# monatis/clip.cpp

Measured on AMD Instinct MI355X. Metric: image+text embeddings/sec, higher is better.
Workload: dtype f16

## Files before the change

### clip_cpp_amd/__init__.py

```python
import ctypes as C
import os
import weakref

import numpy as np

_HERE = os.path.dirname(os.path.abspath(__file__))
LIB_PATH = os.environ.get("CLIP_AMD_LIB") or os.path.join(_HERE, "libclip.so")


class ClipTextHparams(C.Structure):
    _fields_ = [("n_vocab", C.c_int32), ("num_positions", C.c_int32), ("hidden_size", C.c_int32),
                ("n_intermediate", C.c_int32), ("projection_dim", C.c_int32), ("n_head", C.c_int32),
                ("n_layer", C.c_int32), ("eps", C.c_float)]


class ClipVisionHparams(C.Structure):
    _fields_ = [("image_size", C.c_int32), ("patch_size", C.c_int32), ("hidden_size", C.c_int32),
                ("n_intermediate", C.c_int32), ("projection_dim", C.c_int32), ("n_head", C.c_int32),
                ("n_layer", C.c_int32), ("eps", C.c_float)]


class ClipTokens(C.Structure):
    _fields_ = [("data", C.POINTER(C.c_int32)), ("size", C.c_size_t)]


class ClipImageU8(C.Structure):
    _fields_ = [("nx", C.c_int), ("ny", C.c_int), ("data", C.POINTER(C.c_uint8)), ("size", C.c_size_t)]


class ClipImageF32(C.Structure):
    _fields_ = [("nx", C.c_int), ("ny", C.c_int), ("data", C.POINTER(C.c_float)), ("size", C.c_size_t)]


class ClipImageU8Batch(C.Structure):
    _fields_ = [("data", C.POINTER(ClipImageU8)), ("size", C.c_size_t)]


class ClipImageF32Batch(C.Structure):
    _fields_ = [("data", C.POINTER(ClipImageF32)), ("size", C.c_size_t)]


API_SYMBOLS = [
    "clip_model_load", "clip_free", "clip_get_text_hparams", "clip_get_vision_hparams", "clip_tokenize",
    "clip_image_u8_make", "clip_image_f32_make", "clip_image_u8_clean", "clip_image_f32_clean", "clip_image_u8_free",
    "clip_image_f32_free", "clip_image_load_from_file", "clip_image_preprocess", "clip_image_batch_preprocess",
    "clip_text_encode", "clip_image_encode", "clip_image_batch_encode", "clip_compare_text_and_image",
    "clip_similarity_score", "softmax_with_sorting", "clip_zero_shot_label_image", "clip_model_quantize",
    "ggml_time_init", "ggml_time_us", "ggml_time_ms",
]
AMD_SYMBOLS = [
    "clip_amd_device_count", "clip_amd_model_load", "clip_amd_model_load_multi", "clip_amd_ctx_device_count", "clip_amd_weights_from_cache", "clip_amd_shard_bounds",
    "clip_amd_gathered_embeddings", "clip_amd_ctx_device", "clip_amd_set_stream", "clip_amd_set_device_shared", "clip_amd_image_batch_encode_device_multi",
    "clip_amd_text_batch_encode_device_multi", "clip_amd_encode_pair_device_multi",
    "clip_amd_image_batch_encode_device", "clip_text_batch_encode", "clip_amd_text_batch_encode_device",
    "clip_amd_image_batch_preprocess_device", "clip_amd_image_batch_encode_u8",
    "clip_amd_zero_shot_score_device", "clip_amd_zero_shot_label_images",
    "clip_amd_synchronize", "clip_amd_profile_enable", "clip_amd_profile_read", "clip_amd_profile_report",
    "clip_amd_test_gemm", "clip_amd_test_gemm_ex", "clip_amd_test_gemm_tile", "clip_amd_test_gemm_tile_ex", "clip_amd_test_skinny", "clip_amd_test_layernorm", "clip_amd_test_attention", "clip_amd_bench_gemm",
    "clip_amd_test_attention_ex", "clip_amd_bench_attention",
    "clip_amd_test_layernorm_ex", "clip_amd_test_text_embed", "clip_amd_test_im2col", "clip_amd_test_layernorm_prep", "clip_amd_test_rows",
    "clip_amd_index_create", "clip_amd_index_add", "clip_amd_index_add_device", "clip_amd_index_size", "clip_amd_index_dim",
    "clip_amd_index_search", "clip_amd_index_search_device", "clip_amd_index_save", "clip_amd_index_load", "clip_amd_index_free",
    "clip_amd_bench_search", "clip_amd_index_range_search", "clip_amd_index_pairs", "clip_amd_bench_range",
    "clip_amd_index_remove", "clip_amd_index_live", "clip_amd_index_live_mask", "clip_amd_index_compact", "clip_amd_index_search_subset",
    "clip_amd_index_search_subset_device", "clip_amd_index_range_search_subset", "clip_amd_bench_search_subset",
    "clip_amd_index_search_ids", "clip_amd_index_search_ids_device", "clip_amd_index_knn_graph", "clip_amd_test_index_knn_route", "clip_amd_bench_knn",
    "clip_amd_index_search_index", "clip_amd_index_append", "clip_amd_test_index_cross_route", "clip_amd_bench_cross",
    "clip_amd_image_batch_encode_files", "clip_amd_image_batch_encode_memory", "clip_amd_test_jpeg_plan", "clip_amd_test_jpeg_decode_device",
    "clip_amd_bench_jpeg_kernels", "clip_amd_test_jpeg_device_count",
    "clip_amd_index_search_grouped", "clip_amd_index_search_grouped_device", "clip_amd_bench_search_grouped",
    "clip_amd_image_batch_encode_regions", "clip_amd_image_batch_preprocess_regions_device", "clip_amd_image_batch_encode_files_grid",
    "clip_amd_image_batch_encode_memory_grid",
    "clip_amd_index_search_sets", "clip_amd_index_search_sets_device", "clip_amd_index_search_ids_sets", "clip_amd_test_index_sets_block",
    "clip_amd_bench_search_sets",
    "clip_amd_index_search_distinct", "clip_amd_index_search_distinct_device", "clip_amd_index_search_ids_distinct",
    "clip_amd_test_index_distinct_block", "clip_amd_bench_search_distinct",
]

_lib = None


def build_lib(force=False):
    import importlib
    return importlib.import_module(__name__ + ".build").build(force=force)


def lib():
    global _lib
    if _lib is not None:
        return _lib
    if not os.path.exists(LIB_PATH):
        build_lib()
    L = C.CDLL(LIB_PATH)
    vp, i32, f32p = C.c_void_p, C.c_int, C.POINTER(C.c_float)
    L.clip_model_load.restype = vp
    L.clip_model_load.argtypes = [C.c_char_p, i32]
    L.clip_amd_model_load.restype = vp
    L.clip_amd_model_load.argtypes = [C.c_char_p, i32, i32]
    L.clip_amd_model_load_multi.restype = vp
    L.clip_amd_model_load_multi.argtypes = [C.c_char_p, i32, i32]
    L.clip_amd_ctx_device_count.restype = i32
    L.clip_amd_ctx_device_count.argtypes = [vp]
    L.clip_amd_weights_from_cache.restype = i32
    L.clip_amd_weights_from_cache.argtypes = [vp]
    L.clip_amd_shard_bounds.argtypes = [i32, i32, i32, C.POINTER(i32), C.POINTER(i32), C.POINTER(i32)]
    L.clip_amd_gathered_embeddings.restype = vp
    L.clip_amd_gathered_embeddings.argtypes = [vp, i32]
    L.clip_free.argtypes = [vp]
    L.clip_get_text_hparams.restype = C.POINTER(ClipTextHparams)
    L.clip_get_text_hparams.argtypes = [vp]
    L.clip_get_vision_hparams.restype = C.POINTER(ClipVisionHparams)
    L.clip_get_vision_hparams.argtypes = [vp]
    L.clip_tokenize.restype = C.c_bool
    L.clip_tokenize.argtypes = [vp, C.c_char_p, C.POINTER(ClipTokens)]
    L.clip_image_u8_make.restype = C.POINTER(ClipImageU8)
    L.clip_image_f32_make.restype = C.POINTER(ClipImageF32)
    L.clip_image_u8_clean.argtypes = [C.POINTER(ClipImageU8)]
    L.clip_image_f32_clean.argtypes = [C.POINTER(ClipImageF32)]
    L.clip_image_u8_free.argtypes = [C.POINTER(ClipImageU8)]
    L.clip_image_f32_free.argtypes = [C.POINTER(ClipImageF32)]
    L.clip_image_load_from_file.restype = C.c_bool
    L.clip_image_load_from_file.argtypes = [C.c_char_p, C.POINTER(ClipImageU8)]
    L.clip_image_preprocess.restype = C.c_bool
    L.clip_image_preprocess.argtypes = [vp, C.POINTER(ClipImageU8), C.POINTER(ClipImageF32)]
    L.clip_image_batch_preprocess.argtypes = [vp, i32, C.POINTER(ClipImageU8Batch), C.POINTER(ClipImageF32Batch)]
    L.clip_text_encode.restype = C.c_bool
    L.clip_text_encode.argtypes = [vp, i32, C.POINTER(ClipTokens), f32p, C.c_bool]
    L.clip_text_batch_encode.restype = C.c_bool
    L.clip_text_batch_encode.argtypes = [vp, i32, C.POINTER(ClipTokens), C.c_size_t, f32p, C.c_bool]
    L.clip_image_encode.restype = C.c_bool
    L.clip_image_encode.argtypes = [vp, i32, C.POINTER(ClipImageF32), f32p, C.c_bool]
    L.clip_image_batch_encode.restype = C.c_bool
    L.clip_image_batch_encode.argtypes = [vp, i32, C.POINTER(ClipImageF32Batch), f32p, C.c_bool]
    L.clip_compare_text_and_image.restype = C.c_bool
    L.clip_compare_text_and_image.argtypes = [vp, i32, C.c_char_p, C.POINTER(ClipImageU8), f32p]
    L.clip_similarity_score.restype = C.c_float
    L.clip_similarity_score.argtypes = [f32p, f32p, i32]
    L.softmax_with_sorting.restype = C.c_bool
    L.softmax_with_sorting.argtypes = [f32p, i32, f32p, C.POINTER(C.c_int)]
    L.clip_zero_shot_label_image.restype = C.c_bool
    L.clip_zero_shot_label_image.argtypes = [vp, i32, C.POINTER(ClipImageU8), C.POINTER(C.c_char_p), C.c_size_t, f32p,
                                             C.POINTER(C.c_int)]
    L.clip_model_quantize.restype = C.c_bool
    L.clip_model_quantize.argtypes = [C.c_char_p, C.c_char_p, i32]
    L.clip_amd_device_count.restype = i32
    L.clip_amd_ctx_device.restype = i32
    L.clip_amd_ctx_device.argtypes = [vp]
    L.clip_amd_set_stream.argtypes = [vp, vp]
    L.clip_amd_set_device_shared.restype = None
    L.clip_amd_set_device_shared.argtypes = [vp, i32]
    L.clip_amd_synchronize.argtypes = [vp]
    L.clip_amd_image_batch_encode_device.restype = C.c_bool
    L.clip_amd_image_batch_encode_device.argtypes = [vp, vp, i32, vp, C.c_bool]
    L.clip_amd_image_batch_preprocess_device.restype = C.c_bool
    L.clip_amd_image_batch_preprocess_device.argtypes = [vp, C.POINTER(ClipImageU8), i32, vp]
    L.clip_amd_zero_shot_score_device.restype = C.c_bool
    L.clip_amd_zero_shot_score_device.argtypes = [vp, vp, i32, vp, i32, i32, vp, vp]
    L.clip_amd_zero_shot_label_images.restype = C.c_bool
    L.clip_amd_zero_shot_label_images.argtypes = [vp, C.POINTER(ClipImageU8), i32, C.POINTER(C.c_char_p), C.c_size_t, f32p, C.POINTER(C.c_int)]
    L.clip_amd_image_batch_encode_u8.restype = C.c_bool
    L.clip_amd_image_batch_encode_u8.argtypes = [vp, C.POINTER(ClipImageU8), i32, f32p, C.c_bool]
    L.clip_amd_text_batch_encode_device.restype = C.c_bool
    L.clip_amd_text_batch_encode_device.argtypes = [vp, vp, C.POINTER(C.c_int32), i32, vp, C.c_bool]
    L.clip_amd_image_batch_encode_device_multi.restype = C.c_bool
    L.clip_amd_image_batch_encode_device_multi.argtypes = [vp, C.POINTER(vp), i32, C.c_bool, f32p]
    L.clip_amd_text_batch_encode_device_multi.restype = C.c_bool
    L.clip_amd_text_batch_encode_device_multi.argtypes = [vp, C.POINTER(vp), C.POINTER(C.c_int32), i32, C.c_bool, f32p]
    L.clip_amd_encode_pair_device_multi.restype = C.c_bool
    L.clip_amd_encode_pair_device_multi.argtypes = [vp, C.POINTER(vp), i32, C.POINTER(vp), C.POINTER(C.c_int32), i32, C.c_bool, f32p, f32p]
    L.clip_amd_profile_enable.argtypes = [vp, C.c_bool]
    L.clip_amd_profile_report.restype = i32
    L.clip_amd_profile_report.argtypes = [vp, C.c_char_p, i32, C.c_bool]
    L.clip_amd_test_gemm.restype = i32
    L.clip_amd_test_gemm.argtypes = [i32, vp, C.c_int64, C.c_int64, f32p, C.c_int64, f32p, f32p, f32p, i32, i32]
    L.clip_amd_test_gemm_ex.restype = i32
    L.clip_amd_test_gemm_ex.argtypes = [i32, vp, C.c_int64, C.c_int64, f32p, C.c_int64, f32p, f32p, f32p, i32, i32, i32, C.c_float, i32, i32, f32p]
    L.clip_amd_test_lnfold.restype = i32
    L.clip_amd_test_lnfold.argtypes = [i32, vp, C.c_int64, C.c_int64, vp, C.c_int64, f32p, C.c_int64, f32p, f32p, f32p, f32p, C.c_float, f32p,
                                       i32, i32, i32, i32, i32, C.c_float, f32p, f32p]
    L.clip_amd_test_gemm_tile.restype = i32
    L.clip_amd_test_gemm_tile.argtypes = [C.c_int64, C.c_int64, C.c_int64, i32]
    L.clip_amd_test_gemm_tile_ex.restype = i32
    L.clip_amd_test_gemm_tile_ex.argtypes = [C.c_int64, C.c_int64, C.c_int64, i32, i32]
    L.clip_amd_test_skinny.restype = i32
    L.clip_amd_test_skinny.argtypes = [i32, vp, C.c_int64, C.c_int64, f32p, C.c_int64, f32p, f32p, f32p, f32p, C.c_float, f32p, i32, i32, C.c_float, f32p]
    L.clip_amd_bench_gemm.restype = C.c_float
    L.clip_amd_bench_gemm.argtypes = [i32, C.c_int64, C.c_int64, C.c_int64, i32, i32, i32]
    L.clip_amd_test_layernorm.restype = i32
    L.clip_amd_test_layernorm.argtypes = [f32p, f32p, f32p, C.c_float, C.c_int64, C.c_int64, f32p, i32]
    u16p, i32p = C.POINTER(C.c_uint16), C.POINTER(C.c_int32)
    L.clip_amd_test_layernorm_ex.restype = i32
    L.clip_amd_test_layernorm_ex.argtypes = [f32p, C.c_int64, i32, i32p, i32, f32p, f32p, C.c_float, i32, i32, u16p, i32, f32p, i32]
    L.clip_amd_test_text_embed.restype = i32
    L.clip_amd_test_text_embed.argtypes = [i32, vp, C.c_int64, i32, i32p, i32p, i32, i32, f32p, i32, f32p, i32, f32p, u16p, i32, f32p, f32p]
    L.clip_amd_test_im2col.restype = i32
    L.clip_amd_test_im2col.argtypes = [f32p, i32, i32, i32, i32, i32, u16p]
    L.clip_amd_test_layernorm_prep.restype = i32
    L.clip_amd_test_layernorm_prep.argtypes = [f32p, i32, f32p, f32p, C.c_float, i32, i32, f32p, i32, f32p, f32p, i32, i32, f32p, i32, u16p, i32, f32p, f32p]
    L.clip_amd_test_rows.restype = i32
    L.clip_amd_test_rows.argtypes = [i32, vp, vp, i32p, C.c_int64, C.c_int64, C.c_int64, C.c_int64, C.c_int64, vp, vp]
    L.clip_amd_test_attention.restype = i32
    L.clip_amd_test_attention.argtypes = [f32p, i32, i32, i32, i32, i32, f32p]
    L.clip_amd_test_attention_ex.restype = i32
    L.clip_amd_test_attention_ex.argtypes = [f32p, i32, i32, i32, i32, i32, f32p, i32]
    L.clip_amd_bench_attention.restype = C.c_float
    L.clip_amd_bench_attention.argtypes = [i32, i32, i32, i32, i32, i32, i32]
    i64, i64p = C.c_int64, C.POINTER(C.c_int64)
    L.clip_amd_index_create.restype = vp
    L.clip_amd_index_create.argtypes = [vp, i32, i32]
    L.clip_amd_index_add.restype = C.c_bool
    L.clip_amd_index_add.argtypes = [vp, f32p, i64]
    L.clip_amd_index_add_device.restype = C.c_bool
    L.clip_amd_index_add_device.argtypes = [vp, vp, i64]
    L.clip_amd_index_size.restype = i64
    L.clip_amd_index_size.argtypes = [vp]
    L.clip_amd_index_dim.restype = i32
    L.clip_amd_index_dim.argtypes = [vp]
    L.clip_amd_index_search.restype = C.c_bool
    L.clip_amd_index_search.argtypes = [vp, f32p, i32, i32, f32p, i64p]
    L.clip_amd_index_search_device.restype = C.c_bool
    L.clip_amd_index_search_device.argtypes = [vp, vp, i32, i32, vp, vp]
    L.clip_amd_index_save.restype = C.c_bool
    L.clip_amd_index_save.argtypes = [vp, C.c_char_p]
    L.clip_amd_index_load.restype = vp
    L.clip_amd_index_load.argtypes = [vp, C.c_char_p]
    L.clip_amd_index_free.restype = None
    L.clip_amd_index_free.argtypes = [vp]
    L.clip_amd_bench_search.restype = C.c_float
    L.clip_amd_bench_search.argtypes = [i32, i64, i32, i32, i32, i32]
    L.clip_amd_index_range_search.restype = i64
    L.clip_amd_index_range_search.argtypes = [vp, f32p, i32, C.c_float, i64p, f32p, i64p, i64]
    L.clip_amd_index_pairs.restype = i64
    L.clip_amd_index_pairs.argtypes = [vp, C.c_float, i64p, f32p, i64p, i64]
    L.clip_amd_bench_range.restype = C.c_float
    L.clip_amd_bench_range.argtypes = [i32, i64, i32, i32, C.c_float, i32]
    u64p = C.POINTER(C.c_uint64)
    L.clip_amd_index_remove.restype = i64
    L.clip_amd_index_remove.argtypes = [vp, i64p, i64]
    L.clip_amd_index_live.restype = i64
    L.clip_amd_index_live.argtypes = [vp]
    L.clip_amd_index_live_mask.restype = C.c_bool
    L.clip_amd_index_live_mask.argtypes = [vp, u64p]
    L.clip_amd_index_compact.restype = i64
    L.clip_amd_index_compact.argtypes = [vp, i64p]
    L.clip_amd_index_search_subset.restype = C.c_bool
    L.clip_amd_index_search_subset.argtypes = [vp, f32p, i32, i32, u64p, f32p, i64p]
    L.clip_amd_index_search_subset_device.restype = C.c_bool
    L.clip_amd_index_search_subset_device.argtypes = [vp, vp, i32, i32, vp, vp, vp]
    L.clip_amd_index_range_search_subset.restype = i64
    L.clip_amd_index_range_search_subset.argtypes = [vp, f32p, i32, C.c_float, u64p, i64p, f32p, i64p, i64]
    L.clip_amd_index_search_grouped.restype = C.c_bool
    L.clip_amd_index_search_grouped.argtypes = [vp, f32p, i32, i32, C.POINTER(C.c_int32), u64p, f32p, i64p]
    L.clip_amd_index_search_grouped_device.restype = C.c_bool
    L.clip_amd_index_search_grouped_device.argtypes = [vp, vp, i32, i32, vp, vp, vp, vp]
    L.clip_amd_bench_search_grouped.restype = C.c_float
    L.clip_amd_bench_search_grouped.argtypes = [i32, i64, i32, i32, i32, i32, i32]
    L.clip_amd_index_search_sets.restype = C.c_bool
    L.clip_amd_index_search_sets.argtypes = [vp, f32p, i32, i64p, i64, i32, C.POINTER(C.c_int32), u64p, f32p, i64p, C.POINTER(C.c_int32)]
    L.clip_amd_index_search_sets_device.restype = C.c_bool
    L.clip_amd_index_search_sets_device.argtypes = [vp, vp, i32, i64p, i64, i32, vp, vp, vp, vp, vp]
    L.clip_amd_index_search_ids_sets.restype = C.c_bool
    L.clip_amd_index_search_ids_sets.argtypes = [vp, i64p, i64, i64p, i64, i32, i32, C.POINTER(C.c_int32), u64p, f32p, i64p, C.POINTER(C.c_int32)]
    L.clip_amd_test_index_sets_block.restype = i64
    L.clip_amd_test_index_sets_block.argtypes = [vp, i64]
    L.clip_amd_bench_search_sets.restype = C.c_float
    L.clip_amd_bench_search_sets.argtypes = [i32, i64, i32, i32, i32, i32, i32, i32]
    L.clip_amd_index_search_distinct.restype = C.c_bool
    L.clip_amd_index_search_distinct.argtypes = [vp, f32p, i32, i32, C.c_float, i32, u64p, f32p, i64p, C.POINTER(C.c_int32)]
    L.clip_amd_index_search_distinct_device.restype = C.c_bool
    L.clip_amd_index_search_distinct_device.argtypes = [vp, vp, i32, i32, C.c_float, i32, vp, vp, vp, vp]
    L.clip_amd_index_search_ids_distinct.restype = C.c_bool
    L.clip_amd_index_search_ids_distinct.argtypes = [vp, i64p, i32, i32, C.c_float, i32, i32, u64p, f32p, i64p, C.POINTER(C.c_int32)]
    L.clip_amd_test_index_distinct_block.restype = i32
    L.clip_amd_test_index_distinct_block.argtypes = [vp, i32]
    L.clip_amd_bench_search_distinct.restype = C.c_float
    L.clip_amd_bench_search_distinct.argtypes = [i32, i64, i32, i32, i32, i32, C.c_float, i32, i32]
    L.clip_amd_bench_search_subset.restype = C.c_float
    L.clip_amd_bench_search_subset.argtypes = [i32, i64, i32, i32, i32, C.c_float, i32, i32]
    L.clip_amd_index_search_ids.restype = C.c_bool
    L.clip_amd_index_search_ids.argtypes = [vp, i64p, i32, i32, i32, u64p, f32p, i64p]
    L.clip_amd_index_search_ids_device.restype = C.c_bool
    L.clip_amd_index_search_ids_device.argtypes = [vp, vp, i32, i32, i32, vp, vp, vp]
    L.clip_amd_index_knn_graph.restype = C.c_bool
    L.clip_amd_index_knn_graph.argtypes = [vp, i32, f32p, i64p]
    L.clip_amd_test_index_knn_route.restype = i32
    L.clip_amd_test_index_knn_route.argtypes = [vp, i32]
    L.clip_amd_bench_knn.restype = C.c_float
    L.clip_amd_bench_knn.argtypes = [i32, i64, i32, i32, i32, i32]
    L.clip_amd_index_search_index.restype = C.c_bool
    L.clip_amd_index_search_index.argtypes = [vp, vp, i64p, i64, i32, u64p, f32p, i64p]
    L.clip_amd_index_append.restype = i64
    L.clip_amd_index_append.argtypes = [vp, vp, i64p]
    L.clip_amd_test_index_cross_route.restype = i32
    L.clip_amd_test_index_cross_route.argtypes = [vp, i32]
    L.clip_amd_bench_cross.restype = C.c_float
    L.clip_amd_bench_cross.argtypes = [i32, i64, i64, i32, i32, i32, i32]
    u8p, szp = C.POINTER(C.c_uint8), C.POINTER(C.c_size_t)
    L.clip_amd_image_batch_encode_files.restype = i32
    L.clip_amd_image_batch_encode_files.argtypes = [vp, C.POINTER(C.c_char_p), i32, i32, i32, C.c_bool, f32p, C.POINTER(i32), u8p]
    i32p = C.POINTER(C.c_int32)
    L.clip_amd_image_batch_encode_regions.restype = C.c_bool
    L.clip_amd_image_batch_encode_regions.argtypes = [vp, C.POINTER(ClipImageU8), i32, i32p, i32, f32p, C.c_bool]
    L.clip_amd_image_batch_preprocess_regions_device.restype = C.c_bool
    L.clip_amd_image_batch_preprocess_regions_device.argtypes = [vp, C.POINTER(ClipImageU8), i32, i32p, i32, vp]
    L.clip_amd_image_batch_encode_files_grid.restype = i32
    L.clip_amd_image_batch_encode_files_grid.argtypes = [vp, C.POINTER(C.c_char_p), i32, i32, i32, i32, C.c_bool, f32p, i32p, C.POINTER(i32), u8p]
    L.clip_amd_image_batch_encode_memory_grid.restype = i32
    L.clip_amd_image_batch_encode_memory_grid.argtypes = [vp, C.POINTER(C.c_char_p), szp, i32, i32, i32, i32, C.c_bool, f32p, i32p, C.POINTER(i32), u8p]
    L.clip_amd_image_batch_encode_memory.restype = i32
    L.clip_amd_image_batch_encode_memory.argtypes = [vp, C.POINTER(C.c_char_p), szp, i32, i32, i32, C.c_bool, f32p, C.POINTER(i32), u8p]
    L.clip_amd_test_jpeg_plan.restype = i32
    L.clip_amd_test_jpeg_plan.argtypes = [C.c_char_p, C.c_size_t, C.POINTER(i32)]
    L.clip_amd_test_jpeg_decode_device.restype = i32
    L.clip_amd_test_jpeg_decode_device.argtypes = [C.c_char_p, C.c_size_t, u8p, C.c_size_t, C.POINTER(i32), C.POINTER(i32)]
    L.clip_amd_test_jpeg_device_count.restype = C.c_longlong
    L.clip_amd_test_jpeg_device_count.argtypes = []
    L.clip_amd_bench_jpeg_kernels.restype = i32
    L.clip_amd_bench_jpeg_kernels.argtypes = [C.c_char_p, C.c_size_t, i32, i32, f32p, C.POINTER(C.c_double)]
    _lib = L
    return L


def device_count():
    return lib().clip_amd_device_count()


def _fp(a):
    return a.ctypes.data_as(C.POINTER(C.c_float))


def _struct_to_dict(s):
    return {f: getattr(s, f) for f, _ in s._fields_}


class Clip:

    def __init__(self, model_path_or_repo_id, verbosity=0, device=None, n_devices=None):
        L = lib()
# ... 728 lines not shown
```

### clip_cpp_amd/build.py

```python
import os
import shutil
import subprocess
import sys
from concurrent.futures import ThreadPoolExecutor

HERE = os.path.dirname(os.path.abspath(__file__))
CSRC = os.path.join(HERE, "csrc")
BUILD = os.path.join(HERE, "build")
LIB = os.path.join(HERE, "libclip.so")
GGML_STUB = os.path.join(HERE, "libggml.so")
ARCH = "gfx950"

HOST_SOURCES = ["gguf.cpp", "quant.cpp", "load.cpp", "forward.cpp", "tokenizer.cpp", "preprocess.cpp", "image_io.cpp", "image_formats.cpp",
                "jpeg_decode.cpp", "host_pipeline.cpp", "files_pipeline.cpp", "api.cpp", "search.cpp"]
HIP_SOURCES = ["k_attn.hip", "k_attn_long.hip", "k_attn_f32.hip", "k_misc.hip", "k_preproc.hip", "k_jpeg.hip", "k_gemm.hip", "k_gemm8.hip", "k_gemm4.hip", "k_gemm32.hip", "k_gemm_f32.hip", "k_skinny.hip", "k_gemm_ring.hip", "k_fold.hip", "k_search.hip", "k_join.hip", "k_graph.hip", "k_group.hip", "k_sets.hip", "k_distinct.hip"]
GEMM_WTYPES = [0, 1, 2, 3, 4, 5]
EXTRA_FLAGS = {"k_attn_f32.hip": ["-fno-slp-vectorize"], "k_attn_long.hip": ["-fno-slp-vectorize"], "k_gemm_f32.hip": ["-fno-slp-vectorize"]}

COMMON = ["-O3", "-std=c++17", "-fPIC", "-ffp-contract=off", "-Wall", "-Wno-unused-function", "-Wno-unused-result", "-Wno-inline-asm", "-Wno-bitwise-instead-of-logical",
          "-I" + os.path.join(os.path.dirname(HERE), "include")]


def hipcc():
    for c in (os.environ.get("HIPCC"), shutil.which("hipcc"), "/opt/rocm/bin/hipcc"):
        if c and os.path.exists(c):
            return c
    raise RuntimeError("hipcc not found")


def _newer(target, deps):
    if not os.path.exists(target):
        return True
    t = os.path.getmtime(target)
    return any(os.path.getmtime(d) > t for d in deps)


def _run(cmd):
    r = subprocess.run(cmd, stdout=subprocess.PIPE, stderr=subprocess.STDOUT, text=True)
    if r.returncode != 0:
        raise RuntimeError("command failed: %s\n%s" % (" ".join(cmd), r.stdout))
    return r.stdout


def build(force=False, verbose=False):
    os.makedirs(BUILD, exist_ok=True)
    cc = hipcc()
    headers = [os.path.join(CSRC, f) for f in os.listdir(CSRC) if f.endswith(".h")]
    headers += [os.path.join(os.path.dirname(HERE), "include", f) for f in ("clip.h", "clip_amd.h")]
    jobs = []
    objs = []
    for src in HOST_SOURCES:
        o = os.path.join(BUILD, src + ".o")
        objs.append(o)
        s = os.path.join(CSRC, src)
        if force or _newer(o, [s] + headers):
            jobs.append([cc, "-x", "hip", "--offload-arch=" + ARCH, "-fwrapv"] + COMMON + ["-c", s, "-o", o])
    for src in HIP_SOURCES:
        s = os.path.join(CSRC, src)
        o = os.path.join(BUILD, src + ".o")
        objs.append(o)
        if force or _newer(o, [s] + headers):
            jobs.append([cc, "--offload-arch=" + ARCH] + COMMON + EXTRA_FLAGS.get(src, []) + ["-c", s, "-o", o])
    s = os.path.join(CSRC, "k_gemm.hip")
    for wt in GEMM_WTYPES:
        o = os.path.join(BUILD, "k_gemm_wt%d.o" % wt)
        objs.append(o)
        if force or _newer(o, [s] + headers):
            jobs.append([cc, "--offload-arch=" + ARCH] + COMMON + ["-DCLIPAMD_GEMM_WT=%d" % wt, "-c", s, "-o", o])
    s = os.path.join(CSRC, "k_skinny.hip")
    for wt in GEMM_WTYPES:
        o = os.path.join(BUILD, "k_skinny_wt%d.o" % wt)
        objs.append(o)
        if force or _newer(o, [s] + headers):
            jobs.append([cc, "--offload-arch=" + ARCH] + COMMON + ["-DCLIPAMD_SKINNY_WT=%d" % wt, "-c", s, "-o", o])
    s = os.path.join(CSRC, "k_gemm_ring.hip")
    for wt in GEMM_WTYPES:
        o = os.path.join(BUILD, "k_gemm_ring_wt%d.o" % wt)
        objs.append(o)
        if force or _newer(o, [s] + headers):
            jobs.append([cc, "--offload-arch=" + ARCH] + COMMON + ["-DCLIPAMD_RING_WT=%d" % wt, "-c", s, "-o", o])
    if jobs:
        with ThreadPoolExecutor(max_workers=min(8, os.cpu_count() or 4)) as ex:
            for out in ex.map(_run, jobs):
                if verbose and out.strip():
                    print(out)
    if force or jobs or _newer(LIB, objs):
        _run([cc, "--offload-arch=" + ARCH, "-shared", "-fPIC", "-o", LIB] + objs + ["-lz", "-lpthread", "-ldl"])
    stub_src = os.path.join(CSRC, "ggml_stub.c")
    if force or _newer(GGML_STUB, [stub_src]):
        _run(["gcc", "-O2", "-fPIC", "-shared", "-o", GGML_STUB, stub_src])
    return LIB


if __name__ == "__main__":
    p = build(force="--force" in sys.argv, verbose=True)
    print("built", p)
```

### clip_cpp_amd/csrc/api.cpp

```cpp
#include <algorithm>
#include <chrono>
#include <cmath>
#include <cstdio>
#include <cstdlib>
#include <cstring>
#include <exception>
#include <set>
#include <thread>
#include <vector>

#include "../../include/clip_amd.h"
#include "model.h"

using namespace clipamd;

namespace {

int default_device() {
    const char * e = getenv("CLIP_AMD_DEVICE");
    if (!e || !*e) e = getenv("LOCAL_RANK");
    if (e && *e) {
        int n = 0;
        if (hipGetDeviceCount(&n) == hipSuccess && n > 0) return atoi(e) % n;
        (void)hipGetLastError();
// ... 895 lines not shown
    void * wbase = nullptr;
    if (!repack_for_test(type, raw.data(), N, K, W, &wbase)) return -2.f;
    const int Kpad = W.Kpad;
    DBuf dx((size_t)(M + 1) * Kpad * 2), dbias((size_t)N * 4), dout((size_t)M * N * 4);
    std::vector<uint16_t> hx((size_t)M * Kpad);
    for (auto & v : hx) { st = st * 1664525u + 1013904223u; v = f32_to_f16_bits(((int)(st >> 9) % 2001 - 1000) * 1e-3f); }
    (void)hipMemcpy(dx.p, hx.data(), hx.size() * 2, hipMemcpyHostToDevice);
    (void)hipMemset(dbias.p, 0, (size_t)N * 4);
    (void)hipMemset(dout.p, 0, (size_t)M * N * 4);
    GemmParams p;
    p.A = (const half_t *)dx.p; p.lda = Kpad; p.M = (int)M; p.W = W; p.bias = (const float *)dbias.p; p.ldc = (int)N; p.out = dout.p;
    p.resid = (const float *)dout.p; p.qcols = 0;
    DBuf skw((size_t)64 << 20), skc(4096 * 4);
    (void)hipMemset(skc.p, 0, 4096 * 4);
    p.sk_ws = (float *)skw.p; p.sk_ws_floats = (size_t)16 << 20; p.sk_cnt = (unsigned *)skc.p; p.sk_cnt_n = 4096;
    DBuf panel((size_t)W.Npad * W.Kpad * 2);
    const bool pre = (epilogue >> 16) & 1;
    if (pre && W.wtype != W_F16 && W.wtype != W_F32 && panel.p) {
        const DevWeight * w = &W;
        half_t * o = (half_t *)panel.p;
        launch_dequant(&w, &o, 1, nullptr);
        p.w16_pre = (const half_t *)panel.p;
    } else {
        p.w16_scratch = (half_t *)panel.p; p.w16_scratch_halfs = panel.p ? (size_t)W.Npad * W.Kpad : 0;
    }
    p.debug = (epilogue >> 8) & 0xFF;
    const bool fold = (epilogue >> 17) & 1;
    epilogue &= 0xFF;
    const int st_stride = (int)((M + 63) & ~(int64_t)63);
    DBuf dstats(fold ? (size_t)(N > K ? N : K) / 32 * st_stride * 8 + 64 : 16), dvec(fold ? (size_t)(N > K ? N : K) * 4 + 64 : 16), dxg(fold ? (size_t)M * N * 2 + 64 : 16);
    if (fold) {
        std::vector<float> hs((size_t)(N > K ? N : K) / 32 * st_stride * 2), hv((size_t)(N > K ? N : K), 1.0f);
        for (size_t i = 0; i < hs.size(); i += 2) { hs[i] = 0.5f * 64; hs[i + 1] = 60.f; }
        (void)hipMemcpy(dstats.p, hs.data(), hs.size() * 4, hipMemcpyHostToDevice);
        (void)hipMemcpy(dvec.p, hv.data(), hv.size() * 4, hipMemcpyHostToDevice);
        if (epilogue == EPI_RESID_F32) {
            p.xg_out = (half_t *)dxg.p; p.ldxg = (int)N; p.xg_gamma = (const float *)dvec.p; p.stats_out = (float2 *)dstats.p; p.stats_stride = st_stride;
        } else if (epilogue == EPI_F16 || epilogue == EPI_GELU_F16 || epilogue == EPI_QGELU_F16) {
            p.ln_c = (const float *)dvec.p; p.ln_stats = (const float2 *)dstats.p; p.ln_slotw = 64; p.ln_slots = (int)K / 64; p.ln_stride = st_stride; p.ln_eps = 1e-5f;
        }
    }
    hipEvent_t a, b;
    (void)hipEventCreate(&a);
    (void)hipEventCreate(&b);
    int rot = 1;
    { const char * e = getenv("GEMM_ROTATE"); if (e) rot = atoi(e); if (rot < 1) rot = 1; if (rot > 64) rot = 64; }
    std::vector<DevWeight> Ws(1, p.W);
    std::vector<const half_t *> pans(1, p.w16_pre);
    std::vector<void *> owned;
    for (int r = 1; r < rot; r++) {
        DevWeight Wr;
        void * base = nullptr;
        if (!repack_for_test(type, raw.data(), N, K, Wr, &base)) break;
        owned.push_back(base);
        const half_t * pr = nullptr;
        if (pre && Wr.wtype != W_F16 && Wr.wtype != W_F32) {
            void * pp = nullptr;
            if (hipMalloc(&pp, (size_t)Wr.Npad * Wr.Kpad * 2) != hipSuccess) break;
            owned.push_back(pp);
            const DevWeight * w = &Wr;
            half_t * o = (half_t *)pp;
            launch_dequant(&w, &o, 1, nullptr);
            pr = (const half_t *)pp;
        }
        Ws.push_back(Wr);
        pans.push_back(pr);
    }
    rot = (int)Ws.size();
    auto go = [&](int i) { p.W = Ws[i % rot]; if (pre) p.w16_pre = pans[i % rot]; launch_gemm(p, epilogue, tile, nullptr); };
    for (int i = 0; i < 3; i++) go(i);
    (void)hipEventRecord(a, nullptr);
    for (int i = 0; i < iters; i++) go(i);
    (void)hipEventRecord(b, nullptr);
    float ms = -1.f;
    if (hipEventSynchronize(b) == hipSuccess && hipGetLastError() == hipSuccess) (void)hipEventElapsedTime(&ms, a, b);
    (void)hipEventDestroy(a);
    (void)hipEventDestroy(b);
    for (void * o : owned) (void)hipFree(o);
    if (getenv("CLIPAMD_G8_STAMPS")) {
        const int nwg = 4096;
        std::vector<unsigned long long> st((size_t)nwg * 8);
        (void)hipMemcpy(st.data(), skw.p, st.size() * 8, hipMemcpyDeviceToHost);
        FILE * f = fopen(getenv("CLIPAMD_G8_STAMPS"), "a");
        if (f) {
            fprintf(f, "# N=%lld K=%lld M=%lld epi=%d tile=%d\n", (long long)N, (long long)K, (long long)M, epilogue, tile);
            for (int i = 0; i < nwg; i++) {
                const unsigned long long * s8 = &st[(size_t)i * 8];
                if (!s8[0] || !s8[3]) continue;
                fprintf(f, "%d %llu %llu %llu %llu %llu %llu %llu\n", i, s8[0], s8[1], s8[2], s8[3], s8[5], s8[4], s8[6]);
            }
            fclose(f);
        }
    }
    (void)hipFree(wbase);
    return ms < 0 ? -4.f : ms * 1000.f / iters;
}

int clip_amd_test_skinny(int type, const void * w_raw, int64_t N, int64_t K, const float * x, int64_t M, const float * bias, const float * resid,
                         const float * ln_w, const float * ln_b, float eps, float * y, int epilogue, int qcols, float qscale, float * stats_out) {
    int ndev = 0;
    if (hipGetDeviceCount(&ndev) != hipSuccess || ndev <= 0) { (void)hipGetLastError(); return -1; }
    DevWeight W;
    void * wbase = nullptr;
    if (!repack_for_test(type, w_raw, N, K, W, &wbase)) return -2;
    const int Kpad = W.Kpad;
    DBuf dx32((size_t)M * K * 4), dx16((size_t)(M + 1) * Kpad * 2), dbias((size_t)N * 4), dout((size_t)M * N * 4), dout32((size_t)M * N * 4), dlw((size_t)K * 4), dlb((size_t)K * 4),
        dst((size_t)2 * SKINNY_MAX_ROWS * 128 * 8);
    hipStream_t s = nullptr;
    (void)hipMemcpy(dx32.p, x, (size_t)M * K * 4, hipMemcpyHostToDevice);
    if (bias) (void)hipMemcpy(dbias.p, bias, (size_t)N * 4, hipMemcpyHostToDevice);
    (void)hipMemset(dst.p, 0, (size_t)2 * SKINNY_MAX_ROWS * 128 * 8);
    SkinnyParams p;
    p.M = (int)M; p.W = W; p.bias = bias ? (const float *)dbias.p : nullptr; p.ldc = (int)N; p.qcols = qcols; p.qscale = qscale;
    if (ln_w) {
        (void)hipMemcpy(dlw.p, ln_w, (size_t)K * 4, hipMemcpyHostToDevice);
        (void)hipMemcpy(dlb.p, ln_b, (size_t)K * 4, hipMemcpyHostToDevice);
        launch_row_stats((const float *)dx32.p, (int)K, (int)M, (int)K, (float2 *)dst.p, s);
        p.x32 = (const float *)dx32.p; p.ldx = (int)K; p.ln_w = (const float *)dlw.p; p.ln_b = (const float *)dlb.p; p.eps = eps;
        p.stats_in = (const float2 *)dst.p; p.stats_slots = 1;
    } else {
        launch_f32_to_f16((const float *)dx32.p, (int)K, (half_t *)dx16.p, Kpad, (int)M, (int)K, Kpad, s);
        p.A16 = (const half_t *)dx16.p; p.lda = Kpad;
    }
    int epi = EPI_F32;
    switch (epilogue) {
    case 0: epi = EPI_F32; p.out = dout32.p; break;
    case 1: epi = EPI_F16; p.out = dout.p; break;
    case 2: epi = EPI_GELU_F16; p.out = dout.p; break;
    case 3: epi = EPI_QGELU_F16; p.out = dout.p; break;
    case 4:
        epi = EPI_RESID_F32;
        (void)hipMemcpy(dout32.p, resid, (size_t)M * N * 4, hipMemcpyHostToDevice);
        p.out = dout32.p; p.resid = (const float *)dout32.p;
        p.stats_out = (float2 *)dst.p + (size_t)SKINNY_MAX_ROWS * 128;
        break;
    default: (void)hipFree(wbase); return -3;
    }
    int rc = 0;
    if (!skinny_supported(p, epi)) rc = -5;
    else {
        launch_skinny(p, epi, s);
        if (epi == EPI_F16 || epi == EPI_GELU_F16 || epi == EPI_QGELU_F16)
            launch_f16_to_f32((const half_t *)dout.p, (int)N, (float *)dout32.p, (int)N, (int)M, (int)N, s);
        if (hipDeviceSynchronize() != hipSuccess || hipGetLastError() != hipSuccess) rc = -4;
        else {
            (void)hipMemcpy(y, dout32.p, (size_t)M * N * 4, hipMemcpyDeviceToHost);
            if (stats_out && epi == EPI_RESID_F32) (void)hipMemcpy(stats_out, (float2 *)dst.p + (size_t)SKINNY_MAX_ROWS * 128, (size_t)128 * 128 * 8, hipMemcpyDeviceToHost);
        }
    }
    (void)hipFree(wbase);
    return rc;
}

static bool test_device() {
    int ndev = 0;
    if (hipGetDeviceCount(&ndev) != hipSuccess || ndev <= 0) { (void)hipGetLastError(); return false; }
    return true;
}
static void poison32(const DBuf & d, size_t n) { if (n) (void)hipMemsetD32((hipDeviceptr_t)d.p, 0x7fc00000, n); }
static void poison16(const DBuf & d, size_t n) { if (n) (void)hipMemsetD16((hipDeviceptr_t)d.p, 0x7e00, n); }
static void upload(const DBuf & d, const void * src, size_t bytes) { if (src && bytes) (void)hipMemcpy(d.p, src, bytes, hipMemcpyHostToDevice); }
static void download(void * dst, const DBuf & d, size_t bytes) { if (dst && bytes) (void)hipMemcpy(dst, d.p, bytes, hipMemcpyDeviceToHost); }
static bool test_rows_ok(const int32_t * in_rows, int64_t in_row_mul, int64_t rows, int64_t n_src) {
    if (!in_rows) return in_row_mul >= 0 && (rows - 1) * in_row_mul < n_src;
    for (int64_t r = 0; r < rows; r++)
        if (in_rows[r] < 0 || in_rows[r] >= n_src) return false;
    return true;
}
static bool test_sync() { return hipDeviceSynchronize() == hipSuccess && hipGetLastError() == hipSuccess; }

int clip_amd_test_layernorm_ex(const float * x, int64_t x_rows, int ldx, const int32_t * in_rows, int in_row_mul, const float * w, const float * b, float eps,
                               int rows, int h, uint16_t * out16, int ld16, float * out32, int ld32) {
    if (!test_device()) return -1;
    if (rows <= 0 || x_rows <= 0 || h <= 0 || h % 4 || ldx < h || (out16 && ld16 < h) || (out32 && ld32 < h) || ldx % 4 || ld16 % 4 || ld32 % 4 ||
        !test_rows_ok(in_rows, in_row_mul, rows, x_rows)) return -3;
    const size_t n16 = out16 ? (size_t)rows * ld16 : 0, n32 = out32 ? (size_t)rows * ld32 : 0;
    DBuf dx((size_t)x_rows * ldx * 4), dr((size_t)rows * 4), dw((size_t)h * 4), db((size_t)h * 4), d16(n16 * 2), d32(n32 * 4);
    upload(dx, x, (size_t)x_rows * ldx * 4);
    upload(dr, in_rows, (size_t)rows * 4);
    upload(dw, w, (size_t)h * 4);
    upload(db, b, (size_t)h * 4);
    poison16(d16, n16);
    poison32(d32, n32);
    launch_layernorm((const float *)dx.p, ldx, in_rows ? (const int *)dr.p : nullptr, in_row_mul, (const float *)dw.p, (const float *)db.p, eps, rows, h,
                     out16 ? (half_t *)d16.p : nullptr, ld16, out32 ? (float *)d32.p : nullptr, ld32, nullptr);
    if (!test_sync()) return -4;
    download(out16, d16, n16 * 2);
    download(out32, d32, n32 * 4);
    return 0;
}

int clip_amd_test_layernorm(const float * x, const float * w, const float * b, float eps, int64_t rows, int64_t h, float * y, int out_f16) {
    if (!out_f16) return clip_amd_test_layernorm_ex(x, rows, (int)h, nullptr, 1, w, b, eps, (int)rows, (int)h, nullptr, 0, y, (int)h);
    std::vector<uint16_t> y16((size_t)rows * h);
    const int rc = clip_amd_test_layernorm_ex(x, rows, (int)h, nullptr, 1, w, b, eps, (int)rows, (int)h, y16.data(), (int)h, nullptr, 0);
    if (rc == 0)
        for (size_t i = 0; i < y16.size(); i++) y[i] = f16_bits_to_f32(y16[i]);
    return rc;
}

int clip_amd_test_text_embed(int type, const void * tok_raw, int64_t tok_bytes, int h, const int32_t * ids, const int32_t * seq_start, int nseq, int rows,
                             const float * pos, int n_pos, const float * gamma_next, int centred, float * x, uint16_t * xg, int ldxg, float * stats, float * mu) {
    if (!test_device()) return -1;
    if (rows <= 0 || nseq <= 0 || n_pos <= 0 || tok_bytes <= 0 || h <= 0 || h % 64 || h > 2048 || ldxg < h || ldxg % 4) return -3;
    size_t row_bytes = 0;
    switch (type) {
    case 0: row_bytes = (size_t)h * 4; break;
    case 1: row_bytes = (size_t)h * 2; break;
    case 2: row_bytes = (size_t)(h / 32) * 18; break;
    case 3: row_bytes = (size_t)(h / 32) * 20; break;
    case 6: row_bytes = (size_t)(h / 32) * 22; break;
    case 7: row_bytes = (size_t)(h / 32) * 24; break;
    case 8: row_bytes = (size_t)(h / 32) * 34; break;
    default: return -3;
    }
    if (seq_start[0] != 0 || seq_start[nseq] != rows) return -3;
    for (int i = 0; i < nseq; i++)
        if (seq_start[i + 1] <= seq_start[i] || seq_start[i + 1] - seq_start[i] > n_pos) return -3;
    for (int r = 0; r < rows; r++)
        if (ids[r] < 0 || ((size_t)ids[r] + 1) * row_bytes > (size_t)tok_bytes) return -3;
    const size_t nx = (size_t)rows * h, ng = (size_t)rows * ldxg;
    DBuf dt((size_t)tok_bytes), di((size_t)rows * 4), ds((size_t)(nseq + 1) * 4), dp((size_t)n_pos * h * 4), dg((size_t)h * 4), dx(nx * 4), dxg(ng * 2),
        dst((size_t)rows * 8), dmu((size_t)rows * 4);
    upload(dt, tok_raw, (size_t)tok_bytes);
    upload(di, ids, (size_t)rows * 4);
    upload(ds, seq_start, (size_t)(nseq + 1) * 4);
    upload(dp, pos, (size_t)n_pos * h * 4);
    upload(dg, gamma_next, (size_t)h * 4);
    poison32(dx, nx);
    poison16(dxg, ng);
    poison32(dst, (size_t)rows * 2);
    poison32(dmu, (size_t)rows);
    if (gamma_next)
        launch_text_embed((const int32_t *)di.p, (const int *)ds.p, nseq, rows, dt.p, type, (const float *)dp.p, h, (float *)dx.p, nullptr, (const float *)dg.p,
                          (half_t *)dxg.p, ldxg, (float2 *)dst.p, centred ? (float *)dmu.p : nullptr);
    else
        launch_text_embed((const int32_t *)di.p, (const int *)ds.p, nseq, rows, dt.p, type, (const float *)dp.p, h, (float *)dx.p, nullptr);
    if (!test_sync()) return -4;
    download(x, dx, nx * 4);
    download(xg, dxg, ng * 2);
    download(stats, dst, (size_t)rows * 8);
    download(mu, dmu, (size_t)rows * 4);
    return 0;
}

int clip_amd_test_im2col(const float * imgs, int imgs_f16, int B, int S, int P, int Kpad, uint16_t * col) {
    if (!test_device()) return -1;
    if (B <= 0 || S <= 0 || P <= 0 || S % P || Kpad < 3 * P * P || Kpad % 2) return -3;
    const size_t n_in = (size_t)B * S * S * 3, n_col = (size_t)B * (S / P) * (S / P) * Kpad;
    DBuf d32(n_in * 4), d16(n_in * 2), dc(n_col * 2);
    upload(d32, imgs, n_in * 4);
    poison16(dc, n_col);
    if (imgs_f16) launch_f32_to_f16((const float *)d32.p, (int)n_in, (half_t *)d16.p, (int)n_in, 1, (int)n_in, (int)n_in, nullptr);
    launch_im2col(imgs_f16 ? d16.p : d32.p, imgs_f16 != 0, (half_t *)dc.p, B, S, P, Kpad, nullptr);
    if (!test_sync()) return -4;
    download(col, dc, n_col * 2);
    return 0;
}

int clip_amd_test_layernorm_prep(const float * x, int ldx, const float * w, const float * b, float eps, int rows, int h, const float * gamma_next, int centred,
                                 const float * class_embd, const float * pos0, int T, int in_place, float * out32, int ld32, uint16_t * xg, int ldxg,
                                 float * stats, float * mu) {
    if (!test_device()) return -1;
    if (in_place) ld32 = ldx;
    if (rows <= 0 || h <= 0 || h % 64 || h > 2048 || ldx < h || ld32 < h || ldx % 4 || ld32 % 4 || ldxg < h || ldxg % 4 || !gamma_next || (w != nullptr) != (b != nullptr) ||
        (class_embd != nullptr) != (pos0 != nullptr) || (class_embd && T <= 0)) return -3;
    const size_t nx = (size_t)rows * ldx, no = (size_t)rows * ld32, ng = (size_t)rows * ldxg;
    DBuf dx(nx * 4), dw((size_t)h * 4), db((size_t)h * 4), dg((size_t)h * 4), dc((size_t)h * 4), dp((size_t)h * 4), dout(in_place ? 0 : no * 4), dxg(ng * 2),
        dst((size_t)rows * 8), dmu((size_t)rows * 4);
    upload(dx, x, nx * 4);
    upload(dw, w, (size_t)h * 4);
    upload(db, b, (size_t)h * 4);
    upload(dg, gamma_next, (size_t)h * 4);
    upload(dc, class_embd, (size_t)h * 4);
    upload(dp, pos0, (size_t)h * 4);
    if (!in_place) poison32(dout, no);
    poison16(dxg, ng);
    poison32(dst, (size_t)rows * 2);
    poison32(dmu, (size_t)rows);
    launch_layernorm_prep((const float *)dx.p, ldx, w ? (const float *)dw.p : nullptr, w ? (const float *)db.p : nullptr, eps, rows, h,
                          (float *)(in_place ? dx.p : dout.p), ld32, (const float *)dg.p, (half_t *)dxg.p, ldxg, (float2 *)dst.p, nullptr,
                          centred ? (float *)dmu.p : nullptr, class_embd ? (const float *)dc.p : nullptr, class_embd ? (const float *)dp.p : nullptr, T);
    if (!test_sync()) return -4;
    download(out32, in_place ? dx : dout, no * 4);
    download(xg, dxg, ng * 2);
    download(stats, dst, (size_t)rows * 8);
    download(mu, dmu, (size_t)rows * 4);
    return 0;
}

int clip_amd_test_rows(int op, const void * in0, const void * in1, const int32_t * idx, int64_t n0, int64_t n1, int64_t n2, int64_t n3, int64_t n4,
                       void * out0, void * out1) {
    if (!test_device()) return -1;
    if (!in0 || !out0 || n0 <= 0 || n1 <= 0) return -3;
    switch (op) {
    case 0: {
        const size_t B = (size_t)n0, T = (size_t)n1, h = (size_t)n2;
        if (!in1 || n2 <= 0) return -3;
        DBuf dc(h * 4), dp(h * 4), dx(B * T * h * 4);
        upload(dc, in0, h * 4);
        upload(dp, in1, h * 4);
        upload(dx, out0, B * T * h * 4);
        launch_cls_rows((float *)dx.p, (const float *)dc.p, (const float *)dp.p, (int)B, (int)T, (int)h, nullptr);
        if (!test_sync()) return -4;
        download(out0, dx, B * T * h * 4);
        return 0;
// ... 225 lines not shown
```

### clip_cpp_amd/csrc/forward.cpp

```cpp
#include <cmath>
#include <cstdio>
#include <cstdlib>
#include <cstring>
#include <thread>
#include <utility>

#include "model.h"

namespace clipamd {

namespace {

constexpr size_t kGuardBytes = 4096;
constexpr int kGuardByte = 0xA5;
bool guard_mode() {
    static const bool on = [] { const char * e = getenv("CLIP_AMD_GUARD"); return e && e[0] == '1'; }();
    return on;
}

struct Carver {
    uint8_t * base;
    size_t off = 0;
    std::vector<size_t> * gaps = nullptr;
    explicit Carver(void * b, std::vector<size_t> * g = nullptr) : base((uint8_t *)b), gaps(g) { if (gaps) gaps->clear(); }
// ... 121 lines not shown
    ctx->w16_panel_halfs = 0;
    if (hipMalloc((void **)&ctx->w16_panel, halfs * sizeof(half_t)) != hipSuccess) { (void)hipGetLastError(); return false; }
    ctx->w16_panel_halfs = halfs;
    return true;
}

LayerPanels dequant_layer(clip_ctx * ctx, const DevLayer & l, int rows, const half_t * const * res = nullptr) {
    LayerPanels lp;
    const DevWeight * ws[4] = {&l.qkv, &l.o, &l.ff1, &l.ff2};
    const half_t ** slot[4] = {&lp.qkv, &lp.o, &lp.ff1, &lp.ff2};
    const DevWeight * jw[4];
    half_t * jo[4];
    int nj = 0;
    size_t need = 0;
    bool todo[4];
    for (int i = 0; i < 4; i++) {
        const bool for32 = i == 0 || i == 2;
        if (res && res[i] && (!for32 || gemm_tile_for(rows, ws[i]->N, ws[i]->Kpad, false, device_shared(ctx)) % 1000 == 261)) { *slot[i] = res[i]; todo[i] = false; continue; }
        todo[i] = ws[i]->wtype != W_F16 && ws[i]->wtype != W_F32 && gemm_tile_uses_panel(gemm_tile_for(rows, ws[i]->N, ws[i]->Kpad, true));
        if (todo[i]) need += (size_t)ws[i]->Npad * ws[i]->Kpad;
    }
    if (!need || !ensure_panel(ctx, need)) return lp;
    size_t off = 0;
    for (int i = 0; i < 4; i++)
        if (todo[i]) {
            jw[nj] = ws[i];
            jo[nj] = ctx->w16_panel + off;
            *slot[i] = jo[nj];
            off += (size_t)ws[i]->Npad * ws[i]->Kpad;
            nj++;
        }
    ProfScope ps(ctx, "dequant_layer", rows, nj, 0, 0, (double)need * 2.5625);
    launch_dequant(jw, jo, nj, ctx->stream);
    return lp;
}

bool skinny_enabled() {
    static int on = -1;
    if (on < 0) { const char * e = getenv("CLIP_AMD_SKINNY"); on = !(e && e[0] == '0'); }
    return on != 0;
}

#ifdef CLIPAMD_SK_TIMING
unsigned long long * g_sk_stamps = nullptr;
int g_sk_stamp_launch = 0;
constexpr int SK_STAMP_LAUNCHES = 512;
#endif

void skinny(clip_ctx * ctx, const char * what, const SkinnyParams & p0, int epi) {
#ifdef CLIPAMD_SK_TIMING
    SkinnyParams p = p0;
    if (!g_sk_stamps && hipMalloc((void **)&g_sk_stamps, SK_STAMP_LAUNCHES * 16 * 8) == hipSuccess) (void)hipMemset(g_sk_stamps, 0, SK_STAMP_LAUNCHES * 16 * 8);
    if (g_sk_stamps) p.stamps = g_sk_stamps + (size_t)(g_sk_stamp_launch++ % SK_STAMP_LAUNCHES) * 16;
#else
    const SkinnyParams & p = p0;
#endif
    if (!ctx->profiling) { launch_skinny(p, epi, ctx->stream); return; }
    char fam[96];
    const int nw = (!p.x32 && p.W.Kpad >= 2048 && (epi == EPI_RESID_F32 || epi == EPI_PATCH_F32)) ? 8 : 4;
    snprintf(fam, sizeof fam, "skinny_kernel<%d,1,%d,%d,%s>/%s", p.W.wtype, nw, epi, p.x32 ? "true" : "false", what);
    const double fl = 2.0 * p.M * (double)p.W.N * p.W.K;
    const double by = weight_bytes(p.W) + (double)p.M * p.W.K * (p.x32 ? 4 : 2) + (double)p.M * p.W.N * (epi == EPI_RESID_F32 ? 8 : epi == EPI_F32 || epi == EPI_PATCH_F32 ? 4 : 2);
    ProfScope ps(ctx, fam, p.M, p.W.N, p.W.K, fl, by);
    launch_skinny(p, epi, ctx->stream);
}

int skinny_row_limit() {
    static int lim = -1;
    if (lim < 0) {
        const char * e = getenv("CLIP_AMD_SKINNY_ROWS");
        lim = e ? atoi(e) : 64;
        if (lim > SKINNY_MAX_ROWS) lim = SKINNY_MAX_ROWS;
    }
    return lim;
}

bool layers_fit_skinny(const DevTower & tw, int rows, int h, int ff) {
    if (!skinny_enabled() || rows <= 0 || rows > skinny_row_limit() || h > 2048 || h % 16 || h / 16 > 128 || tw.layers.empty()) return false;
    const DevLayer & l = tw.layers[0];
    if (l.qkv.wtype == W_F32 || l.o.wtype == W_F32 || l.ff1.wtype == W_F32 || l.ff2.wtype == W_F32) return false;
    return l.qkv.K == l.qkv.Kpad && l.ff1.K == l.ff1.Kpad && l.o.N == h && l.ff2.N == h && l.ff1.N == ff;
}

const half_t * const * resident_panels(clip_ctx * ctx, const DevTower & tw, int which, int rows) {
    if (!ctx->resident_panels_on || tw.layers.empty()) return nullptr;
    if (ctx->owner) {
        clip_ctx * o = ctx->owner;
        return (o->res_panel_mask[which] && o->res_panels[which].size() == 4 * tw.layers.size()) ? o->res_panels[which].data() : nullptr;
    }
    const DevLayer & l0 = tw.layers[0];
    unsigned want = 0;
    if (l0.ff2.wtype != W_F16 && l0.ff2.wtype != W_F32 && rows >= 4096 && gemm_tile_uses_panel(gemm_tile_for(rows, l0.ff2.N, l0.ff2.Kpad, false))) want |= 8u;
    if (l0.o.wtype != W_F16 && l0.o.wtype != W_F32 && rows >= 4096 && rows < 32768 && gemm_tile_uses_panel(gemm_tile_for(rows, l0.o.N, l0.o.Kpad, false))) want |= 2u;
    if (rows >= 32768 && l0.qkv.wtype != W_F16 && l0.qkv.wtype != W_F32 && gemm_tile_for(rows, l0.qkv.N, l0.qkv.Kpad, false, device_shared(ctx)) % 1000 == 261) want |= 1u;
    if (rows >= 32768 && l0.ff1.wtype != W_F16 && l0.ff1.wtype != W_F32 && gemm_tile_for(rows, l0.ff1.N, l0.ff1.Kpad, false, device_shared(ctx)) % 1000 == 261) want |= 4u;
    if (!want) return nullptr;
    auto & tab = ctx->res_panels[which];
    if ((ctx->res_panel_mask[which] & want) == want && tab.size() == 4 * tw.layers.size()) return tab.data();
    hipStreamCaptureStatus cs = hipStreamCaptureStatusNone;
    (void)hipStreamIsCapturing(ctx->stream, &cs);
    if (cs != hipStreamCaptureStatusNone) return (ctx->res_panel_mask[which] && tab.size() == 4 * tw.layers.size()) ? tab.data() : nullptr;
    want |= ctx->res_panel_mask[which];
    (void)hipStreamSynchronize(ctx->stream);
    if (ctx->res_panel_buf[which]) (void)hipFree(ctx->res_panel_buf[which]);
    ctx->res_panel_buf[which] = nullptr;
    ctx->res_panel_mask[which] = 0;
    tab.clear();
    size_t halfs = 0;
    for (const DevLayer & l : tw.layers) {
        const DevWeight * ws[4] = {&l.qkv, &l.o, &l.ff1, &l.ff2};
        for (int i = 0; i < 4; i++) if (want >> i & 1) halfs += (size_t)ws[i]->Npad * ws[i]->Kpad;
    }
    if (hipMalloc((void **)&ctx->res_panel_buf[which], halfs * sizeof(half_t)) != hipSuccess) { (void)hipGetLastError(); return nullptr; }
    size_t off = 0;
    for (const DevLayer & l : tw.layers) {
        const DevWeight * ws[4] = {&l.qkv, &l.o, &l.ff1, &l.ff2};
        for (int i = 0; i < 4; i++) {
            if (!(want >> i & 1)) { tab.push_back(nullptr); continue; }
            half_t * o = ctx->res_panel_buf[which] + off;
            launch_dequant(&ws[i], &o, 1, ctx->stream);
            tab.push_back(o);
            off += (size_t)ws[i]->Npad * ws[i]->Kpad;
        }
    }
    (void)hipStreamSynchronize(ctx->stream);
    ctx->res_panel_mask[which] = want;
    return tab.data();
}

bool fold_pays(const DevTower & tw, int rows, bool shared) {
    if (tw.layers.empty()) return false;
    const DevLayer & l = tw.layers[0];
    for (const DevWeight * w : {&l.qkv, &l.o, &l.ff1, &l.ff2})
        if (gemm_tile_uses_panel(gemm_tile_for(rows, w->N, w->Kpad, w->wtype != W_F16, shared)) &&
            gemm_tile_for(rows, w->N, w->Kpad, w->wtype != W_F16, shared) % 1000 != 261) return false;
    return true;
}

struct TowerPass {
    const DevTower * tw = nullptr;
    int which = 0;
    int rows = 0, h = 0, nh = 0, ff = 0, proj = 0;
    float eps = 0.f;
    int nseq = 0, T_uniform = 0;
    const int * seq_start = nullptr;
    int max_len = 0;
    bool causal = false;
    const int * in_rows = nullptr;
    int in_row_mul = 1;
    TowerBufs b;
    bool skinny = false;
    bool fold = false;
    bool prune = false;
    bool f32 = false;
    float * mu = nullptr;
    const half_t * const * resp = nullptr;
};

void choose_form(const clip_ctx * ctx, TowerPass & P) {
    const DevTower & tw = *P.tw;
    P.skinny = layers_fit_skinny(tw, P.rows, P.h, P.ff);
    P.fold = ctx->ln_fold && !tw.layers.empty() && (ctx->ln_fold_force || fold_pays(tw, P.rows, device_shared(ctx)));
    P.prune = ctx->prune_last && !P.skinny && !tw.layers.empty() && P.rows > P.nseq;
    P.f32 = acts_f32(ctx, tw);
    P.mu = ctx->ln_fold_centre ? P.b.mu : nullptr;
}

struct LnState {
    int slots = 1, slotw = 0;
    float * mu_cur = nullptr, * mu_alt = nullptr;
    float2 * st_cur = nullptr, * st_alt = nullptr;
    int st_slots = 1;
    LnState(const clip_ctx * ctx, const TowerPass & P) : slotw(P.h), mu_cur(P.mu), mu_alt(P.mu ? P.mu + P.b.st_stride : nullptr),
                                                         st_cur(ctx->sk_stats), st_alt(ctx->sk_stats + (size_t)SKINNY_MAX_ROWS * 128) {}
};

struct Linear { const char * gemm_tag, * skinny_tag; const DevWeight & W; const float * bias; const half_t * panel; };
struct Norm { const float * w, * b, * c, * bf; };

void norm_linear(clip_ctx * ctx, const TowerPass & P, LnState & ln, const Linear & L, const Norm & N, half_t * out, int epi, float qscale = 1.0f, int qcols = 0) {
    const TowerBufs & B = P.b;
    if (P.skinny) {
        SkinnyParams p;
        p.M = P.rows; p.W = L.W; p.out = out; p.ldc = L.W.N; p.qscale = qscale; p.qcols = qcols; p.eps = P.eps;
        if (P.fold) {
            p.A16 = B.xn; p.lda = P.h; p.bias = N.bf; p.ln_c = N.c; p.fstats = B.stats; p.fslots = ln.slots; p.fslotw = ln.slotw; p.fstride = B.st_stride;
            if (ln.mu_cur) { p.ln_mu = ln.mu_cur; p.mu_out = ln.mu_alt; std::swap(ln.mu_cur, ln.mu_alt); }
        } else {
            p.x32 = B.x; p.ldx = P.h; p.ln_w = N.w; p.ln_b = N.b; p.stats_in = ln.st_cur; p.stats_slots = ln.st_slots; p.bias = L.bias;
        }
        skinny(ctx, L.skinny_tag, p, epi);
        return;
    }
    GemmParams p;
    p.A = B.xn; p.lda = P.h; p.M = P.rows; p.W = L.W; p.out = out; p.ldc = L.W.N; p.w16_pre = L.panel; p.qscale = qscale; p.qcols = qcols; p.act_f32 = P.f32;
    if (P.fold) {
        p.bias = N.bf; p.ln_c = N.c; p.ln_stats = B.stats; p.ln_slots = ln.slots; p.ln_slotw = ln.slotw; p.ln_stride = B.st_stride; p.ln_eps = P.eps;
        if (ln.mu_cur) { p.ln_mu = ln.mu_cur; p.mu_out = ln.mu_alt; std::swap(ln.mu_cur, ln.mu_alt); }
    } else {
        ProfScope ps(ctx, "layernorm", P.rows, P.h, 0, 0, (double)P.rows * P.h * 6);
        layernorm_act(P.f32, B.x, P.h, nullptr, 1, N.w, N.b, P.eps, P.rows, P.h, B.xn, ctx->stream);
        p.bias = L.bias;
    }
    gemm(ctx, L.gemm_tag, p, epi);
}

void resid_linear(clip_ctx * ctx, const TowerPass & P, LnState & ln, const Linear & L, const half_t * A, const float * gamma_next) {
    const TowerBufs & B = P.b;
    if (P.skinny) {
        SkinnyParams p;
        p.A16 = A; p.lda = L.W.K; p.M = P.rows; p.W = L.W; p.bias = L.bias; p.out = B.x; p.ldc = P.h; p.resid = B.x;
        if (!P.fold) {
            p.stats_out = ln.st_alt;
            std::swap(ln.st_cur, ln.st_alt);
            ln.st_slots = P.h / 16;
        } else if (gamma_next) {
            p.xg_mu = ln.mu_cur;
            p.xg_out = B.xn; p.ldxg = P.h; p.xg_gamma = gamma_next; p.fstats_out = B.stats; p.fstride_out = B.st_stride;
            ln.slots = P.h / 16; ln.slotw = 16;
        }
        skinny(ctx, L.skinny_tag, p, EPI_RESID_F32);
        return;
    }
    GemmParams p;
    p.A = A; p.lda = L.W.K; p.M = P.rows; p.W = L.W; p.bias = L.bias; p.out = B.x; p.ldc = P.h; p.resid = B.x; p.w16_pre = L.panel; p.act_f32 = P.f32;
    if (P.fold && gamma_next) {
        p.xg_mu = ln.mu_cur;
        p.xg_out = B.xn; p.ldxg = P.h; p.xg_gamma = gamma_next; p.stats_out = B.stats; p.stats_stride = B.st_stride;
        const bool quant = !p.w16_pre && p.W.wtype != W_F16;
        ln.slotw = gemm_fold_slotw_for(p.M, p.W.N, p.W.Kpad, quant, device_shared(ctx));
        ln.slots = P.h / ln.slotw;
    }
    gemm(ctx, L.gemm_tag, p, EPI_RESID_F32);
}

bool run_layers(clip_ctx * ctx, const TowerPass & P) {
    const DevTower & tw = *P.tw;
    const TowerBufs & B = P.b;
    const int h = P.h, dh = h / P.nh;
    const float qscale = 1.0f / sqrtf((float)dh);
    const int act = ctx->use_gelu ? EPI_GELU_F16 : EPI_QGELU_F16;
    LnState ln(ctx, P);
    for (size_t li = 0; li < tw.layers.size(); li++) {
        const DevLayer & l = tw.layers[li];
        const bool last = li + 1 == tw.layers.size();
        const LayerPanels lp = P.skinny ? LayerPanels() : dequant_layer(ctx, l, P.rows, P.resp ? P.resp + 4 * li : nullptr);
        norm_linear(ctx, P, ln, {"gemm_qkv", "ln1_qkv", l.qkv, l.qkv_b, lp.qkv}, {l.ln1_w, l.ln1_b, l.qkv_c, l.qkv_bf}, B.qkv, EPI_F16, qscale, h);
        {
            const double afl = 4.0 * (double)P.nseq * P.nh * (double)P.max_len * P.max_len * dh;
            ProfScope ps(ctx, "attention", P.nseq * P.nh, P.max_len, dh, afl, (double)P.rows * h * 8);
            if (!(P.f32 ? launch_attention_f32((const float *)B.qkv, (float *)B.att, P.nseq, P.T_uniform, P.seq_start, P.max_len, h, P.nh, P.causal, ctx->stream)
                        : launch_attention(B.qkv, B.att, P.nseq, P.T_uniform, P.seq_start, P.max_len, h, P.nh, P.causal, ctx->stream))) {
                fprintf(stderr, "clip (hip): attention kernel does not support T=%d d_head=%d\n", P.max_len, dh);
                return false;
            }
        }
        if (P.prune && last) break;
        resid_linear(ctx, P, ln, {"gemm_out", "out_resid", l.o, l.o_b, lp.o}, B.att, l.ln2_w);
        norm_linear(ctx, P, ln, {"gemm_ffn_up", "ln2_ffn_up", l.ff1, l.ff1_b, lp.ff1}, {l.ln2_w, l.ln2_b, l.ff1_c, l.ff1_bf}, B.mid, act);
        resid_linear(ctx, P, ln, {"gemm_ffn_down", "ffn_down_resid", l.ff2, l.ff2_b, lp.ff2}, B.mid, last ? nullptr : tw.layers[li + 1].ln1_w);
    }
    return true;
}

void pooled_tail(clip_ctx * ctx, const TowerPass & P) {
    const DevLayer & l = P.tw->layers.back();
    const TowerBufs & B = P.b;
    const int n = P.nseq, h = P.h;
    {
        ProfScope ps(ctx, "gather_pooled", n, h, 0, 0, (double)n * h * 12);
        if (P.f32) {
            launch_gather_rows(B.x, nullptr, P.in_rows, P.in_row_mul, n, h, B.xp, nullptr, ctx->stream);
            launch_gather_rows((const float *)B.att, nullptr, P.in_rows, P.in_row_mul, n, h, (float *)B.ap, nullptr, ctx->stream);
        } else launch_gather_rows(B.x, B.att, P.in_rows, P.in_row_mul, n, h, B.xp, B.ap, ctx->stream);
    }
    TowerPass T = P;
    T.rows = n; T.skinny = T.fold = false;
    T.b.x = B.xp; T.b.att = B.ap; T.b.xn = B.xnp; T.b.mid = B.midp;
    LnState ln(ctx, T);
    resid_linear(ctx, T, ln, {"gemm_out_pooled", "", l.o, l.o_b, nullptr}, T.b.att, nullptr);
    norm_linear(ctx, T, ln, {"gemm_ffn_up_pooled", "", l.ff1, l.ff1_b, nullptr}, {l.ln2_w, l.ln2_b, nullptr, nullptr}, T.b.mid, ctx->use_gelu ? EPI_GELU_F16 : EPI_QGELU_F16);
    resid_linear(ctx, T, ln, {"gemm_ffn_down_pooled", "", l.ff2, l.ff2_b, nullptr}, T.b.mid, nullptr);
}

bool check_device(clip_ctx * ctx, const char * who) {
    if (!ctx || ctx->device < 0) {
        fprintf(stderr, "%s: no HIP device bound to this context — the encoders have no CPU fallback\n", who);
        return false;
    }
    if (hipSetDevice(ctx->device) != hipSuccess) {
        fprintf(stderr, "%s: hipSetDevice(%d) failed\n", who, ctx->device);
        return false;
    }
    return true;
}

bool launch_ok(const char * who) {
    const hipError_t e = hipGetLastError();
    if (e != hipSuccess) {
        fprintf(stderr, "%s: HIP launch error: %s\n", who, hipGetErrorString(e));
        return false;
    }
    return true;
}

void carve_tower(Carver & c, TowerBufs & b, int rows, int n, int h, int ff, int proj, bool f32) {
    b.st_stride = (rows + 63) & ~63;
    b.stats = c.take<float2>((size_t)(h / 16) * b.st_stride);
    b.mu = c.take<float>((size_t)2 * b.st_stride);
    b.x = c.take<float>((size_t)rows * h);
    const size_t aw = f32 ? 2 : 1;
    b.xn = c.take<half_t>(aw * rows * h);
    b.qkv = c.take<half_t>(aw * rows * 3 * h);
    b.att = c.take<half_t>(aw * rows * h);
    b.mid = c.take<half_t>(aw * rows * ff);
    b.pooled = c.take<half_t>(aw * n * h);
    b.emb = c.take<float>((size_t)n * proj);
    b.xp = c.take<float>((size_t)n * h);
    b.ap = c.take<half_t>(aw * n * h);
    b.xnp = c.take<half_t>(aw * n * h);
    b.midp = c.take<half_t>(aw * n * ff);
}

template <typename F> bool carve_workspace(clip_ctx * ctx, F carve) {
    Carver sizer(nullptr);
    carve(sizer);
    if (!ensure_workspace(ctx, sizer.off + 4096)) return false;
    Carver c(ctx->ws.base, &ctx->guard_gaps);
    carve(c);
    return guard_arm(ctx);
}

bool run_tower(clip_ctx * ctx, TowerPass & P, float * d_out, bool normalize) {
    const DevTower & tw = *P.tw;
    const TowerBufs & B = P.b;
    hipStream_t s = ctx->stream;
    if (P.skinny && !P.fold) launch_row_stats(B.x, P.h, P.rows, P.h, ctx->sk_stats, s);
    P.resp = P.skinny ? nullptr : resident_panels(ctx, tw, P.which, P.rows);
    if (!run_layers(ctx, P)) return false;
    if (P.prune) {
        pooled_tail(ctx, P);
        layernorm_act(P.f32, B.xp, P.h, nullptr, 1, tw.post_ln_w, tw.post_ln_b, P.eps, P.nseq, P.h, B.pooled, s);
    } else {
        layernorm_act(P.f32, B.x, P.h, P.in_rows, P.in_row_mul, tw.post_ln_w, tw.post_ln_b, P.eps, P.nseq, P.h, B.pooled, s);
    }
    GemmParams pj;
    pj.A = B.pooled; pj.lda = P.h; pj.M = P.nseq; pj.W = tw.proj; pj.out = B.emb; pj.ldc = P.proj; pj.act_f32 = P.f32;
    gemm(ctx, "gemm_proj", pj, EPI_F32);
    launch_l2norm(B.emb, d_out, P.nseq, P.proj, normalize, s);
    return true;
}

}

void drop_graphs(clip_ctx * ctx) {
    for (auto & g : ctx->vgraphs) {
        if (g.exec) (void)hipGraphExecDestroy(g.exec);
        if (g.graph) (void)hipGraphDestroy(g.graph);
    }
    ctx->vgraphs.clear();
    for (auto & g : ctx->tgraphs) {
        if (g.exec) (void)hipGraphExecDestroy(g.exec);
        if (g.graph) (void)hipGraphDestroy(g.graph);
    }
    ctx->tgraphs.clear();
}

bool ensure_workspace(clip_ctx * ctx, size_t bytes) {
    if (ctx->ws.bytes >= bytes) return true;
    (void)hipStreamSynchronize(ctx->stream);
    drop_graphs(ctx);
    if (ctx->owner) {
        (void)hipStreamSynchronize(ctx->owner->stream);
        drop_graphs(ctx->owner);
    }
    if (ctx->ws.base) (void)hipFree(ctx->ws.base);
    ctx->ws.base = nullptr;
    ctx->ws.bytes = 0;
    const size_t want = bytes + bytes / 8 + (1 << 20);
    if (hipMalloc(&ctx->ws.base, want) != hipSuccess) {
        (void)hipGetLastError();
        fprintf(stderr, "clip (hip): cannot allocate %zu MB of workspace\n", want >> 20);
        return false;
    }
    ctx->ws.bytes = want;
    return true;
}

bool ensure_pinned(clip_ctx * ctx, size_t bytes) {
    if (ctx->pinned_bytes >= bytes) return true;
    if (ctx->pinned) (void)hipHostFree(ctx->pinned);
    ctx->pinned = nullptr;
    ctx->pinned_bytes = 0;
    if (hipHostMalloc(&ctx->pinned, bytes, hipHostMallocDefault) != hipSuccess) {
        (void)hipGetLastError();
        return false;
    }
    ctx->pinned_bytes = bytes;
    return true;
}

bool ensure_io(clip_ctx * ctx, size_t in_bytes, size_t out_bytes) {
    auto grow = [&](void *& p, size_t & have, size_t want) {
        if (have >= want) return true;
        (void)hipStreamSynchronize(ctx->stream);
        if (p) (void)hipFree(p);
        p = nullptr;
        have = 0;
        if (hipMalloc(&p, want) != hipSuccess) { (void)hipGetLastError(); return false; }
        have = want;
        return true;
    };
    return grow(ctx->io_in, ctx->io_in_bytes, in_bytes) && grow(ctx->io_out, ctx->io_out_bytes, out_bytes);
}

void prof_collect(clip_ctx * ctx) {
    if (ctx->pending.empty()) return;
    (void)hipStreamSynchronize(ctx->stream);
    for (auto & p : ctx->pending) {
        float ms = 0;
        if (hipEventElapsedTime(&ms, p.a, p.b) == hipSuccess) {
            ProfEntry & e = ctx->prof[p.tag];
            e.ms += ms;
            e.launches += 1;
            e.flops += p.flops;
            e.bytes += p.bytes;
        }
        (void)hipEventDestroy(p.a);
        (void)hipEventDestroy(p.b);
    }
    ctx->pending.clear();
}

static bool vision_forward_one(clip_ctx * ctx, const float * d_imgs, int B, float * d_out, bool normalize);

static bool vision_forward_launch(clip_ctx * ctx, const float * d_imgs, int B, float * d_out, bool normalize) {
    bool split = !ctx->weights_borrowed && !ctx->sibling_busy && !ctx->profiling && ctx->has_vision_encoder && B >= 2;
    if (split) {
        if (ctx->split_max >= 0) split = B >= ctx->split_min && B <= ctx->split_max;
        else {
            const auto & hp = ctx->vision_hparams;
            const int G = hp.image_size / hp.patch_size;
            const long rows = (long)B * (G * G + 1);
            split = hp.hidden_size >= 1024 ? (rows >= 2000 && rows <= 8400) : (rows >= 2000 && rows <= 3300);
        }
    }
    int ways = split ? std::min(ctx->split_ways, B) : 1;
    clip_ctx * part_ctx[4] = {ctx, nullptr, nullptr, nullptr};
    if (split) {
        hipStreamCaptureStatus cs = hipStreamCaptureStatusNone;
        (void)hipStreamIsCapturing(ctx->stream, &cs);
        for (int w = 1; w < ways; w++) {
            clip_ctx * have = w == 1 ? ctx->sibling : ctx->more_siblings[w - 2];
            part_ctx[w] = have ? have : (cs == hipStreamCaptureStatusNone ? sibling_context(ctx, w - 1) : nullptr);
            if (!part_ctx[w]) { ways = 1; break; }
        }
    }
    ctx->last_launch_split = ways >= 2;
    if (ways < 2) return vision_forward_one(ctx, d_imgs, B, d_out, normalize);
    const size_t per = (size_t)ctx->vision_hparams.image_size * ctx->vision_hparams.image_size * 3;
    const int proj = ctx->vision_hparams.projection_dim;
    if (hipEventRecord(ctx->ev_fork, ctx->stream) != hipSuccess) return false;
    bool ok = true;
    int b0 = 0;
    for (int w = 0; w < ways; w++) {
        const int n = B / ways + (w < B % ways ? 1 : 0);
        clip_ctx * c = part_ctx[w];
        c->input_f16 = ctx->input_f16;
        const float * src = ctx->input_f16 ? (const float *)((const half_t *)d_imgs + (size_t)b0 * per) : d_imgs + (size_t)b0 * per;
        if (w > 0 && hipStreamWaitEvent(c->stream, ctx->ev_fork, 0) != hipSuccess) return false;
        ok = vision_forward_one(c, src, n, d_out + (size_t)b0 * proj, normalize) && ok;
        b0 += n;
    }
    for (int w = 1; w < ways; w++) {
        hipEvent_t ej = w == 1 ? ctx->ev_join : ctx->ev_join_more[w - 2];
        if (hipEventRecord(ej, part_ctx[w]->stream) != hipSuccess || hipStreamWaitEvent(ctx->stream, ej, 0) != hipSuccess) return false;
    }
    return ok;
}

bool renew_streams_after_failed_capture(clip_ctx * ctx) {
    bool ok = true, synced = false;
    auto one = [&](clip_ctx * c) {
        if (!c) return;
        hipStreamCaptureStatus st = hipStreamCaptureStatusNone;
        const hipError_t qe = hipStreamIsCapturing(c->stream, &st);
        (void)hipGetLastError();
        if (qe == hipSuccess && st == hipStreamCaptureStatusNone) return;
        if (c->stream != c->own_stream) { ok = false; return; }
        if (!synced) { (void)hipDeviceSynchronize(); (void)hipGetLastError(); synced = true; }
        hipStream_t fresh = nullptr;
        if (hipStreamCreateWithFlags(&fresh, hipStreamNonBlocking) != hipSuccess) { (void)hipGetLastError(); ok = false; return; }
// ... 307 lines not shown
```

### clip_cpp_amd/csrc/gemm_common.h

```cpp
#pragma once

#include "kernels.h"

namespace clipamd {

typedef _Float16 h8 __attribute__((ext_vector_type(8)));
typedef _Float16 h2 __attribute__((ext_vector_type(2)));
typedef float f4 __attribute__((ext_vector_type(4)));
typedef unsigned int u32x4 __attribute__((ext_vector_type(4)));

namespace {

constexpr int BK = 64;

__device__ __forceinline__ h2 u2h(uint32_t u) { return __builtin_bit_cast(h2, u); }
__device__ __forceinline__ uint32_t h2u(h2 h) { return __builtin_bit_cast(uint32_t, h); }
__device__ __forceinline__ h2 splat(float x) { return (h2){(_Float16)x, (_Float16)x}; }

__device__ __forceinline__ int lds_off(int r, int c) { return r * BK + ((c ^ (r & 7)) << 3); }

template <int WT> struct WFrag;
template <> struct WFrag<W_F16> { uint32_t q; };
template <> struct WFrag<W_Q4_0> { uint32_t q; half_t d; };
template <> struct WFrag<W_Q4_1> { uint32_t q; h2 dm; };
template <> struct WFrag<W_Q5_0> { uint32_t q, h; half_t d; };
template <> struct WFrag<W_Q5_1> { uint32_t q, h; h2 dm; };
template <> struct WFrag<W_Q8_0> { uint32_t q, q1; half_t d; };

template <int WT>
__device__ __forceinline__ uint32_t dequant_hbits(const WFrag<WT> & f, int g) {
    if constexpr (WT == W_Q5_0 || WT == W_Q5_1) return (uint32_t)(((uint64_t)f.h << 4) >> (4 * g));
    else return 0u;
}
template <int WT>
__device__ __forceinline__ uint32_t dequant_wpair(const WFrag<WT> & f, uint32_t hb, int s) {
    if constexpr (WT == W_F16) return f.q;
    else if constexpr (WT == W_Q8_0) {
        const h2 scale = (h2){f.d, f.d};
        const h2 sub = splat(1152.0f);
        const uint32_t w = s < 2 ? f.q : f.q1;
        const uint32_t u = ((s & 1) ? (w >> 8) : w) & 0x00FF00FFu;
        return h2u((u2h(u | 0x64006400u) - sub) * scale);
    } else {
        h2 scale, sub, add;
        if constexpr (WT == W_Q4_0) { scale = (h2){f.d, f.d}; sub = splat(1032.0f); }
        if constexpr (WT == W_Q5_0) { scale = (h2){f.d, f.d}; sub = splat(1040.0f); }
        if constexpr (WT == W_Q4_1 || WT == W_Q5_1) {
            scale = (h2){f.dm[0], f.dm[0]};
            add = (h2){f.dm[1], f.dm[1]};
            sub = splat(1024.0f);
        }
        h2 v;
#ifdef CLIPAMD_DEQUANT_R5
        constexpr bool inplace = false;
#else
        constexpr bool inplace = WT == W_Q4_0 || WT == W_Q4_1;
#endif
        if constexpr (inplace) {
            const uint32_t w = s < 2 ? f.q : f.q >> 8;
            uint32_t magic = 0x64006400u, mask = (s & 1) ? 0x00F000F0u : 0x000F000Fu;
#ifndef CLIPAMD_DEQUANT_R5
            asm("" : "+v"(magic));
            asm("" : "+s"(mask));
#endif
            const uint32_t u = (w & mask) | magic;
            if (s & 1) {
                const float z = WT == W_Q4_0 ? 72.0f : 64.0f;
                v = __builtin_elementwise_fma(u2h(u), splat(0.0625f), splat(-z));
            } else {
                v = u2h(u) - sub;
            }
        } else {
            uint32_t u = ((f.q >> (4 * s)) & 0x000F000Fu) | 0x64006400u;
            if constexpr (WT == W_Q5_0 || WT == W_Q5_1) u |= (hb >> s) & 0x00100010u;
            v = u2h(u) - sub;
        }
        if constexpr (WT == W_Q4_1 || WT == W_Q5_1) v = __builtin_elementwise_fma(v, scale, add);
        else v = v * scale;
        return h2u(v);
    }
}

template <int WT>
__device__ __forceinline__ h8 dequant_wfrag(const WFrag<WT> & f, int g) {
    if constexpr (WT == W_F16) return __builtin_bit_cast(h8, (u32x4){f.q, 0u, 0u, 0u});
    else {
        const uint32_t hb = dequant_hbits<WT>(f, g);
        return __builtin_bit_cast(h8, (u32x4){dequant_wpair<WT>(f, hb, 0), dequant_wpair<WT>(f, hb, 1), dequant_wpair<WT>(f, hb, 2), dequant_wpair<WT>(f, hb, 3)});
    }
}

template <int WT> struct RawBlock { u32x4 qs, qs1; uint32_t h; half_t d; h2 dm; };

template <int WT>
__device__ __forceinline__ void load_block(RawBlock<WT> & r, const DevWeight & W, size_t idx) {
    if constexpr (WT == W_Q8_0) {
        const u32x4 * q = (const u32x4 *)W.qs + idx * 2;
        r.qs = q[0];
        r.qs1 = q[1];
    } else if constexpr (WT != W_F16) {
        r.qs = ((const u32x4 *)W.qs)[idx];
    }
    if constexpr (WT == W_Q5_0 || WT == W_Q5_1) r.h = ((const uint32_t *)W.qh)[idx];
    if constexpr (WT == W_Q4_1 || WT == W_Q5_1) r.dm = ((const h2 *)W.dm)[idx];
    else if constexpr (WT != W_F16) r.d = ((const half_t *)W.dm)[idx];
}

template <int WT>
__device__ __forceinline__ WFrag<WT> block_word(const RawBlock<WT> & r, int j) {
    WFrag<WT> f;
    if constexpr (WT == W_Q8_0) {
        const uint32_t w[8] = {r.qs[0], r.qs[1], r.qs[2], r.qs[3], r.qs1[0], r.qs1[1], r.qs1[2], r.qs1[3]};
        f.q = w[2 * j];
        f.q1 = w[2 * j + 1];
    } else {
        f.q = r.qs[j];
    }
    if constexpr (WT == W_Q5_0 || WT == W_Q5_1) f.h = r.h;
    if constexpr (WT == W_Q4_1 || WT == W_Q5_1) f.dm = r.dm;
    else if constexpr (WT != W_F16) f.d = r.d;
    return f;
}

#define GELU_SCALAR_FENCE(t, x) asm volatile("" : "+v"(t), "+v"(x))
__device__ __forceinline__ float gelu_tanh(float x) {
#ifdef CLIPAMD_GELU_R5
    const float u = 0.79788456080286535587989211986876f * x * (1.0f + 0.044715f * x * x);
    const float e = __expf(2.0f * u);
    return x - x * __builtin_amdgcn_rcpf(e + 1.0f);
#else
    constexpr float C1 = 2.0f * 0.79788456080286535587989211986876f * 1.44269504088896340736f;
    constexpr float C2 = C1 * 0.044715f;
    const float e = __builtin_amdgcn_exp2f(x * __builtin_fmaf(x * x, C2, C1));
    float t = __builtin_amdgcn_rcpf(e + 1.0f);
    GELU_SCALAR_FENCE(t, x);
    float r = __builtin_fmaf(-x, t, x);
    asm volatile("" : "+v"(r));
    return r;
#endif
}
__device__ __forceinline__ float gelu_quick(float x) {
#ifdef CLIPAMD_GELU_R5
    return x * __builtin_amdgcn_rcpf(1.0f + __expf(-1.702f * x));
#else
    float t = __builtin_amdgcn_rcpf(1.0f + __builtin_amdgcn_exp2f(x * (-1.702f * 1.44269504088896340736f)));
    GELU_SCALAR_FENCE(t, x);
    return x * t;
#endif
}

__device__ __forceinline__ void ln_pair32(float s0, float q0, float s1, float q1, float & mean, float & m2) {
    const float m0 = s0 * (1.0f / 32.0f), m1 = s1 * (1.0f / 32.0f);
    const float d = m1 - m0;
    mean = m0 + d * 0.5f;
    m2 = q0 + (q1 + (d * d) * 16.0f);
}

__device__ __forceinline__ float sum4_fgrp(float s) {
    float a = s, b = s;
    asm volatile("s_nop 1\n\tv_permlane16_swap_b32 %0, %1\n\ts_nop 1" : "+v"(a), "+v"(b));
    s = a + b;
    a = s; b = s;
    asm volatile("s_nop 1\n\tv_permlane32_swap_b32 %0, %1\n\ts_nop 1" : "+v"(a), "+v"(b));
    return a + b;
}

template <int C0>
__device__ __forceinline__ void ln_row_chunk(const float2 * st, size_t stride, int units, bool pairs, float w, float invw, float & mean, float & m2) {
    constexpr int CH = 16;
    float mu[CH], q[CH];
    if (pairs) {
        float2 v0[CH], v1[CH];
#pragma unroll
        for (int j = 0; j < CH; j++) {
            const int u = C0 + j < units ? C0 + j : units - 1;
            v0[j] = st[(size_t)(2 * u) * stride];
            v1[j] = st[(size_t)(2 * u + 1) * stride];
        }
#pragma unroll
        for (int j = 0; j < CH; j++) ln_pair32(v0[j].x, v0[j].y, v1[j].x, v1[j].y, mu[j], q[j]);
    } else {
        float2 v[CH];
#pragma unroll
        for (int j = 0; j < CH; j++) {
            const int u = C0 + j < units ? C0 + j : units - 1;
            v[j] = st[(size_t)u * stride];
        }
#pragma unroll
        for (int j = 0; j < CH; j++) { mu[j] = v[j].x * invw; q[j] = v[j].y; }
    }
#pragma unroll
    for (int j = 0; j < CH; j++) {
        constexpr float one = 1.0f;
        const int t = C0 + j;
        const float ok = t < units ? one : 0.0f;
        const float k1 = ok * (one / (float)(t + 1));
        const float k2 = ok * (w * ((float)t / (float)(t + 1)));
        const float d = mu[j] - mean;
        mean = mean + d * k1;
        m2 = m2 + ok * q[j] + (d * d) * k2;
    }
}

__device__ __forceinline__ float2 ln_row_final(const GemmParams & p, int m) {
    const bool pairs = p.ln_slotw == 32;
    const int units = pairs ? p.ln_slots >> 1 : p.ln_slots;
    const float w = pairs ? 64.f : (float)p.ln_slotw, invw = 1.0f / w;
    const float2 * st = p.ln_stats + m;
    const size_t stride = (size_t)p.ln_stride;
    float mean = 0.f, m2 = 0.f;
    ln_row_chunk<0>(st, stride, units, pairs, w, invw, mean, m2);
    if (units > 16) ln_row_chunk<16>(st, stride, units, pairs, w, invw, mean, m2);
    const float invh = 1.0f / ((float)p.ln_slots * (float)p.ln_slotw);
    return make_float2(mean, 1.0f / sqrtf(m2 * invh + p.ln_eps));
}

__device__ __forceinline__ float2 ln_row_centred(const GemmParams & p, int m, bool writer) {
    const float mu = p.ln_mu ? p.ln_mu[m] : 0.f;
    float2 r = ln_row_final(p, m);
    if (writer && p.mu_out) p.mu_out[m] = r.x;
    r.x -= mu;
    return r;
}

template <typename SYNC>
__device__ __forceinline__ void ln_rows_publish(float2 * rs, float2 mine, int tid, int BM, SYNC sync) {
    sync();
    if (tid < BM) rs[tid] = mine;
    sync();
}
template <int TM>
__device__ __forceinline__ void ln_rows_read(float2 (&mr)[TM], bool ln, const float2 * rs_lane) {
#pragma unroll
    for (int b = 0; b < TM; b++) mr[b] = ln ? rs_lane[b * 16] : make_float2(0.f, 1.f);
}

template <int TN> constexpr int fold_slotw() { return TN * 16 >= 64 ? 64 : 32; }

template <int TN, int TM>
__device__ __forceinline__ void resid_fold_tail(const GemmParams & p, f4 (&acc)[TN][TM], int nbase, int mbase, int frow, int fgrp,
                                                half_t * stage, int lane) {
    constexpr int SW = fold_slotw<TN>(), SA = SW / 16;
    static_assert(TN % SA == 0, "a wave's columns are whole statistics slots");
    const int N = p.W.N;
    const bool staged = SA == 4 && stage != nullptr && (p.ldxg & 7) == 0;
    auto mu_of = [&](int b) {
        const int m = mbase + b * 16 + frow;
        return p.xg_mu ? p.xg_mu[m < p.M ? m : p.M - 1] : 0.f;
    };
#pragma unroll
    for (int sp = 0; sp < TN / SA; sp++) {
        const int n = nbase + sp * SW;
        if (n >= N) continue;
        f4 gam[SA];
#pragma unroll
        for (int i = 0; i < SA; i++) gam[i] = *(const f4 *)(p.xg_gamma + n + i * 16 + fgrp * 4);
#pragma unroll
        for (int b = 0; b < TM; b++) {
            float s32[SA / 2], q32[SA / 2];
#pragma unroll
            for (int i = 0; i < SA / 2; i++) {
                const f4 u = acc[sp * SA + 2 * i][b], v = acc[sp * SA + 2 * i + 1][b];
                const float s = sum4_fgrp(((u[0] + u[1]) + (u[2] + u[3])) + ((v[0] + v[1]) + (v[2] + v[3])));
                const float mean = s * (1.0f / 32.0f);
                const f4 du = u - mean, dv = v - mean;
                const float q = sum4_fgrp(((du[0] * du[0] + du[1] * du[1]) + (du[2] * du[2] + du[3] * du[3])) +
                                          ((dv[0] * dv[0] + dv[1] * dv[1]) + (dv[2] * dv[2] + dv[3] * dv[3])));
                s32[i] = s; q32[i] = q;
            }
            float2 o;
            if constexpr (SW == 64) {
                float mean64, q64;
                ln_pair32(s32[0], q32[0], s32[1], q32[1], mean64, q64);
                o = make_float2(mean64 * 64.f, q64);
            } else {
                o = make_float2(s32[0], q32[0]);
            }
            const int m = mbase + b * 16 + frow;
            if (fgrp == 0 && m < p.M) p.stats_out[(size_t)(n / SW) * p.stats_stride + m] = o;
        }
        if constexpr (SA == 4) {
            if (staged) {
                constexpr int RS = 68;
                const int rrow = lane >> 3, rchunk = lane & 7;
#pragma unroll
                for (int b = 0; b < TM; b++) {
                    const float mub = mu_of(b);
#pragma unroll
                    for (int a = 0; a < 4; a++) {
                        const f4 g = (acc[sp * 4 + a][b] - mub) * gam[a];
                        const h2 lo = (h2){(_Float16)g[0], (_Float16)g[1]};
                        const h2 hi = (h2){(_Float16)g[2], (_Float16)g[3]};
                        *(uint2 *)(stage + (b * 16 + frow) * RS + a * 16 + fgrp * 4) = make_uint2(h2u(lo), h2u(hi));
                    }
                }
#pragma unroll
                for (int i = 0; i < TM * 2; i++) {
                    const int ml = i * 8 + rrow;
                    const int m = mbase + ml;
                    const u32x4 v = *(const u32x4 *)(stage + ml * RS + rchunk * 8);
                    if (m < p.M) *(u32x4 *)(p.xg_out + (size_t)m * p.ldxg + n + rchunk * 8) = v;
                }
                continue;
// ... 262 lines not shown
```

### clip_cpp_amd/csrc/k_skinny.hip

```cpp

#include "gemm_common.h"

namespace clipamd {

namespace {

__device__ __forceinline__ h8 normalise8(const f4 lo, const f4 hi, float mean, float rstd, const f4 g0, const f4 g1, const f4 b0, const f4 b1) {
    const f4 y0 = ((lo - mean) * rstd) * g0 + b0;
    const f4 y1 = ((hi - mean) * rstd) * g1 + b1;
    return (h8){(_Float16)y0[0], (_Float16)y0[1], (_Float16)y0[2], (_Float16)y0[3], (_Float16)y1[0], (_Float16)y1[1], (_Float16)y1[2], (_Float16)y1[3]};
}

template <int WT, int MF, int NW, int EPI, bool LNA>
__global__ void __launch_bounds__(NW * 64) skinny_kernel(const SkinnyParams p) {
    constexpr int CH = LNA ? 3 : (MF == 1 ? 6 : 4);
    __shared__ f4 red[NW * MF * 64];
    constexpr bool FOLDC = !LNA && (EPI == EPI_F16 || EPI == EPI_GELU_F16 || EPI == EPI_QGELU_F16);
    __shared__ float2 lnst[(LNA || FOLDC) ? 128 : 1];
    __shared__ float lng[LNA ? 2048 : 1], lnb[LNA ? 2048 : 1];

    const int tid = threadIdx.x;
    const int lane = tid & 63;
    const int wave = __builtin_amdgcn_readfirstlane(tid >> 6);
    const int frow = lane & 15, fgrp = lane >> 4;
    const int n0 = blockIdx.x * 16;
    const int m_base = blockIdx.y * (MF * 16);
    const int nkb = p.W.Kpad / 32;
    const int kb_lo = wave * nkb / NW, kb_hi = (wave + 1) * nkb / NW;

    int mrow[MF];
#pragma unroll
    for (int b = 0; b < MF; b++) { const int m = m_base + b * 16 + frow; mrow[b] = m < p.M ? m : p.M - 1; }
#ifdef CLIPAMD_SK_TIMING
    const bool sk_first = blockIdx.x == 0 && blockIdx.y == 0, sk_last = blockIdx.x == gridDim.x - 1 && blockIdx.y == gridDim.y - 1;
    const bool stamper = p.stamps && tid == 0 && (sk_first || sk_last);
    unsigned long long * stamp = p.stamps + (sk_first ? 0 : 8);
#define SK_STAMP(i_) if (stamper) stamp[i_] = __builtin_amdgcn_s_memtime()
    if (stamper) stamp[6] = __builtin_amdgcn_s_memrealtime();
#else
#define SK_STAMP(i_)
#endif
    SK_STAMP(0);

    struct WReg { WFrag<WT> q; h8 h; };
    auto load_w = [&](WReg & w, int kb) {
        if constexpr (WT == W_F16) {
            w.h = *(const h8 *)((const half_t *)p.W.w16 + (size_t)(n0 + frow) * p.W.Kpad + kb * 32 + fgrp * 8);
        } else {
            const size_t idx = (size_t)kb * p.W.Npad + n0 + frow;
            if constexpr (WT == W_Q8_0) {
                const uint2 q = ((const uint2 *)p.W.qs)[idx * 4 + fgrp];
                w.q.q = q.x;
                w.q.q1 = q.y;
            } else {
                w.q.q = ((const uint32_t *)p.W.qs)[idx * 4 + fgrp];
            }
            if constexpr (WT == W_Q5_0 || WT == W_Q5_1) w.q.h = ((const uint32_t *)p.W.qh)[idx];
            if constexpr (WT == W_Q4_1 || WT == W_Q5_1) w.q.dm = ((const h2 *)p.W.dm)[idx];
            else w.q.d = ((const half_t *)p.W.dm)[idx];
        }
    };
    struct XReg { h8 h; f4 lo, hi; };
    auto load_x = [&](XReg & x, int kb, int b) {
        if constexpr (LNA) {
            const float * src = p.x32 + (size_t)mrow[b] * p.ldx + kb * 32 + fgrp * 8;
            x.lo = *(const f4 *)src;
            x.hi = *(const f4 *)(src + 4);
        } else {
            x.h = *(const h8 *)(p.A16 + (size_t)mrow[b] * p.lda + kb * 32 + fgrp * 8);
        }
    };

    WReg wA[CH], wB[CH];
    XReg xA[CH][MF], xB[CH][MF];
#define SK_LOAD(W_, X_, c_)                                                                    \
    _Pragma("unroll") for (int i = 0; i < CH; i++)                                             \
        if ((c_) + i < kb_hi) {                                                                \
            load_w(W_[i], (c_) + i);                                                           \
            _Pragma("unroll") for (int b = 0; b < MF; b++) load_x(X_[i][b], (c_) + i, b);      \
        }
    SK_LOAD(wA, xA, kb_lo);
    static_assert(MF <= NW, "each wave finalises at most one fragment row");
    f4 bias_pre = (f4){0.f, 0.f, 0.f, 0.f}, resid_pre = (f4){0.f, 0.f, 0.f, 0.f}, c_pre = (f4){0.f, 0.f, 0.f, 0.f}, gam_pre = (f4){0.f, 0.f, 0.f, 0.f};
    const bool foldc = FOLDC && p.ln_c != nullptr;
    float mu_pre = 0.f;
    {
        const int n = n0 + fgrp * 4, m = m_base + wave * 16 + frow;
        if constexpr (EPI == EPI_RESID_F32) { if (p.xg_out && p.xg_mu && wave < MF) mu_pre = p.xg_mu[m < p.M ? m : p.M - 1]; }
        if (EPI != EPI_PATCH_F32 && p.bias && n < p.W.N) bias_pre = *(const f4 *)(p.bias + n);
        if constexpr (FOLDC) { if (foldc && n < p.W.N) c_pre = *(const f4 *)(p.ln_c + n); }
        if constexpr (EPI == EPI_RESID_F32) { if (p.xg_out && n < p.W.N) gam_pre = *(const f4 *)(p.xg_gamma + n); }
        if constexpr (EPI == EPI_RESID_F32) {
            if (wave < MF && m < p.M && n < p.W.N) resid_pre = *(const f4 *)(p.resid + (size_t)m * p.ldc + n);
        }
    }

    SK_STAMP(1);
    float mean[MF], rstd[MF];
    if constexpr (LNA) {
        for (int k4 = tid; k4 < p.W.K / 4; k4 += NW * 64) {
            *(f4 *)(lng + 4 * k4) = *(const f4 *)(p.ln_w + 4 * k4);
            *(f4 *)(lnb + 4 * k4) = *(const f4 *)(p.ln_b + 4 * k4);
        }
        {
            constexpr int TPR = (NW * 64) / (MF * 16);
            const int r = tid / TPR, sub = tid % TPR;
            const int gr = m_base + r;
            const float2 * row = p.stats_in + (size_t)(gr < p.M ? gr : p.M - 1) * p.stats_cap;
            float s1 = 0.f, s2 = 0.f;
            for (int base = 0; base < p.stats_slots; base += TPR * 16) {
                float2 v[16];
#pragma unroll
                for (int i = 0; i < 16; i++) {
                    const int sl = base + i * TPR + sub;
                    v[i] = sl < p.stats_slots ? row[sl] : make_float2(0.f, 0.f);
                }
#pragma unroll
                for (int i = 0; i < 16; i++) { s1 += v[i].x; s2 += v[i].y; }
            }
#pragma unroll
            for (int o = TPR / 2; o > 0; o >>= 1) { s1 += __shfl_xor(s1, o); s2 += __shfl_xor(s2, o); }
            if (sub == 0) {
                const float mu = s1 / (float)p.W.K;
                float var = s2 / (float)p.W.K - mu * mu;
                var = var > 0.f ? var : 0.f;
                lnst[r] = make_float2(mu, 1.0f / sqrtf(var + p.eps));
            }
        }
        __syncthreads();
#pragma unroll
        for (int b = 0; b < MF; b++) { const float2 st = lnst[b * 16 + frow]; mean[b] = st.x; rstd[b] = st.y; }
    }

    if constexpr (FOLDC) {
        if (foldc) {
            constexpr int TPR = (NW * 64) / (MF * 16);
            static_assert(TPR == 16 || TPR == 32, "16 or 32 threads per row");
            const int r = tid / TPR, sub = tid % TPR;
            const int gr = m_base + r;
            const float2 * st = p.fstats + (gr < p.M ? gr : p.M - 1);
            const float mu_in = (sub == 0 && p.ln_mu) ? p.ln_mu[gr < p.M ? gr : p.M - 1] : 0.f;
            const float w = (float)p.fslotw, invw = 1.0f / w;
            float n_ = 0.f, mean_ = 0.f, m2_ = 0.f;
            for (int base = 0; base < p.fslots; base += TPR * 8) {
                float2 v[8];
#pragma unroll
                for (int i = 0; i < 8; i++) {
                    const int sl = base + i * TPR + sub;
                    v[i] = st[(size_t)(sl < p.fslots ? sl : p.fslots - 1) * p.fstride];
                }
#pragma unroll
                for (int i = 0; i < 8; i++) {
                    if (base + i * TPR + sub < p.fslots) {
                        const float nn = n_ + w, d = v[i].x * invw - mean_, inv = __builtin_amdgcn_rcpf(nn);
                        mean_ += d * (w * inv);
                        m2_ += v[i].y + (d * d) * (n_ * w * inv);
                        n_ = nn;
                    }
                }
            }
#pragma unroll
            for (int o = 1; o < TPR; o <<= 1) {
                const float nb = __shfl_xor(n_, o), mb = __shfl_xor(mean_, o), qb = __shfl_xor(m2_, o);
                const bool upper = (sub & o) != 0;
// ... 225 lines not shown
```

### clip_cpp_amd/csrc/kernels.h

```cpp
#pragma once

#include <hip/hip_runtime.h>
#include <cstdint>
#include <cstdio>

#include "jpeg_stages.h"

namespace clipamd {

typedef _Float16 half_t;

template <typename K>
inline void opt_in_dynamic_lds(K kernel, size_t bytes, unsigned long long & done) {
    int dev = 0;
    (void)hipGetDevice(&dev);
    const unsigned long long bit = 1ull << (dev & 63);
    if (done & bit) return;
    const hipError_t e = hipFuncSetAttribute((const void *)kernel, hipFuncAttributeMaxDynamicSharedMemorySize, (int)bytes);
    if (e != hipSuccess) {
        fprintf(stderr, "clip (hip): hipFuncSetAttribute(MaxDynamicSharedMemorySize = %zu) failed: %s\n", bytes, hipGetErrorString(e));
        (void)hipGetLastError();
        return;
    }
    done |= bit;
}

enum WType : int { W_F16 = 0, W_Q4_0 = 1, W_Q4_1 = 2, W_Q5_0 = 3, W_Q5_1 = 4, W_Q8_0 = 5, W_F32 = 6 };

struct DevWeight {
    int wtype = W_F16;
    int N = 0, K = 0;
    int Npad = 0;
    int Kpad = 0;
    const void * qs = nullptr;
    const void * qh = nullptr;
    const void * dm = nullptr;
    const void * w16 = nullptr;
};

enum Epilogue : int {
    EPI_F32 = 0,
    EPI_F16 = 1,
    EPI_GELU_F16 = 2,
    EPI_QGELU_F16 = 3,
    EPI_RESID_F32 = 4,
    EPI_PATCH_F32 = 5,
    EPI_COUNT = 6
};

struct GemmParams {
    const half_t * A = nullptr;
    int lda = 0;
    int M = 0;
    DevWeight W;
    const float * bias = nullptr;
    void * out = nullptr;
    int ldc = 0;
    const float * resid = nullptr;
    float qscale = 1.0f;
    int qcols = 0;
    int Np = 0, T = 0;
    const float * pos = nullptr;
    float * sk_ws = nullptr;
    size_t sk_ws_floats = 0;
    unsigned * sk_cnt = nullptr;
    int sk_cnt_n = 0;
    int ksplit = 1;
    bool no_splitk = false;
    const half_t * w16_pre = nullptr;
    half_t * w16_scratch = nullptr;
    size_t w16_scratch_halfs = 0;
    int debug = 0;
    const float * ln_c = nullptr;
    const float2 * ln_stats = nullptr;
    int ln_slots = 0, ln_slotw = 0;
    int ln_stride = 0;
    float ln_eps = 0.f;
    half_t * xg_out = nullptr;
    int ldxg = 0;
    const float * xg_gamma = nullptr;
    float2 * stats_out = nullptr;
    int stats_stride = 0;
    const float * xg_mu = nullptr;
    const float * ln_mu = nullptr;
    float * mu_out = nullptr;
    bool shared_device = false;
    bool act_f32 = false;
};

void launch_gemm(const GemmParams & p, int epilogue, int tile, hipStream_t stream);
int gemm_tile_for(int M, int N, int Kpad, bool quantised, bool shared_device = false);
inline bool gemm_tile_is_ring(int tile) { return (tile % 1000000) / 1000 == 65; }
inline bool gemm_tile_uses_panel(int tile) { const int bn = tile % 1000; return !gemm_tile_is_ring(tile) && (bn == 256 || (bn >= 258 && bn <= 261)); }

void launch_gemm_ring(const GemmParams & p, int epilogue, int bn, hipStream_t stream);

void launch_gemm8(const GemmParams & p, int epilogue, int tm, hipStream_t stream);
void launch_gemm_f32(const GemmParams & p, int epilogue, hipStream_t stream);
void launch_gemm4(const GemmParams & p, int epilogue, hipStream_t stream);
bool gemm32_supported(const GemmParams & p, int epilogue);
void launch_gemm32(const GemmParams & p, int epilogue, int form, hipStream_t stream);
struct DequantJobs { DevWeight W[4]; half_t * out[4]; int blk_end[4]; int n = 0; };
void launch_dequant(const DevWeight * const * ws, half_t * const * outs, int n, hipStream_t stream);

int gemm_fold_slotw(int tile);
int gemm_fold_slotw_for(int M, int N, int Kpad, bool quantised, bool shared_device = false);
void launch_fold_vectors(const DevWeight & W, const float * gamma, const float * beta, const float * bias, float * c_out, float * b_out,
                         hipStream_t stream);

struct SkinnyParams {
    const half_t * A16 = nullptr;
    int lda = 0;
    const float * x32 = nullptr;
    int ldx = 0;
    const float * ln_w = nullptr, * ln_b = nullptr;
    float eps = 0.f;
    const float2 * stats_in = nullptr;
    int stats_slots = 0;
    int M = 0;
    DevWeight W;
    const float * bias = nullptr;
    void * out = nullptr;
    int ldc = 0;
    const float * resid = nullptr;
    float qscale = 1.0f;
    int qcols = 0;
    int Np = 0, T = 0;
    const float * pos = nullptr;
    float2 * stats_out = nullptr;
    int stats_cap = 128;
    const float * ln_c = nullptr;
    const float2 * fstats = nullptr;
    int fslots = 0, fslotw = 0, fstride = 0;
    half_t * xg_out = nullptr;
    int ldxg = 0;
    const float * xg_gamma = nullptr;
    float2 * fstats_out = nullptr;
    int fstride_out = 0;
    const float * xg_mu = nullptr, * ln_mu = nullptr;
    float * mu_out = nullptr;
    unsigned long long * stamps = nullptr;
};
constexpr int SKINNY_MAX_ROWS = 512;
bool skinny_supported(const SkinnyParams & p, int epilogue);
void launch_skinny(const SkinnyParams & p, int epilogue, hipStream_t stream);
void launch_row_stats(const float * x, int ldx, int rows, int h, float2 * stats, hipStream_t stream);

void launch_layernorm(const float * x, int ldx, const int * in_rows, int in_row_mul, const float * w, const float * b, float eps,
                      int rows, int h, half_t * out16, int ld16, float * out32, int ld32, hipStream_t stream);
void launch_layernorm_prep(const float * x, int ldx, const float * w, const float * b, float eps, int rows, int h, float * out32, int ld32,
                           const float * gamma_next, half_t * xg, int ldxg, float2 * stats, hipStream_t stream, float * mu_out = nullptr,
                           const float * class_embd = nullptr, const float * pos0 = nullptr, int T = 0);

bool launch_attention(const half_t * qkv, half_t * out, int nseq, int T_uniform, const int * seq_start, int max_len,
                      int h, int n_head, bool causal, hipStream_t stream);
int attention_whole_row_max_len(int d_head);
bool launch_attention_whole_row(const half_t * qkv, half_t * out, int nseq, int T_uniform, const int * seq_start, int max_len,
                                int h, int n_head, bool causal, hipStream_t stream);
bool launch_attention_long(const half_t * qkv, half_t * out, int nseq, int T_uniform, const int * seq_start, int max_len,
                           int h, int n_head, bool causal, hipStream_t stream);

bool launch_attention_f32(const float * qkv, float * out, int nseq, int T_uniform, const int * seq_start, int max_len,
                          int h, int n_head, bool causal, hipStream_t stream);

void launch_im2col(const void * imgs, bool imgs_f16, half_t * col, int B, int S, int P, int Kpad, hipStream_t stream);

void launch_gather_rows(const float * x, const half_t * a, const int * in_rows, int in_row_mul, int rows, int h, float * xp, half_t * ap, hipStream_t stream);

void launch_cls_rows(float * x, const float * class_embd, const float * pos, int B, int T, int h, hipStream_t stream);

void launch_meta_upload(const int * src_mapped, int * seq, int * last, int n_texts, unsigned * done_mapped, unsigned stamp, hipStream_t stream);
void launch_text_embed(const int32_t * ids, const int * seq_start, int nseq, int rows, const void * tok_raw,
                       int tok_type, const float * pos, int h, float * x, hipStream_t stream,
                       const float * gamma_next = nullptr, half_t * xg = nullptr, int ldxg = 0, float2 * stats = nullptr, float * mu_out = nullptr);

void launch_l2norm(const float * v, float * out, int rows, int n, bool normalize, hipStream_t stream);

struct PreImg {
    long long src_off;
    int nx, ny;
    int x0, y0;
    int ylo, nrows;
    long long hbuf_off;
    int th, tv;
    int stride;
    int reserved;
};
struct PreTaps { long long w_off; int first_off, count_off, ksize; };
void launch_preprocess(const uint8_t * raw, const PreImg * imgs, const PreTaps * taps, const double * wpool, const int * ipool, float * hbuf,
                       float * out, int n_imgs, int S, int max_rows, const float * mean, const float * stdv, hipStream_t stream);

void launch_jpeg_idct(const JpegPlaneDesc * planes_desc, int n_planes, int max_blocks, const int16_t * coef, uint8_t * planes, hipStream_t stream);
void launch_jpeg_rgb(const JpegPlaneDesc * planes_desc, const JpegImgDesc * imgs, int n_imgs, long long max_pixels, const uint8_t * planes, uint8_t * raw,
                     hipStream_t stream);

bool launch_zero_shot(const float * img, int B, const float * txt, int n, int dim, float * scores, int * indices, hipStream_t stream);

void launch_f32_to_f16(const float * src, int lds, half_t * dst, int ldd, int rows, int cols, int cols_pad,
                       hipStream_t stream);
void launch_f16_to_f32(const half_t * src, int lds, float * dst, int ldd, int rows, int cols, hipStream_t stream);

enum { SEARCH_F32 = 0, SEARCH_F16 = 1, SEARCH_I8 = 3 };
inline size_t search_elem_size(int dtype) { return dtype == SEARCH_I8 ? 1 : dtype == SEARCH_F16 ? 2 : 4; }
inline int search_dpad(int dtype, int dim) { return dtype == SEARCH_I8 ? (dim + 63) / 64 * 64 : (dim + 31) / 32 * 32; }
inline int64_t search_allow_words(int64_t n) { return (n + 63) / 64 * 2; }
int search_candidate_capacity(int k);
int search_sort_size(int k);
void launch_search_prepare(const float * src, int64_t n_src, int64_t n_rows, int dim, int Dpad, int dtype, void * dst, float * inv,
                           hipStream_t stream);
void launch_search_row_inv(const void * rows, int64_t n, int Dpad, float * inv, hipStream_t stream);
struct ScanArgs {
    const void * rows = nullptr;
    const float * rinv = nullptr;
    int64_t n = 0;
    int Dpad = 0, dtype = 0;
    const void * q = nullptr;
    const float * qinv = nullptr;
    int nq = 0, qt = 1, k = 0;
    void * cand = nullptr;
    int n_chunks = 0;
    int64_t rows_per_chunk = 0;
    const uint32_t * mask = nullptr;
    const int * qself = nullptr;
    const int * groups = nullptr;
    const int * qgroup = nullptr;
};
bool launch_search_scan(const ScanArgs & a, hipStream_t stream);
void launch_search_merge(const void * in, int64_t in_stride, int n_in, void * out, int nq, int k, hipStream_t stream);
void launch_search_finish(const void * in, int64_t in_stride, int nq, int k, float * dist, int64_t * ids, const int * qself, hipStream_t stream);
void launch_search_merge_grouped(const void * in, int64_t in_stride, int n_in, void * out, int nq, int k, const int * groups, hipStream_t stream);
void launch_sets_fill(float * dist, int64_t * ids, int * qrows, int64_t count, hipStream_t stream);
void launch_sets_qgroup(const int * groups, const int * qself, int * qgroup, int64_t n_rows, hipStream_t stream);
void launch_sets_fold(const void * lists, int64_t stride, int64_t q0, int m, const int64_t * lims, int64_t s_lo, int64_t n_fold, int k,
                      const int * groups, float * dist, int64_t * ids, int * qrows, int64_t qrow_base, hipStream_t stream);
void launch_search_gather(const void * rows, const float * rinv, const uint32_t * live, int64_t n, const int64_t * ids, int64_t first, int n_ids,
                          int64_t n_rows, int64_t row_bytes, void * q, float * qinv, int * qself, hipStream_t stream);
bool launch_graph(const void * rows, const float * rinv, int64_t n, int64_t q_first, int nq, int Dpad, int dtype, int k, void * cand, int n_chunks,
                  int64_t rows_per_chunk, const uint32_t * mask, hipStream_t stream);
bool launch_graph_cross(const void * rows, const float * rinv, int64_t n, const void * qrows, const float * qrinv, int64_t qn, int64_t q_first, int nq,
                        int Dpad, int dtype, int k, void * cand, int n_chunks, int64_t rows_per_chunk, const uint32_t * mask, hipStream_t stream);
void launch_search_fill_random(float * x, int64_t n, uint64_t seed, hipStream_t stream);
void launch_live_set(uint32_t * live, int64_t lo, int64_t hi, hipStream_t stream);
void launch_live_remove(uint32_t * live, const int64_t * ids, int64_t n, unsigned long long * removed, hipStream_t stream);
void launch_mask_and(const uint32_t * live, const uint32_t * allow, int64_t allow_words, uint32_t * out, int64_t words, hipStream_t stream);
void launch_compact_ids(const uint32_t * live, int64_t n, int64_t * new_ids, unsigned long long * total, hipStream_t stream);
void launch_compact_gather(const void * src, void * dst, const float * sinv, float * dinv, const int64_t * new_ids, int64_t n, int64_t row_bytes,
                           hipStream_t stream);
void launch_search_fill_allow(uint32_t * allow, int64_t n, float fraction, bool contiguous, uint64_t seed, hipStream_t stream);

constexpr int JOIN_HIT_BYTES = 12;
bool launch_join(const void * rows, const float * rinv, int64_t n, const void * q, const float * qinv, int64_t nq, int Dpad, int dtype, bool pairs,
                 float radius, int * count, unsigned long long * total, void * hits, int64_t hit_cap, const uint32_t * mask, hipStream_t stream);
void launch_join_scatter(const void * hits, int64_t total, const int64_t * offs, int * cursor, void * out, hipStream_t stream);
void * launch_join_sort(void * buf, void * tmp, const int64_t * offs, int64_t nseg, int64_t total, int64_t longest, hipStream_t stream);
void launch_join_finish(const void * in, int64_t total, float * dist, int64_t * ids, hipStream_t stream);
void launch_join_plant(float * x, int64_t rows, int dim, uint64_t seed, hipStream_t stream);

int distinct_near_words(int pool);
void launch_distinct_near(const void * rows, const float * rinv, int Dpad, int dtype, const int64_t * pool_ids, int nq, int pool, float radius,
                          uint32_t * near, hipStream_t stream);
void launch_distinct_pick(const float * pool_dist, const int64_t * pool_ids, const uint32_t * near, int nq, int pool, int k, float * dist,
                          int64_t * ids, int * counts, hipStream_t stream);
void launch_distinct_plant(float * x, int64_t rows, int dim, int64_t first_row, int copies, float amp, uint64_t seed, hipStream_t stream);

}
```

### clip_cpp_amd/csrc/load.cpp

```cpp
#include <cstdarg>
#include <cstdio>
#include <cstdlib>
#include <cstring>
#include <algorithm>
#include <memory>
#include <ctime>
#include <dirent.h>
#include <sys/stat.h>
#include <unistd.h>
#include <fcntl.h>
#include <cerrno>
#include <atomic>
#include <thread>
#include <functional>

#include "model.h"

namespace clipamd {

namespace {

struct RepackPlan {
    DevWeight W;
    size_t bytes_qs = 0, bytes_qh = 0, bytes_dm = 0, bytes_w16 = 0;
// ... 412 lines not shown
        ctx->max_token_len = 0;
        if (ctx->has_text_encoder) {
            auto & hp = ctx->text_hparams;
            bool ok = kv_u32(g, "clip.text.embedding_length", hp.hidden_size, kerr) & kv_u32(g, "clip.text.attention.head_count", hp.n_head, kerr) &
                      kv_u32(g, "clip.text.feed_forward_length", hp.n_intermediate, kerr) & kv_u32(g, "clip.text.block_count", hp.n_layer, kerr) &
                      kv_u32(g, "clip.text.context_length", hp.num_positions, kerr) & kv_u32(g, "clip.text.projection_dim", hp.projection_dim, kerr);
            if (!g.get_f32("clip.text.attention.layer_norm_epsilon", hp.eps)) { ok = false; if (kerr.empty()) kerr = "key clip.text.attention.layer_norm_epsilon not found in file"; }
            const GgufValue * toks = g.find("tokenizer.ggml.tokens");
            if (!toks || toks->type != GV_ARR || toks->elem_type != GV_STR) { ok = false; if (kerr.empty()) kerr = "key tokenizer.ggml.tokens not found in file"; }
            if (!ok) { why = kerr; return false; }
            hp.n_vocab = (int32_t)toks->strs.size();
            ctx->id_to_token = toks->strs;
            ctx->token_to_id.reserve(toks->strs.size() * 2);
            for (int32_t id = 0; id < hp.n_vocab; id++) {
                ctx->token_to_id[toks->strs[id]] = id;
                ctx->max_token_len = std::max(ctx->max_token_len, toks->strs[id].size());
            }
            if (hp.hidden_size <= 0 || hp.n_head <= 0 || hp.hidden_size % hp.n_head || hp.hidden_size % 64 || hp.n_intermediate % 64)
                { why = "unsupported text hparams (hidden/ff must be multiples of 64)"; return false; }
            { const std::string lim = kernel_limits("text", hp.hidden_size, hp.n_head, hp.projection_dim, hp.num_positions); if (!lim.empty()) { why = lim; return false; } }
            if (verbosity >= 2) {
                printf("\n%s: text model hparams\n", "clip_model_load");
                printf("n_vocab            %d\nnum_positions      %d\nt_hidden_size      %d\nt_n_intermediate   %d\n", hp.n_vocab, hp.num_positions, hp.hidden_size, hp.n_intermediate);
                printf("t_projection_dim   %d\nt_n_head           %d\nt_n_layer          %d\n", hp.projection_dim, hp.n_head, hp.n_layer);
            }
            DevTower & T = ctx->text;
            const int h = hp.hidden_size;
            if (!L.raw("t.token_embd.weight", &T.tok_raw, &T.tok_type, h, hp.n_vocab) ||
                !L.table_f32("t.position_embd.weight", &T.pos, h, hp.num_positions) ||
                !L.vec_f32({"t.post_ln.weight"}, &T.post_ln_w, h) || !L.vec_f32({"t.post_ln.bias"}, &T.post_ln_b, h) ||
                !L.linear({"text_projection.weight"}, T.proj, h, hp.projection_dim) ||
                !L.layers("t", hp.n_layer, h, hp.n_intermediate, T.layers))
                { why = L.err; return false; }
        }
        if (ctx->has_vision_encoder) {
            auto & hp = ctx->vision_hparams;
            bool ok = kv_u32(g, "clip.vision.embedding_length", hp.hidden_size, kerr) & kv_u32(g, "clip.vision.attention.head_count", hp.n_head, kerr) &
                      kv_u32(g, "clip.vision.feed_forward_length", hp.n_intermediate, kerr) & kv_u32(g, "clip.vision.block_count", hp.n_layer, kerr) &
                      kv_u32(g, "clip.vision.image_size", hp.image_size, kerr) & kv_u32(g, "clip.vision.patch_size", hp.patch_size, kerr) &
                      kv_u32(g, "clip.vision.projection_dim", hp.projection_dim, kerr);
            if (!g.get_f32("clip.vision.attention.layer_norm_epsilon", hp.eps)) { ok = false; if (kerr.empty()) kerr = "key clip.vision.attention.layer_norm_epsilon not found in file"; }
            const GgufValue * mean = g.find("clip.vision.image_mean");
            const GgufValue * stdv = g.find("clip.vision.image_std");
            if (!mean || !stdv || mean->type != GV_ARR || stdv->type != GV_ARR || mean->elem_type != GV_F32 || stdv->elem_type != GV_F32 ||
                mean->count < 3 || stdv->count < 3) { ok = false; if (kerr.empty()) kerr = "key clip.vision.image_mean/std not found in file"; }
            if (!ok) { why = kerr; return false; }
            memcpy(ctx->image_mean, mean->raw.data(), 12);
            memcpy(ctx->image_std, stdv->raw.data(), 12);
            if (hp.hidden_size <= 0 || hp.n_head <= 0 || hp.hidden_size % hp.n_head || hp.hidden_size % 64 || hp.n_intermediate % 64 ||
                hp.patch_size <= 0 || hp.image_size % hp.patch_size)
                { why = "unsupported vision hparams (hidden/ff must be multiples of 64)"; return false; }
            { const int g_ = hp.image_size / hp.patch_size; const std::string lim = kernel_limits("vision", hp.hidden_size, hp.n_head, hp.projection_dim, g_ * g_ + 1); if (!lim.empty()) { why = lim; return false; } }
            if (verbosity >= 2) {
                printf("\n%s: vision model hparams\n", "clip_model_load");
                printf("image_size         %d\npatch_size         %d\nv_hidden_size      %d\nv_n_intermediate   %d\n", hp.image_size, hp.patch_size, hp.hidden_size, hp.n_intermediate);
                printf("v_projection_dim   %d\nv_n_head           %d\nv_n_layer          %d\n", hp.projection_dim, hp.n_head, hp.n_layer);
            }
            DevTower & V = ctx->vision;
            const int h = hp.hidden_size, P = hp.patch_size, Gd = hp.image_size / P, T = Gd * Gd + 1;
            const GgufTensorInfo * pe = L.need("v.patch_embd.weight");
            if (!pe) { why = L.err; return false; }
            if (pe->type != GT_F16 && pe->type != GT_F32) { why = "v.patch_embd.weight must be f16"; return false; }
            if (!L.linear({"v.patch_embd.weight"}, V.patch, 3 * P * P, h, true) ||
                !L.vec_f32({"v.class_embd"}, &V.class_embd, h) ||
                !L.table_f32("v.position_embd.weight", &V.pos, h, T) ||
                !L.vec_f32({"v.pre_ln.weight"}, &V.pre_ln_w, h) || !L.vec_f32({"v.pre_ln.bias"}, &V.pre_ln_b, h) ||
                !L.vec_f32({"v.post_ln.weight"}, &V.post_ln_w, h) || !L.vec_f32({"v.post_ln.bias"}, &V.post_ln_b, h) ||
                !L.linear({"visual_projection.weight"}, V.proj, h, hp.projection_dim) ||
                !L.layers("v", hp.n_layer, h, hp.n_intermediate, V.layers))
                { why = L.err; return false; }
        }
        return true;
    };
    for (int attempt = 0; attempt < 2; attempt++) {
        Lp.reset(new Loader(g));
        Lp->st.plan_only = cache.readable;
        std::string why;
        if (!build(*Lp, why)) return fail(why);
        {
            uint64_t ph = 1469598103934665603ull;
            for (const Fix & f : Lp->fixes) ph = WeightCache::fnv(ph, &f.off, sizeof f.off);
            const uint64_t tot = Lp->st.size;
            ph = WeightCache::fnv(ph, &tot, 8);
            cache.plan_hash = (uint32_t)(ph ^ (ph >> 32));
        }
        if (!Lp->st.plan_only) break;
        if (cache.image_bytes == Lp->st.size && cache.file_plan_hash == cache.plan_hash) break;
        cache.readable = false;
    }
    Loader & L = *Lp;
    if (verbosity >= 1) {
        printf("%s: text_encoder:   %d\n", "clip_model_load", ctx->has_text_encoder);
        printf("%s: vision_encoder: %d\n", "clip_model_load", ctx->has_vision_encoder);
        printf("%s: model size:     %.2f MB (HBM image, repacked)\n", "clip_model_load", L.st.size / 1024.0 / 1024.0);
    }

    int ndev = 0;
    if (hipGetDeviceCount(&ndev) != hipSuccess) ndev = 0;
    if (ndev <= 0) {
        (void)hipGetLastError();
        const char * allow = getenv("CLIP_AMD_ALLOW_NO_DEVICE");
        if (allow && allow[0] == '1') {
            if (verbosity >= 1) fprintf(stderr, "clip_model_load: no HIP device — host-only context (tokenizer / preprocessing only; encoders will fail)\n");
            ctx->device = -1;
            if (L.st.plan_only) ctx->weights_from_cache = true;
            else cache.write_image(L.st.buf);
            return ctx;
        }
        return fail("no HIP device available: this library has no CPU fallback (set CLIP_AMD_ALLOW_NO_DEVICE=1 for a host-only context)");
    }
    if (device < 0 || device >= ndev) return fail("invalid HIP device ordinal " + std::to_string(device));
    if (hipSetDevice(device) != hipSuccess) return fail("hipSetDevice failed");
    ctx->device = device;
    { const char * g = getenv("CLIP_AMD_GRAPHS"); if (g && g[0] == '0') ctx->graphs_enabled = false; }
    if (!alloc_runtime_buffers(ctx)) return fail("stream / split-K workspace / LayerNorm statistics allocation failed");
    {
        int lo = 0, hi = 0, ways = 2;
        const char * e = getenv("CLIP_AMD_SPLIT");
        if (e && sscanf(e, "%d,%d,%d", &lo, &hi, &ways) >= 2) { ctx->split_min = lo; ctx->split_max = hi; ctx->split_ways = ways < 2 ? 2 : ways > 4 ? 4 : ways; }
    }
    ctx->weights_bytes = L.st.size + 256;
    if (hipMalloc(&ctx->weights_base, ctx->weights_bytes) != hipSuccess) return fail("hipMalloc of the weight image failed");
    if (L.st.plan_only) {
        if (!cache.read_image(L.st.buf, L.st.size)) {
            Lp.reset(new Loader(g));
            std::string why;
            if (!build(*Lp, why)) return fail(why);
        } else {
            ctx->weights_from_cache = true;
        }
    }
    Loader & LL = *Lp;
    if (hipMemcpy(ctx->weights_base, LL.st.buf.data(), LL.st.size, hipMemcpyHostToDevice) != hipSuccess) return fail("weight upload failed");
    if (!ctx->weights_from_cache) cache.write_image(LL.st.buf);
    for (const Fix & f : LL.fixes) *f.slot = (const uint8_t *)ctx->weights_base + f.off;
    {
        bool f32_weights = false;
        for (DevTower * tw : {&ctx->vision, &ctx->text})
            for (DevLayer & l : tw->layers) {
                if (l.qkv.wtype == W_F32 || l.o.wtype == W_F32 || l.ff1.wtype == W_F32 || l.ff2.wtype == W_F32) { f32_weights = true; continue; }
                launch_fold_vectors(l.qkv, l.ln1_w, l.ln1_b, l.qkv_b, (float *)l.qkv_c, (float *)l.qkv_bf, ctx->stream);
                launch_fold_vectors(l.ff1, l.ln2_w, l.ln2_b, l.ff1_b, (float *)l.ff1_c, (float *)l.ff1_bf, ctx->stream);
            }
        if (hipStreamSynchronize(ctx->stream) != hipSuccess || hipGetLastError() != hipSuccess) return fail("LayerNorm fold vectors: kernel failed");
        const char * e = getenv("CLIP_AMD_LNFOLD");
        ctx->ln_fold = !(e && e[0] == '0') && !f32_weights;
        ctx->ln_fold_force = e && e[0] == '2';
        const char * e2 = getenv("CLIP_AMD_RESIDENT_PANELS");
        ctx->resident_panels_on = !(e2 && e2[0] == '0');
        const char * ef = getenv("CLIP_AMD_F32_ACTS");
        ctx->f32_acts = !(ef && ef[0] == '0');
        const char * ep = getenv("CLIP_AMD_PRUNE_LAST");
        ctx->prune_last = !(ep && ep[0] == '0');
        const char * ec = getenv("CLIP_AMD_LNFOLD_CENTRE");
        ctx->ln_fold_centre = !(ec && ec[0] == '0');
    }
    if (verbosity >= 1) printf("\n%s: %zu MB of HBM allocated for weights on device %d\n", "clip_model_load", ctx->weights_bytes / 1024 / 1024, device);
    return ctx;
}

namespace {
bool alloc_runtime_buffers(clip_ctx * ctx) {
    if (hipStreamCreateWithFlags(&ctx->own_stream, hipStreamNonBlocking) != hipSuccess) return false;
    ctx->stream = ctx->own_stream;
    const size_t nfl = (size_t)16 << 20;
    void * w = nullptr, * c = nullptr;
    if (hipMalloc(&w, nfl * sizeof(float)) != hipSuccess || hipMalloc(&c, 4096 * sizeof(unsigned)) != hipSuccess || hipMemset(c, 0, 4096 * sizeof(unsigned)) != hipSuccess) return false;
    ctx->sk_ws = (float *)w; ctx->sk_ws_floats = nfl; ctx->sk_cnt = (unsigned *)c; ctx->sk_cnt_n = 4096;
    return hipMalloc((void **)&ctx->sk_stats, (size_t)2 * SKINNY_MAX_ROWS * 128 * sizeof(float2)) == hipSuccess;
}
}

clip_ctx * sibling_context(clip_ctx * owner, int index) {
    if (!owner || owner->device < 0 || owner->weights_borrowed || index < 0 || index > 2) return nullptr;
    clip_ctx *& slot = index == 0 ? owner->sibling : owner->more_siblings[index - 1];
    if (slot) return slot;
    (void)hipSetDevice(owner->device);
    clip_ctx * c = new clip_ctx();
    c->has_text_encoder = owner->has_text_encoder; c->has_vision_encoder = owner->has_vision_encoder; c->use_gelu = owner->use_gelu; c->ftype = owner->ftype;
    c->text_hparams = owner->text_hparams; c->vision_hparams = owner->vision_hparams;
    memcpy(c->image_mean, owner->image_mean, sizeof c->image_mean); memcpy(c->image_std, owner->image_std, sizeof c->image_std);
    c->device = owner->device;
    c->vision = owner->vision; c->text = owner->text;
    c->weights_borrowed = true;
    c->owner = owner;
    c->ln_fold = owner->ln_fold; c->ln_fold_force = owner->ln_fold_force; c->ln_fold_centre = owner->ln_fold_centre; c->prune_last = owner->prune_last;
    c->f32_acts = owner->f32_acts;
    c->resident_panels_on = owner->resident_panels_on;
    c->graphs_enabled = false;
    c->split_min = c->split_max = 0;
    c->verbosity = 0; c->path = owner->path;
    hipEvent_t & evj = index == 0 ? owner->ev_join : owner->ev_join_more[index - 1];
    if (!alloc_runtime_buffers(c) || (!owner->ev_fork && hipEventCreateWithFlags(&owner->ev_fork, hipEventDisableTiming) != hipSuccess) ||
        hipEventCreateWithFlags(&evj, hipEventDisableTiming) != hipSuccess) {
        (void)hipGetLastError();
        fprintf(stderr, "clip (hip): cannot create the sibling context\n");
        free_model(c);
        return nullptr;
    }
    slot = c;
    return c;
}

void free_model(clip_ctx * ctx) {
    if (!ctx) return;
    if (ctx->multi) multi_free(ctx);
    if (ctx->sibling) { free_model(ctx->sibling); ctx->sibling = nullptr; }
    for (clip_ctx *& ms : ctx->more_siblings) if (ms) { free_model(ms); ms = nullptr; }
    if (ctx->device >= 0) {
        (void)hipSetDevice(ctx->device);
        if (ctx->own_stream) (void)hipStreamSynchronize(ctx->own_stream);
        if (ctx->stream && ctx->stream != ctx->own_stream) (void)hipStreamSynchronize(ctx->stream);
        free_host_pipe(ctx);
        for (int i = 0; i < MetaRing::SLOTS; i++) {
            if (ctx->meta.pin[i]) (void)hipHostFree(ctx->meta.pin[i]);
            if (ctx->meta.ev[i]) (void)hipEventDestroy(ctx->meta.ev[i]);
        }
        if (ctx->meta.done) (void)hipHostFree((void *)ctx->meta.done);
        if (ctx->ev_stream_switch) (void)hipEventDestroy(ctx->ev_stream_switch);
        if (ctx->ev_fork) (void)hipEventDestroy(ctx->ev_fork);
        if (ctx->ev_join) (void)hipEventDestroy(ctx->ev_join);
        for (hipEvent_t e : ctx->ev_join_more) if (e) (void)hipEventDestroy(e);
        for (auto & p : ctx->pending) { (void)hipEventDestroy(p.a); (void)hipEventDestroy(p.b); }
        drop_graphs(ctx);
        if (ctx->ws.base) (void)hipFree(ctx->ws.base);
        if (ctx->weights_base && !ctx->weights_borrowed) (void)hipFree(ctx->weights_base);
        if (ctx->pinned) (void)hipHostFree(ctx->pinned);
        if (ctx->io_in) (void)hipFree(ctx->io_in);
        if (ctx->io_out) (void)hipFree(ctx->io_out);
        if (ctx->pre_buf) (void)hipFree(ctx->pre_buf);
        free_preprocess_slots(ctx);
        if (ctx->w16_panel) (void)hipFree(ctx->w16_panel);
        for (auto * b : ctx->res_panel_buf) if (b) (void)hipFree(b);
        if (ctx->sk_stats) (void)hipFree(ctx->sk_stats);
        if (ctx->sk_ws) (void)hipFree(ctx->sk_ws);
        if (ctx->sk_cnt) (void)hipFree(ctx->sk_cnt);
        if (ctx->own_stream) (void)hipStreamDestroy(ctx->own_stream);
    }
    delete ctx;
}

bool repack_for_test(int type, const void * w_raw, int64_t N, int64_t K, DevWeight & W, void ** dev_base) {
    RepackPlan pl;
    std::string err;
    if (!plan_repack(type, N, K, pl, err)) { fprintf(stderr, "repack_for_test: %s\n", err.c_str()); return false; }
    auto up = [](size_t b) { return (b + 255) & ~(size_t)255; };
    const size_t o_w16 = 0, o_qs = up(pl.bytes_w16), o_qh = o_qs + up(pl.bytes_qs), o_dm = o_qh + up(pl.bytes_qh);
    const size_t total = o_dm + up(pl.bytes_dm) + 256;
    std::vector<uint8_t> host(total, 0);
    repack_rows(pl, type, (const uint8_t *)w_raw, N, K, 0, &host[o_qs], &host[o_qh], &host[o_dm], &host[o_w16]);
    void * base = nullptr;
    if (hipMalloc(&base, total) != hipSuccess) return false;
    if (hipMemcpy(base, host.data(), total, hipMemcpyHostToDevice) != hipSuccess) { (void)hipFree(base); return false; }
    W = pl.W;
    const uint8_t * b = (const uint8_t *)base;
    if (pl.bytes_w16) W.w16 = b + o_w16;
    if (pl.bytes_qs) W.qs = b + o_qs;
    if (pl.bytes_qh) W.qh = b + o_qh;
    if (pl.bytes_dm) W.dm = b + o_dm;
    *dev_base = base;
    return true;
}

}
```

### clip_cpp_amd/csrc/model.h

```cpp
#pragma once

#include <functional>
#include <map>
#include <string>
#include <unordered_map>
#include <vector>

#include "../../include/clip.h"
#include "gguf.h"
#include "kernels.h"

namespace clipamd {

struct DevLayer {
    DevWeight qkv, o, ff1, ff2;
    const float *qkv_b = nullptr, *o_b = nullptr, *ff1_b = nullptr, *ff2_b = nullptr;
    const float *ln1_w = nullptr, *ln1_b = nullptr, *ln2_w = nullptr, *ln2_b = nullptr;
    const float *qkv_c = nullptr, *qkv_bf = nullptr, *ff1_c = nullptr, *ff1_bf = nullptr;
};

struct DevTower {
    std::vector<DevLayer> layers;
    const float * pos = nullptr;
    const float *post_ln_w = nullptr, *post_ln_b = nullptr;
    DevWeight proj;
    DevWeight patch;
    const float * class_embd = nullptr;
    const float *pre_ln_w = nullptr, *pre_ln_b = nullptr;
    const void * tok_raw = nullptr;
    int tok_type = 0;
};

struct ProfEntry {
    double ms = 0;
    int64_t launches = 0;
    double flops = 0;
    double bytes = 0;
};

struct Workspace {
    void * base = nullptr;
    size_t bytes = 0;
};

struct HostPipe {
    hipStream_t copy_stream = nullptr;
    void * pin_in[2] = {nullptr, nullptr};
    size_t pin_in_bytes[2] = {0, 0};
    void * dev_in[2] = {nullptr, nullptr};
    size_t dev_in_bytes[2] = {0, 0};
    hipEvent_t ev_copied[2] = {nullptr, nullptr};
    hipEvent_t ev_consumed[2] = {nullptr, nullptr};
    hipEvent_t ev_sub = nullptr;
    bool used[2] = {false, false};
    struct PackPool * pool = nullptr;
};

struct MetaRing {
    static constexpr int SLOTS = 8;
    int * pin[SLOTS] = {nullptr};
    int * dev[SLOTS] = {nullptr};
    size_t cap[SLOTS] = {0};
    hipEvent_t ev[SLOTS] = {nullptr};
    bool busy[SLOTS] = {false};
    int next = 0;
    volatile unsigned * done = nullptr;
    unsigned * done_dev = nullptr;
    unsigned expect[SLOTS] = {0};
    unsigned stamp = 0;
};

}

struct clip_ctx {
    bool has_text_encoder = false;
    bool has_vision_encoder = false;
    bool use_gelu = false;
    int32_t ftype = 1;
    clip_text_hparams text_hparams{};
    clip_vision_hparams vision_hparams{};
    float image_mean[3] = {0, 0, 0};
    float image_std[3] = {1, 1, 1};

    std::vector<std::string> id_to_token;
    std::unordered_map<std::string, int32_t> token_to_id;
    size_t max_token_len = 0;

    int device = -1;
    hipStream_t own_stream = nullptr;
    hipStream_t stream = nullptr;
    void * weights_base = nullptr;
    size_t weights_bytes = 0;
    bool weights_from_cache = false;
    clipamd::DevTower vision, text;
    clipamd::Workspace ws;
    std::vector<size_t> guard_gaps;
    void * pinned = nullptr;
    size_t pinned_bytes = 0;
    void * io_in = nullptr;
    size_t io_in_bytes = 0;
    void * io_out = nullptr;
    size_t io_out_bytes = 0;
    bool input_f16 = false;
    clipamd::HostPipe pipe;
    clipamd::MetaRing meta;
    void * multi = nullptr;
    clip_ctx * sibling = nullptr;
    clip_ctx * more_siblings[2] = {nullptr, nullptr};
    hipEvent_t ev_join_more[2] = {nullptr, nullptr};
    int split_ways = 2;
    bool weights_borrowed = false;
    clip_ctx * owner = nullptr;
    bool last_launch_split = false;
    bool f32_acts = true;
    bool device_shared = false;
    bool sibling_busy = false;
    hipEvent_t ev_fork = nullptr, ev_join = nullptr;
    int split_min = -1, split_max = -1;
    hipEvent_t ev_stream_switch = nullptr;
    void * pre_buf = nullptr;
    size_t pre_bytes = 0;
    struct PreSlot { void * pin = nullptr; size_t pin_bytes = 0; void * dev = nullptr; size_t dev_bytes = 0; hipEvent_t ev_h2d = nullptr, ev_done = nullptr; bool used = false; };
    static constexpr int PRE_SLOTS = 4;
    PreSlot pre_slot[PRE_SLOTS];
    hipStream_t pre_copy_stream = nullptr;
    float * sk_ws = nullptr;
    size_t sk_ws_floats = 0;
    unsigned * sk_cnt = nullptr;
    int sk_cnt_n = 0;
    float2 * sk_stats = nullptr;
    bool ln_fold_force = false;
    bool prune_last = true;
    bool ln_fold_centre = true;
    bool ln_fold = true;
    clipamd::half_t * w16_panel = nullptr;
    size_t w16_panel_halfs = 0;
    clipamd::half_t * res_panel_buf[2] = {nullptr, nullptr};
    std::vector<const clipamd::half_t *> res_panels[2];
    unsigned res_panel_mask[2] = {0, 0};
    bool resident_panels_on = true;

    bool profiling = false;
    struct PendingEvent { hipEvent_t a, b; std::string tag; double flops, bytes; };
    std::vector<PendingEvent> pending;
    std::map<std::string, clipamd::ProfEntry> prof;

    struct GraphEntry { int B; const void * in; void * out; bool norm; bool in_f16; int seen; hipGraph_t graph; hipGraphExec_t exec; bool split; bool busy_seen; };
    std::vector<GraphEntry> vgraphs;
    struct TextGraphEntry { int n_texts, rows, nt; const void * ids; void * out; bool norm; int seen; hipGraph_t graph; hipGraphExec_t exec; };
    std::vector<TextGraphEntry> tgraphs;
    bool graphs_enabled = true;

    int verbosity = 0;
    std::string path;
};

namespace clipamd {

struct RelaxCapture {
    hipStreamCaptureMode prev = hipStreamCaptureModeRelaxed;
    bool armed = false;
    RelaxCapture() {
        static const bool off = [] { const char * e = getenv("CLIP_AMD_NO_RELAX_CAPTURE"); return e && e[0] == '1'; }();
        if (off) return;
        armed = hipThreadExchangeStreamCaptureMode(&prev) == hipSuccess;
        if (!armed) (void)hipGetLastError();
    }
    ~RelaxCapture() { if (armed) (void)hipThreadExchangeStreamCaptureMode(&prev); }
    RelaxCapture(const RelaxCapture &) = delete;
    RelaxCapture & operator=(const RelaxCapture &) = delete;
};

clip_ctx * load_model(const char * fname, int verbosity, int device);
clip_ctx * sibling_context(clip_ctx * owner, int index = 0);
void free_model(clip_ctx * ctx);
bool repack_for_test(int type, const void * w_raw, int64_t N, int64_t K, DevWeight & W, void ** dev_base);

bool vision_forward_device(clip_ctx * ctx, const float * d_imgs, int B, float * d_out, bool normalize);
bool text_forward_device(clip_ctx * ctx, const int32_t * d_ids, const int32_t * h_offsets, int n_texts, float * d_out,
                         bool normalize);
struct TowerBufs {
    int st_stride = 0;
    float2 * stats = nullptr;
    float * mu = nullptr;
    float * x = nullptr, * emb = nullptr;
    half_t * xn = nullptr, * qkv = nullptr, * att = nullptr, * mid = nullptr, * pooled = nullptr;
    float * xp = nullptr;
    half_t * ap = nullptr, * xnp = nullptr, * midp = nullptr;
};
struct VisionStage {
    TowerBufs b;
    int Bc = 0;
    half_t * col = nullptr;
};
bool vision_stage_begin(clip_ctx * ctx, int Bc, VisionStage & st);
bool vision_stage_patch(clip_ctx * ctx, const VisionStage & st, const void * imgs, int i0, int n);
bool vision_stage_finish(clip_ctx * ctx, const VisionStage & st, float * d_out, bool normalize);
int vision_max_chunk(const clip_ctx * ctx);
bool ensure_workspace(clip_ctx * ctx, size_t bytes);
bool ensure_pinned(clip_ctx * ctx, size_t bytes);
bool ensure_io(clip_ctx * ctx, size_t in_bytes, size_t out_bytes);
void prof_collect(clip_ctx * ctx);
void drop_graphs(clip_ctx * ctx);
bool renew_streams_after_failed_capture(clip_ctx * ctx);

bool encode_images_from_host(clip_ctx * ctx, const clip_image_f32 * imgs, int n, float * d_out, bool normalize, int n_threads);
void free_host_pipe(clip_ctx * ctx);
void multi_shard(int total, int n_dev, int g, int * lo, int * hi, int * per_dev);
clip_ctx * multi_load(const char * fname, int verbosity, int n_devices);
void multi_free(clip_ctx * primary);
int multi_device_count(const clip_ctx * primary);
bool multi_image_batch_encode(clip_ctx * primary, const clip_image_f32 * imgs, int B, float * vec, bool normalize, int n_threads);
bool multi_run(clip_ctx * primary, int total, int proj, float * vec, const char * who,
               const std::function<bool(int, clip_ctx *, int, int, float *)> & run);
bool multi_run_pair(clip_ctx * primary, int n_img, int n_txt, int proj, float * vec_img, float * vec_txt, const char * who,
                    const std::function<bool(int, clip_ctx *, int, int, float *)> & run_img,
                    const std::function<bool(int, clip_ctx *, int, int, float *)> & run_txt);
clip_ctx * multi_replica(const clip_ctx * primary, int g);
const float * multi_gathered(const clip_ctx * primary, int g);

bool tokenize_text(const clip_ctx * ctx, const char * text, std::vector<int32_t> & out);
bool preprocess_image(const clip_ctx * ctx, const clip_image_u8 * img, clip_image_f32 * res);
bool preprocess_batch_device(clip_ctx * ctx, const clip_image_u8 * imgs, int n, float * d_out, int slot = -1);
void free_preprocess_slots(clip_ctx * ctx);
bool load_image_file(const char * fname, clip_image_u8 * img);
bool read_image_file(const char * fname, std::vector<uint8_t> & out);
struct JpegCoefImage;
bool decode_image_bytes(const std::vector<uint8_t> & d, std::vector<uint8_t> & rgb, int & nx, int & ny, std::string & err, JpegCoefImage * staged,
                        bool * is_staged);
struct PreSrc {
    int nx = 0, ny = 0; const uint8_t * rgb = nullptr; const JpegCoefImage * jpeg = nullptr;
    int bx = 0, by = 0, bw = 0, bh = 0;
    int src_id = -1;
    int out_nx() const { return bw ? bw : nx; }
    int out_ny() const { return bw ? bh : ny; }
};
bool preprocess_sources_device(clip_ctx * ctx, const PreSrc * src, int n, float * d_out, int slot = -1);
long long jpeg_device_images();
bool encode_sources_to_device(clip_ctx * ctx, const PreSrc * src, int n, float * d_out, bool normalize);
int encode_encoded_images(clip_ctx * ctx, const char * const * paths, const uint8_t * const * data, const size_t * sizes, int n, int max_images,
                          int n_threads, bool normalize, float * vec, int * consumed, uint8_t * ok, const char * who, int grid = 0,
                          int32_t * boxes_out = nullptr);

void dequantize_row(int type, const void * src, float * dst, int64_t k);
size_t quantize_rows(int type, const float * src, void * dst, int64_t nrows, int64_t k);
uint16_t f32_to_f16_bits(float x);
float f16_bits_to_f32(uint16_t h);

}
```

### include/clip_amd.h

```cpp
#ifndef CLIP_AMD_H
#define CLIP_AMD_H

#include "clip.h"

#ifdef __cplusplus
extern "C" {
#endif

int clip_amd_device_count(void);

struct clip_ctx * clip_amd_model_load(const char * fname, int verbosity, int device);

struct clip_ctx * clip_amd_model_load_multi(const char * fname, int verbosity, int n_devices);
int clip_amd_ctx_device_count(const struct clip_ctx * ctx);

int clip_amd_weights_from_cache(const struct clip_ctx * ctx);
void clip_amd_shard_bounds(int total, int n_devices, int device_index, int * lo, int * hi, int * rows_per_device);
const float * clip_amd_gathered_embeddings(const struct clip_ctx * ctx, int device_index);

bool clip_amd_image_batch_encode_device_multi(struct clip_ctx * ctx, const float * const * d_imgs, int total, bool normalize, float * vec);
bool clip_amd_text_batch_encode_device_multi(struct clip_ctx * ctx, const int32_t * const * d_ids, const int32_t * h_offsets, int total, bool normalize,
                                             float * vec);
bool clip_amd_encode_pair_device_multi(struct clip_ctx * ctx, const float * const * d_imgs, int n_images, const int32_t * const * d_ids,
                                       const int32_t * h_offsets, int n_texts, bool normalize, float * vec_img, float * vec_txt);

int clip_amd_ctx_device(const struct clip_ctx * ctx);

void clip_amd_set_stream(struct clip_ctx * ctx, void * hip_stream);

void clip_amd_set_device_shared(struct clip_ctx * ctx, int shared);

bool clip_amd_image_batch_encode_device(struct clip_ctx * ctx, const float * d_imgs, int batch, float * d_out,
                                        bool normalize);

bool clip_amd_image_batch_preprocess_device(struct clip_ctx * ctx, const struct clip_image_u8 * imgs, int n, float * d_out);

bool clip_amd_image_batch_encode_u8(struct clip_ctx * ctx, const struct clip_image_u8 * imgs, int n, float * vec, bool normalize);

int clip_amd_image_batch_encode_files(struct clip_ctx * ctx, const char * const * paths, int n, int max_images, int n_threads,
                                      bool normalize, float * vec, int * consumed, uint8_t * ok);
int clip_amd_image_batch_encode_memory(struct clip_ctx * ctx, const uint8_t * const * data, const size_t * sizes, int n, int max_images,
                                       int n_threads, bool normalize, float * vec, int * consumed, uint8_t * ok);

bool clip_amd_image_batch_encode_regions(struct clip_ctx * ctx, const struct clip_image_u8 * imgs, int n_imgs, const int32_t * boxes, int n_boxes,
                                         float * vec, bool normalize);
bool clip_amd_image_batch_preprocess_regions_device(struct clip_ctx * ctx, const struct clip_image_u8 * imgs, int n_imgs, const int32_t * boxes,
                                                    int n_boxes, float * d_out);
int clip_amd_image_batch_encode_files_grid(struct clip_ctx * ctx, const char * const * paths, int n, int max_images, int n_threads, int grid,
                                           bool normalize, float * vec, int32_t * boxes_out, int * consumed, uint8_t * ok);
int clip_amd_image_batch_encode_memory_grid(struct clip_ctx * ctx, const uint8_t * const * data, const size_t * sizes, int n, int max_images,
                                            int n_threads, int grid, bool normalize, float * vec, int32_t * boxes_out, int * consumed, uint8_t * ok);

bool clip_text_batch_encode(const struct clip_ctx * ctx, const int n_threads, const struct clip_tokens * tokens,
                            size_t n_texts, float * vec, const bool normalize);

bool clip_amd_text_batch_encode_device(struct clip_ctx * ctx, const int32_t * d_ids, const int32_t * h_offsets,
                                       int n_texts, float * d_out, bool normalize);

bool clip_amd_zero_shot_score_device(struct clip_ctx * ctx, const float * d_img, int n_images, const float * d_txt, int n_labels, int dim,
                                     float * d_scores, int * d_indices);

bool clip_amd_zero_shot_label_images(struct clip_ctx * ctx, const struct clip_image_u8 * imgs, int n_images, const char ** labels,
                                     size_t n_labels, float * scores, int * indices);

void clip_amd_synchronize(struct clip_ctx * ctx);

void clip_amd_profile_enable(struct clip_ctx * ctx, bool on);
int clip_amd_profile_read(struct clip_ctx * ctx, float * ms, int64_t * launches, int cap, bool reset);
int clip_amd_profile_report(struct clip_ctx * ctx, char * buf, int cap, bool reset);

struct clip_amd_index;
struct clip_amd_index * clip_amd_index_create(struct clip_ctx * ctx, int dim, int dtype);
bool clip_amd_index_add(struct clip_amd_index * ix, const float * vecs, int64_t n);
bool clip_amd_index_add_device(struct clip_amd_index * ix, const float * d_vecs, int64_t n);
int64_t clip_amd_index_size(const struct clip_amd_index * ix);
int clip_amd_index_dim(const struct clip_amd_index * ix);
bool clip_amd_index_search(struct clip_amd_index * ix, const float * queries, int n_queries, int k, float * distances, int64_t * ids);
bool clip_amd_index_search_device(struct clip_amd_index * ix, const float * d_queries, int n_queries, int k, float * d_distances,
                                  int64_t * d_ids);
bool clip_amd_index_save(struct clip_amd_index * ix, const char * path);
struct clip_amd_index * clip_amd_index_load(struct clip_ctx * ctx, const char * path);
void clip_amd_index_free(struct clip_amd_index * ix);
int64_t clip_amd_index_remove(struct clip_amd_index * ix, const int64_t * ids, int64_t n);
int64_t clip_amd_index_live(const struct clip_amd_index * ix);
bool clip_amd_index_live_mask(struct clip_amd_index * ix, uint64_t * bits);
int64_t clip_amd_index_compact(struct clip_amd_index * ix, int64_t * new_ids);
bool clip_amd_index_search_subset(struct clip_amd_index * ix, const float * queries, int n_queries, int k, const uint64_t * allow,
                                  float * distances, int64_t * ids);
bool clip_amd_index_search_subset_device(struct clip_amd_index * ix, const float * d_queries, int n_queries, int k, const uint64_t * d_allow,
                                         float * d_distances, int64_t * d_ids);
bool clip_amd_index_search_grouped(struct clip_amd_index * ix, const float * queries, int n_queries, int k, const int32_t * groups,
                                   const uint64_t * allow, float * distances, int64_t * ids);
bool clip_amd_index_search_grouped_device(struct clip_amd_index * ix, const float * d_queries, int n_queries, int k, const int32_t * d_groups,
                                          const uint64_t * d_allow, float * d_distances, int64_t * d_ids);
float clip_amd_bench_search(int dtype, int64_t n, int dim, int n_queries, int k, int iters);
float clip_amd_bench_search_grouped(int dtype, int64_t n, int dim, int n_queries, int k, int group_size, int iters);
bool clip_amd_index_search_sets(struct clip_amd_index * ix, const float * queries, int n_queries, const int64_t * set_lims, int64_t n_sets, int k,
                                const int32_t * groups, const uint64_t * allow, float * distances, int64_t * ids, int32_t * qrows);
bool clip_amd_index_search_sets_device(struct clip_amd_index * ix, const float * d_queries, int n_queries, const int64_t * set_lims, int64_t n_sets,
                                       int k, const int32_t * d_groups, const uint64_t * d_allow, float * d_distances, int64_t * d_ids,
                                       int32_t * d_qrows);
bool clip_amd_index_search_ids_sets(struct clip_amd_index * ix, const int64_t * ids, int64_t n_ids, const int64_t * set_lims, int64_t n_sets, int k,
                                    int exclude_own, const int32_t * groups, const uint64_t * allow, float * distances, int64_t * out_ids,
                                    int32_t * qrows);
int64_t clip_amd_test_index_sets_block(struct clip_amd_index * ix, int64_t rows);
float clip_amd_bench_search_sets(int dtype, int64_t n, int dim, int n_sets, int set_size, int k, int group_size, int iters);
bool clip_amd_index_search_distinct(struct clip_amd_index * ix, const float * queries, int n_queries, int k, float radius, int pool,
                                    const uint64_t * allow, float * distances, int64_t * ids, int32_t * counts);
bool clip_amd_index_search_distinct_device(struct clip_amd_index * ix, const float * d_queries, int n_queries, int k, float radius, int pool,
                                           const uint64_t * d_allow, float * d_distances, int64_t * d_ids, int32_t * d_counts);
bool clip_amd_index_search_ids_distinct(struct clip_amd_index * ix, const int64_t * ids, int n_ids, int k, float radius, int pool, int exclude_self,
                                        const uint64_t * allow, float * distances, int64_t * out_ids, int32_t * counts);
int clip_amd_test_index_distinct_block(struct clip_amd_index * ix, int queries);
float clip_amd_bench_search_distinct(int dtype, int64_t n, int dim, int n_queries, int k, int pool, float radius, int copies, int iters);
float clip_amd_bench_search_subset(int dtype, int64_t n, int dim, int n_queries, int k, float allowed_fraction, int contiguous, int iters);
bool clip_amd_index_search_ids(struct clip_amd_index * ix, const int64_t * ids, int n_ids, int k, int exclude_self, const uint64_t * allow,
                               float * distances, int64_t * out_ids);
bool clip_amd_index_search_ids_device(struct clip_amd_index * ix, const int64_t * d_ids, int n_ids, int k, int exclude_self,
                                      const uint64_t * d_allow, float * d_distances, int64_t * d_out_ids);
bool clip_amd_index_knn_graph(struct clip_amd_index * ix, int k, float * distances, int64_t * ids);
int clip_amd_test_index_knn_route(struct clip_amd_index * ix, int route);
float clip_amd_bench_knn(int dtype, int64_t n, int dim, int k, int route, int iters);
bool clip_amd_index_search_index(struct clip_amd_index * ix, struct clip_amd_index * src, const int64_t * ids, int64_t n_ids, int k,
                                 const uint64_t * allow, float * distances, int64_t * out_ids);
int64_t clip_amd_index_append(struct clip_amd_index * ix, struct clip_amd_index * src, int64_t * new_ids);
int clip_amd_test_index_cross_route(struct clip_amd_index * ix, int route);
float clip_amd_bench_cross(int dtype, int64_t n_rows, int64_t n_queries, int dim, int k, int route, int iters);
int64_t clip_amd_index_range_search(struct clip_amd_index * ix, const float * queries, int n_queries, float radius,
                                    int64_t * lims, float * distances, int64_t * ids, int64_t capacity);
int64_t clip_amd_index_pairs(struct clip_amd_index * ix, float radius, int64_t * lims, float * distances, int64_t * ids, int64_t capacity);
int64_t clip_amd_index_range_search_subset(struct clip_amd_index * ix, const float * queries, int n_queries, float radius, const uint64_t * allow,
                                           int64_t * lims, float * distances, int64_t * ids, int64_t capacity);
float clip_amd_bench_range(int dtype, int64_t n, int dim, int n_queries, float radius, int iters);

int clip_amd_test_gemm(int type, const void * w_raw, int64_t N, int64_t K, const float * x, int64_t M,
                       const float * bias, const float * resid, float * y, int epilogue, int tile);
int clip_amd_test_gemm_ex(int type, const void * w_raw, int64_t N, int64_t K, const float * x, int64_t M,
                          const float * bias, const float * resid, float * y, int epilogue, int tile,
                          int qcols, float qscale, int Np, int T, const float * pos);
int clip_amd_test_lnfold(int type, const void * w1_raw, int64_t h, int64_t K1, const void * w2_raw, int64_t N2, const float * a, int64_t M,
                         const float * b1, const float * resid, const float * gamma, const float * beta, float eps, const float * b2,
                         int epi2, int tile1, int tile2, int fold, int qcols, float qscale, float * x1_out, float * y_out);
int clip_amd_test_gemm_tile(int64_t M, int64_t N, int64_t K, int quantised);
int clip_amd_test_gemm_tile_ex(int64_t M, int64_t N, int64_t K, int quantised, int shared_device);
float clip_amd_bench_gemm(int type, int64_t N, int64_t K, int64_t M, int epilogue, int tile, int iters);
int clip_amd_test_skinny(int type, const void * w_raw, int64_t N, int64_t K, const float * x, int64_t M, const float * bias,
                         const float * resid, const float * ln_w, const float * ln_b, float eps, float * y, int epilogue,
                         int qcols, float qscale, float * stats_out);
int clip_amd_test_layernorm(const float * x, const float * w, const float * b, float eps, int64_t rows, int64_t h,
                            float * y, int out_f16);
int clip_amd_test_layernorm_ex(const float * x, int64_t x_rows, int ldx, const int32_t * in_rows, int in_row_mul, const float * w, const float * b,
                               float eps, int rows, int h, uint16_t * out16, int ld16, float * out32, int ld32);
int clip_amd_test_text_embed(int type, const void * tok_raw, int64_t tok_bytes, int h, const int32_t * ids, const int32_t * seq_start, int nseq, int rows,
                             const float * pos, int n_pos, const float * gamma_next, int centred, float * x, uint16_t * xg, int ldxg, float * stats,
                             float * mu);
int clip_amd_test_im2col(const float * imgs, int imgs_f16, int B, int S, int P, int Kpad, uint16_t * col);
int clip_amd_test_layernorm_prep(const float * x, int ldx, const float * w, const float * b, float eps, int rows, int h, const float * gamma_next,
                                 int centred, const float * class_embd, const float * pos0, int T, int in_place, float * out32, int ld32,
                                 uint16_t * xg, int ldxg, float * stats, float * mu);
int clip_amd_test_rows(int op, const void * in0, const void * in1, const int32_t * idx, int64_t n0, int64_t n1, int64_t n2, int64_t n3, int64_t n4,
                       void * out0, void * out1);
int clip_amd_test_jpeg_plan(const uint8_t * data, size_t size, int * info);
long long clip_amd_test_jpeg_device_count(void);
int clip_amd_test_jpeg_decode_device(const uint8_t * data, size_t size, uint8_t * rgb, size_t cap, int * nx, int * ny);
int clip_amd_bench_jpeg_kernels(const uint8_t * data, size_t size, int copies, int reps, float * ms, double * bytes);
int clip_amd_test_attention(const float * qkv, int nseq, int T, int h, int n_head, int causal, float * out);
int clip_amd_test_attention_ex(const float * qkv, int nseq, int T, int h, int n_head, int causal, float * out, int kernel);
float clip_amd_bench_attention(int nseq, int T, int h, int n_head, int causal, int kernel, int iters);

#ifdef __cplusplus
}
#endif

#endif
```

Baseline: 122,200.

## Fuse pooled last-layer tail into four GEMM kernels with in-epilogue LayerNorm stats

Adds a dedicated tail kernel family for the pruned last layer: out-proj with residual, FFN-up with LayerNorm folded in from partial row stats, FFN-down with residual, and the final projection with post-LN and normalisation. The residual GEMMs write per-column-block partial statistics so the later kernels can normalise without separate layernorm launches. The aim is to remove the separate layernorm, pooling and projection launches on the small pooled-row path. It is enabled by default behind an environment flag, and it adds a stats buffer plus new kernel instantiations for each weight type.

Measured after the change: 122,200, median of 2. Within noise of the previous version (+0.0%).

```diff
diff --git a/clip_cpp_amd/__init__.py b/clip_cpp_amd/__init__.py
--- a/clip_cpp_amd/__init__.py
+++ b/clip_cpp_amd/__init__.py
@@ -56,7 +56,7 @@
     "clip_amd_image_batch_preprocess_device", "clip_amd_image_batch_encode_u8",
     "clip_amd_zero_shot_score_device", "clip_amd_zero_shot_label_images",
     "clip_amd_synchronize", "clip_amd_profile_enable", "clip_amd_profile_read", "clip_amd_profile_report",
-    "clip_amd_test_gemm", "clip_amd_test_gemm_ex", "clip_amd_test_gemm_tile", "clip_amd_test_gemm_tile_ex", "clip_amd_test_skinny", "clip_amd_test_layernorm", "clip_amd_test_attention", "clip_amd_bench_gemm",
+    "clip_amd_test_gemm", "clip_amd_test_gemm_ex", "clip_amd_test_gemm_tile", "clip_amd_test_gemm_tile_ex", "clip_amd_test_skinny", "clip_amd_test_tail", "clip_amd_test_layernorm", "clip_amd_test_attention", "clip_amd_bench_gemm",
     "clip_amd_test_attention_ex", "clip_amd_bench_attention",
     "clip_amd_test_layernorm_ex", "clip_amd_test_text_embed", "clip_amd_test_im2col", "clip_amd_test_layernorm_prep", "clip_amd_test_rows",
     "clip_amd_index_create", "clip_amd_index_add", "clip_amd_index_add_device", "clip_amd_index_size", "clip_amd_index_dim",
@@ -184,6 +184,9 @@
     L.clip_amd_test_gemm_tile_ex.argtypes = [C.c_int64, C.c_int64, C.c_int64, i32, i32]
     L.clip_amd_test_skinny.restype = i32
     L.clip_amd_test_skinny.argtypes = [i32, vp, C.c_int64, C.c_int64, f32p, C.c_int64, f32p, f32p, f32p, f32p, C.c_float, f32p, i32, i32, C.c_float, f32p]
+    L.clip_amd_test_tail.restype = i32
+    L.clip_amd_test_tail.argtypes = [i32, i32, vp, C.c_int64, C.c_int64, f32p, C.c_int64, C.POINTER(C.c_int32), i32, C.c_int64, f32p, f32p, f32p, f32p, C.c_float, f32p,
+                                     i32, i32, i32, f32p, f32p]
     L.clip_amd_bench_gemm.restype = C.c_float
     L.clip_amd_bench_gemm.argtypes = [i32, C.c_int64, C.c_int64, C.c_int64, i32, i32, i32]
     L.clip_amd_test_layernorm.restype = i32
diff --git a/clip_cpp_amd/build.py b/clip_cpp_amd/build.py
--- a/clip_cpp_amd/build.py
+++ b/clip_cpp_amd/build.py
@@ -13,7 +13,7 @@
 
 HOST_SOURCES = ["gguf.cpp", "quant.cpp", "load.cpp", "forward.cpp", "tokenizer.cpp", "preprocess.cpp", "image_io.cpp", "image_formats.cpp",
                 "jpeg_decode.cpp", "host_pipeline.cpp", "files_pipeline.cpp", "api.cpp", "search.cpp"]
-HIP_SOURCES = ["k_attn.hip", "k_attn_long.hip", "k_attn_f32.hip", "k_misc.hip", "k_preproc.hip", "k_jpeg.hip", "k_gemm.hip", "k_gemm8.hip", "k_gemm4.hip", "k_gemm32.hip", "k_gemm_f32.hip", "k_skinny.hip", "k_gemm_ring.hip", "k_fold.hip", "k_search.hip", "k_join.hip", "k_graph.hip", "k_group.hip", "k_sets.hip", "k_distinct.hip"]
+HIP_SOURCES = ["k_attn.hip", "k_attn_long.hip", "k_attn_f32.hip", "k_misc.hip", "k_preproc.hip", "k_jpeg.hip", "k_gemm.hip", "k_gemm8.hip", "k_gemm4.hip", "k_gemm32.hip", "k_gemm_f32.hip", "k_skinny.hip", "k_tail.hip", "k_gemm_ring.hip", "k_fold.hip", "k_search.hip", "k_join.hip", "k_graph.hip", "k_group.hip", "k_sets.hip", "k_distinct.hip"]
 GEMM_WTYPES = [0, 1, 2, 3, 4, 5]
 EXTRA_FLAGS = {"k_attn_f32.hip": ["-fno-slp-vectorize"], "k_attn_long.hip": ["-fno-slp-vectorize"], "k_gemm_f32.hip": ["-fno-slp-vectorize"]}
 
@@ -73,6 +73,12 @@
         objs.append(o)
         if force or _newer(o, [s] + headers):
             jobs.append([cc, "--offload-arch=" + ARCH] + COMMON + ["-DCLIPAMD_SKINNY_WT=%d" % wt, "-c", s, "-o", o])
+    s = os.path.join(CSRC, "k_tail.hip")
+    for wt in GEMM_WTYPES:
+        o = os.path.join(BUILD, "k_tail_wt%d.o" % wt)
+        objs.append(o)
+        if force or _newer(o, [s] + headers):
+            jobs.append([cc, "--offload-arch=" + ARCH] + COMMON + ["-DCLIPAMD_TAIL_WT=%d" % wt, "-c", s, "-o", o])
     s = os.path.join(CSRC, "k_gemm_ring.hip")
     for wt in GEMM_WTYPES:
         o = os.path.join(BUILD, "k_gemm_ring_wt%d.o" % wt)
diff --git a/clip_cpp_amd/csrc/api.cpp b/clip_cpp_amd/csrc/api.cpp
--- a/clip_cpp_amd/csrc/api.cpp
+++ b/clip_cpp_amd/csrc/api.cpp
@@ -1071,6 +1071,70 @@
     return rc;
 }
 
+int clip_amd_test_tail(int op, int type, const void * w_raw, int64_t N, int64_t K, const float * a, int64_t a_rows, const int32_t * idx, int in_row_mul, int64_t M,
+                       const float * bias, const float * resid, const float * ln_w, const float * ln_b, float eps, const float * stats_in, int slots, int act,
+                       int normalize, float * y, float * stats_out) {
+    int ndev = 0;
+    if (hipGetDeviceCount(&ndev) != hipSuccess || ndev <= 0) { (void)hipGetLastError(); return -1; }
+    if (op < 1 || op > 4 || !w_raw || !a || !y || N <= 0 || K <= 0 || M <= 0 || a_rows <= 0) return -3;
+    const bool res = op == 1 || op == 3;
+    if (res) {
+        if (!resid || (op == 3 && (idx || in_row_mul != 1 || a_rows != M))) return -3;
+        if (idx) { for (int64_t r = 0; r < M; r++) if (idx[r] < 0 || idx[r] >= a_rows) return -3; }
+        else if (in_row_mul < 0 || (M - 1) * in_row_mul >= a_rows) return -3;
+    } else if (!ln_w || !ln_b || !stats_in || slots <= 0 || slots > TAIL_STATS_CAP || a_rows != M || (op == 2 && act != 2 && act != 3)) return -3;
+    DevWeight W;
+    void * wbase = nullptr;
+    if (!repack_for_test(type, w_raw, N, K, W, &wbase)) return -2;
+    const size_t rows_out = (size_t)M + 2, ldc = (size_t)N + 4, n_out = rows_out * ldc, n_st = rows_out * TAIL_STATS_CAP * 2;
+    DBuf da32((size_t)a_rows * K * 4), da16((size_t)a_rows * K * 2), dres((size_t)a_rows * N * 4), didx((size_t)M * 4), dbias((size_t)N * 4), dlw((size_t)K * 4), dlb((size_t)K * 4),
+        dsi((size_t)M * TAIL_STATS_CAP * 8), dout32(n_out * 4), dout16(n_out * 2), dso(n_st * 4);
+    (void)hipMemcpy(da32.p, a, (size_t)a_rows * K * 4, hipMemcpyHostToDevice);
+    if (bias) (void)hipMemcpy(dbias.p, bias, (size_t)N * 4, hipMemcpyHostToDevice);
+    if (idx) (void)hipMemcpy(didx.p, idx, (size_t)M * 4, hipMemcpyHostToDevice);
+    (void)hipMemsetD32((hipDeviceptr_t)dout32.p, 0x7fc00000, n_out);
+    (void)hipMemsetD16((hipDeviceptr_t)dout16.p, 0x7e00, n_out);
+    (void)hipMemsetD32((hipDeviceptr_t)dso.p, 0x7fc00000, n_st);
+    TailParams p;
+    p.M = (int)M; p.W = W; p.bias = bias ? (const float *)dbias.p : nullptr; p.ldc = (int)ldc; p.eps = eps; p.normalize = normalize != 0;
+    int epi = EPI_RESID_F32;
+    if (res) {
+        launch_f32_to_f16((const float *)da32.p, (int)K, (half_t *)da16.p, (int)K, (int)a_rows, (int)K, (int)K, nullptr);
+        p.A16 = (const half_t *)da16.p; p.lda = (int)K; p.in_rows = idx ? (const int *)didx.p : nullptr; p.in_row_mul = in_row_mul;
+        p.out = dout32.p; p.stats_out = (float2 *)dso.p;
+        if (op == 3) {
+            (void)hipMemcpy2D(dout32.p, ldc * 4, resid, (size_t)N * 4, (size_t)N * 4, (size_t)M, hipMemcpyHostToDevice);
+            p.resid = (const float *)dout32.p; p.ldr = (int)ldc;
+        } else {
+            (void)hipMemcpy(dres.p, resid, (size_t)a_rows * N * 4, hipMemcpyHostToDevice);
+            p.resid = (const float *)dres.p; p.ldr = (int)N;
+        }
+    } else {
+        (void)hipMemcpy(dlw.p, ln_w, (size_t)K * 4, hipMemcpyHostToDevice);
+        (void)hipMemcpy(dlb.p, ln_b, (size_t)K * 4, hipMemcpyHostToDevice);
+        (void)hipMemsetD32((hipDeviceptr_t)dsi.p, 0x7fc00000, (size_t)M * TAIL_STATS_CAP * 2);
+        (void)hipMemcpy2D(dsi.p, (size_t)TAIL_STATS_CAP * 8, stats_in, (size_t)slots * 8, (size_t)slots * 8, (size_t)M, hipMemcpyHostToDevice);
+        p.x32 = (const float *)da32.p; p.ldx = (int)K; p.ln_w = (const float *)dlw.p; p.ln_b = (const float *)dlb.p;
+        p.stats_in = (const float2 *)dsi.p; p.stats_slots = slots;
+        if (op == 2) { epi = act == 2 ? EPI_GELU_F16 : EPI_QGELU_F16; p.out = dout16.p; }
+        else p.out = dout32.p;
+    }
+    int rc = 0;
+    if (op == 4 ? !tail_proj_supported(p) : !tail_supported(p, epi)) rc = -5;
+    else {
+        if (op == 4) launch_tail_proj(p, nullptr);
+        else launch_tail(p, epi, nullptr);
+        if (op == 2) launch_f16_to_f32((const half_t *)dout16.p, (int)ldc, (float *)dout32.p, (int)ldc, (int)rows_out, (int)ldc, nullptr);
+        if (hipDeviceSynchronize() != hipSuccess || hipGetLastError() != hipSuccess) rc = -4;
+        else {
+            (void)hipMemcpy(y, dout32.p, n_out * 4, hipMemcpyDeviceToHost);
+            if (stats_out && res) (void)hipMemcpy(stats_out, dso.p, n_st * 4, hipMemcpyDeviceToHost);
+        }
+    }
+    (void)hipFree(wbase);
+    return rc;
+}
+
 static bool test_device() {
     int ndev = 0;
     if (hipGetDeviceCount(&ndev) != hipSuccess || ndev <= 0) { (void)hipGetLastError(); return false; }
diff --git a/clip_cpp_amd/csrc/forward.cpp b/clip_cpp_amd/csrc/forward.cpp
--- a/clip_cpp_amd/csrc/forward.cpp
+++ b/clip_cpp_amd/csrc/forward.cpp
@@ -297,10 +297,26 @@
     bool skinny = false;
     bool fold = false;
     bool prune = false;
+    bool tail4 = false;
     bool f32 = false;
     float * mu = nullptr;
     const half_t * const * resp = nullptr;
 };
+
+bool tail_fits(const TowerPass & P) {
+    const DevTower & tw = *P.tw;
+    if (tw.layers.empty() || !P.b.tst) return false;
+    const DevLayer & l = tw.layers.back();
+    TailParams a, u, d, j;
+    const half_t * h16 = P.b.att;
+    a.M = u.M = d.M = j.M = P.nseq;
+    a.W = l.o; a.A16 = h16; a.lda = P.h; a.resid = P.b.x; a.ldr = P.h; a.out = P.b.xp; a.ldc = P.h; a.stats_out = P.b.tst; a.in_row_mul = P.in_row_mul;
+    u.W = l.ff1; u.x32 = P.b.xp; u.ldx = P.h; u.ln_w = l.ln2_w; u.ln_b = l.ln2_b; u.stats_in = P.b.tst; u.stats_slots = (P.h + TAIL_RESID_COLS - 1) / TAIL_RESID_COLS; u.out = P.b.midp; u.ldc = P.ff;
+    d.W = l.ff2; d.A16 = h16; d.lda = P.ff; d.resid = P.b.xp; d.ldr = P.h; d.out = P.b.xp; d.ldc = P.h; d.stats_out = P.b.tst;
+    j.W = tw.proj; j.x32 = P.b.xp; j.ldx = P.h; j.ln_w = tw.post_ln_w; j.ln_b = tw.post_ln_b; j.stats_in = P.b.tst; j.stats_slots = u.stats_slots; j.out = P.b.emb; j.ldc = P.proj;
+    return l.o.N == P.h && l.o.K == P.h && l.ff1.K == P.h && l.ff1.N == P.ff && l.ff2.K == P.ff && l.ff2.N == P.h && tw.proj.K == P.h && tw.proj.N == P.proj &&
+           tail_supported(a, EPI_RESID_F32) && tail_supported(u, EPI_GELU_F16) && tail_supported(d, EPI_RESID_F32) && tail_proj_supported(j);
+}
 
 void choose_form(const clip_ctx * ctx, TowerPass & P) {
     const DevTower & tw = *P.tw;
@@ -309,6 +325,7 @@
     P.prune = ctx->prune_last && !P.skinny && !tw.layers.empty() && P.rows > P.nseq;
     P.f32 = acts_f32(ctx, tw);
     P.mu = ctx->ln_fold_centre ? P.b.mu : nullptr;
+    P.tail4 = P.prune && ctx->pooled_tail4 && !P.f32 && tail_fits(P);
 }
 
 struct LnState {
@@ -428,6 +445,46 @@
     resid_linear(ctx, T, ln, {"gemm_ffn_down_pooled", "", l.ff2, l.ff2_b, nullptr}, T.b.mid, nullptr);
 }
 
+void tail_launch(clip_ctx * ctx, const char * what, const TailParams & p, int epi) {
+    if (!ctx->profiling) { launch_tail(p, epi, ctx->stream); return; }
+    int mf, nf, nw;
+    tail_shape(p, epi, mf, nf, nw);
+    char fam[96];
+    snprintf(fam, sizeof fam, "gemm_tail_kernel<%d,%d,%d,%d,%d>/%s", p.W.wtype, mf, nf, nw, epi, what);
+    const double fl = 2.0 * p.M * (double)p.W.N * p.W.K;
+    const double by = weight_bytes(p.W) + (double)p.M * p.W.K * (p.x32 ? 4 : 2) + (double)p.M * p.W.N * (epi == EPI_RESID_F32 ? 8 : 2);
+    ProfScope ps(ctx, fam, p.M, p.W.N, p.W.K, fl, by);
+    launch_tail(p, epi, ctx->stream);
+}
+
+void fused_tail(clip_ctx * ctx, const TowerPass & P, float * d_out, bool normalize) {
+    const DevTower & tw = *P.tw;
+    const DevLayer & l = tw.layers.back();
+    const TowerBufs & B = P.b;
+    const int n = P.nseq, h = P.h;
+    float2 * st1 = B.tst, * st2 = B.tst + (size_t)n * TAIL_STATS_CAP;
+    const int slots = (h + TAIL_RESID_COLS - 1) / TAIL_RESID_COLS;
+    TailParams a;
+    a.M = n; a.W = l.o; a.bias = l.o_b; a.A16 = B.att; a.lda = h; a.in_rows = P.in_rows; a.in_row_mul = P.in_row_mul;
+    a.resid = B.x; a.ldr = h; a.out = B.xp; a.ldc = h; a.stats_out = st1;
+    tail_launch(ctx, "gemm_out_pooled", a, EPI_RESID_F32);
+    TailParams u;
+    u.M = n; u.W = l.ff1; u.bias = l.ff1_b; u.x32 = B.xp; u.ldx = h; u.ln_w = l.ln2_w; u.ln_b = l.ln2_b; u.eps = P.eps; u.stats_in = st1; u.stats_slots = slots;
+    u.out = B.midp; u.ldc = P.ff;
+    tail_launch(ctx, "gemm_ffn_up_pooled", u, ctx->use_gelu ? EPI_GELU_F16 : EPI_QGELU_F16);
+    TailParams d;
+    d.M = n; d.W = l.ff2; d.bias = l.ff2_b; d.A16 = B.midp; d.lda = P.ff; d.resid = B.xp; d.ldr = h; d.out = B.xp; d.ldc = h; d.stats_out = st2;
+    tail_launch(ctx, "gemm_ffn_down_pooled", d, EPI_RESID_F32);
+    TailParams j;
+    j.M = n; j.W = tw.proj; j.x32 = B.xp; j.ldx = h; j.ln_w = tw.post_ln_w; j.ln_b = tw.post_ln_b; j.eps = P.eps; j.stats_in = st2; j.stats_slots = slots;
+    j.out = d_out; j.ldc = P.proj; j.normalize = normalize;
+    if (!ctx->profiling) { launch_tail_proj(j, ctx->stream); return; }
+    char fam[96];
+    snprintf(fam, sizeof fam, "gemm_tail_proj_kernel<%d,%d>/gemm_proj", j.W.wtype, tail_proj_nfw(j));
+    ProfScope ps(ctx, fam, n, P.proj, h, 2.0 * n * (double)P.proj * h, weight_bytes(j.W) + (double)n * h * 4 + (double)n * P.proj * 4);
+    launch_tail_proj(j, ctx->stream);
+}
+
 bool check_device(clip_ctx * ctx, const char * who) {
     if (!ctx || ctx->device < 0) {
         fprintf(stderr, "%s: no HIP device bound to this context — the encoders have no CPU fallback\n", who);
@@ -465,6 +522,7 @@
     b.ap = c.take<half_t>(aw * n * h);
     b.xnp = c.take<half_t>(aw * n * h);
     b.midp = c.take<half_t>(aw * n * ff);
+    b.tst = c.take<float2>((size_t)2 * n * TAIL_STATS_CAP);
 }
 
 template <typename F> bool carve_workspace(clip_ctx * ctx, F carve) {
@@ -483,6 +541,10 @@
     if (P.skinny && !P.fold) launch_row_stats(B.x, P.h, P.rows, P.h, ctx->sk_stats, s);
     P.resp = P.skinny ? nullptr : resident_panels(ctx, tw, P.which, P.rows);
     if (!run_layers(ctx, P)) return false;
+    if (P.tail4) {
+        fused_tail(ctx, P, d_out, normalize);
+        return true;
+    }
     if (P.prune) {
         pooled_tail(ctx, P);
         layernorm_act(P.f32, B.xp, P.h, nullptr, 1, tw.post_ln_w, tw.post_ln_b, P.eps, P.nseq, P.h, B.pooled, s);
diff --git a/clip_cpp_amd/csrc/gemm_common.h b/clip_cpp_amd/csrc/gemm_common.h
--- a/clip_cpp_amd/csrc/gemm_common.h
+++ b/clip_cpp_amd/csrc/gemm_common.h
@@ -149,6 +149,12 @@
 #endif
 }
 
+__device__ __forceinline__ h8 normalise8(const f4 lo, const f4 hi, float mean, float rstd, const f4 g0, const f4 g1, const f4 b0, const f4 b1) {
+    const f4 y0 = ((lo - mean) * rstd) * g0 + b0;
+    const f4 y1 = ((hi - mean) * rstd) * g1 + b1;
+    return (h8){(_Float16)y0[0], (_Float16)y0[1], (_Float16)y0[2], (_Float16)y0[3], (_Float16)y1[0], (_Float16)y1[1], (_Float16)y1[2], (_Float16)y1[3]};
+}
+
 __device__ __forceinline__ void ln_pair32(float s0, float q0, float s1, float q1, float & mean, float & m2) {
     const float m0 = s0 * (1.0f / 32.0f), m1 = s1 * (1.0f / 32.0f);
     const float d = m1 - m0;
diff --git a/clip_cpp_amd/csrc/k_skinny.hip b/clip_cpp_amd/csrc/k_skinny.hip
--- a/clip_cpp_amd/csrc/k_skinny.hip
+++ b/clip_cpp_amd/csrc/k_skinny.hip
@@ -4,12 +4,6 @@
 namespace clipamd {
 
 namespace {
-
-__device__ __forceinline__ h8 normalise8(const f4 lo, const f4 hi, float mean, float rstd, const f4 g0, const f4 g1, const f4 b0, const f4 b1) {
-    const f4 y0 = ((lo - mean) * rstd) * g0 + b0;
-    const f4 y1 = ((hi - mean) * rstd) * g1 + b1;
-    return (h8){(_Float16)y0[0], (_Float16)y0[1], (_Float16)y0[2], (_Float16)y0[3], (_Float16)y1[0], (_Float16)y1[1], (_Float16)y1[2], (_Float16)y1[3]};
-}
 
 template <int WT, int MF, int NW, int EPI, bool LNA>
 __global__ void __launch_bounds__(NW * 64) skinny_kernel(const SkinnyParams p) {
diff --git a/clip_cpp_amd/csrc/k_tail.hip b/clip_cpp_amd/csrc/k_tail.hip
--- /dev/null
+++ b/clip_cpp_amd/csrc/k_tail.hip
@@ -0,0 +1,417 @@
+
+#include "gemm_common.h"
+
+namespace clipamd {
+
+namespace {
+
+template <int WT> struct TailW { WFrag<WT> q; h8 h; };
+
+template <int WT>
+__device__ __forceinline__ void tail_load_w(TailW<WT> & w, const DevWeight & W, int n, int kb, int fgrp) {
+    if constexpr (WT == W_F16) {
+        w.h = *(const h8 *)((const half_t *)W.w16 + (size_t)n * W.Kpad + kb * 32 + fgrp * 8);
+    } else {
+        const size_t idx = (size_t)kb * W.Npad + n;
+        if constexpr (WT == W_Q8_0) {
+            const uint2 q = ((const uint2 *)W.qs)[idx * 4 + fgrp];
+            w.q.q = q.x;
+            w.q.q1 = q.y;
+        } else {
+            w.q.q = ((const uint32_t *)W.qs)[idx * 4 + fgrp];
+        }
+        if constexpr (WT == W_Q5_0 || WT == W_Q5_1) w.q.h = ((const uint32_t *)W.qh)[idx];
+        if constexpr (WT == W_Q4_1 || WT == W_Q5_1) w.q.dm = ((const h2 *)W.dm)[idx];
+        else w.q.d = ((const half_t *)W.dm)[idx];
+    }
+}
+template <int WT>
+__device__ __forceinline__ h8 tail_wfrag(const TailW<WT> & w, int fgrp) {
+    if constexpr (WT == W_F16) return w.h;
+    else return dequant_wfrag<WT>(w.q, fgrp);
+}
+
+template <int WT, int MF, int NF, int NW, int EPI>
+__global__ void __launch_bounds__(NW * 64) gemm_tail_kernel(const TailParams p) {
+    constexpr bool LNA = EPI != EPI_RESID_F32;
+    constexpr int CH = LNA ? 2 : 3;
+    constexpr int NFR = MF * NF, FPW = (NFR + NW - 1) / NW;
+    __shared__ f4 red[NW * NFR * 64];
+    __shared__ float2 lnst[LNA ? MF * 16 : 1];
+    __shared__ __align__(16) float lng[LNA ? TAIL_LN_KMAX : 4], lnb[LNA ? TAIL_LN_KMAX : 4];
+    __shared__ float2 rowst[LNA ? 1 : MF * 16 * NF];
+
+    const int tid = threadIdx.x;
+    const int lane = tid & 63;
+    const int wave = __builtin_amdgcn_readfirstlane(tid >> 6);
+    const int frow = lane & 15, fgrp = lane >> 4;
+    const int N = p.W.N;
+    const int n0 = blockIdx.x * (NF * 16);
+    const int m_base = blockIdx.y * (MF * 16);
+    const int nkb = p.W.Kpad / 32;
+    const int kb_lo = wave * nkb / NW, kb_hi = (wave + 1) * nkb / NW;
+
+    auto src_row = [&](int m) -> size_t {
+        const int mc = m < p.M ? m : p.M - 1;
+        if constexpr (LNA) return (size_t)mc;
+        else return p.in_rows ? (size_t)p.in_rows[mc] : (size_t)mc * (size_t)p.in_row_mul;
+    };
+    size_t arow[MF];
+#pragma unroll
+    for (int b = 0; b < MF; b++) arow[b] = src_row(m_base + b * 16 + frow);
+
+    struct XReg { h8 h; f4 lo, hi; };
+    auto load_x = [&](XReg & x, int kb, int b) {
+        if constexpr (LNA) {
+            const float * src = p.x32 + arow[b] * p.ldx + kb * 32 + fgrp * 8;
+            x.lo = *(const f4 *)src;
+            x.hi = *(const f4 *)(src + 4);
+        } else {
+            x.h = *(const h8 *)(p.A16 + arow[b] * p.lda + kb * 32 + fgrp * 8);
+        }
+    };
+    TailW<WT> wA[CH][NF], wB[CH][NF];
+    XReg xA[CH][MF], xB[CH][MF];
+#define TL_LOAD(W_, X_, c_)                                                                                       \
+    _Pragma("unroll") for (int i = 0; i < CH; i++)                                                                \
+        if ((c_) + i < kb_hi) {                                                                                   \
+            _Pragma("unroll") for (int a = 0; a < NF; a++) tail_load_w<WT>(W_[i][a], p.W, n0 + a * 16 + frow, (c_) + i, fgrp); \
+            _Pragma("unroll") for (int b = 0; b < MF; b++) load_x(X_[i][b], (c_) + i, b);                        \
+        }
+    TL_LOAD(wA, xA, kb_lo);
+
+    f4 bias_pre[FPW], resid_pre[FPW];
+#pragma unroll
+    for (int j = 0; j < FPW; j++) {
+        bias_pre[j] = (f4){0.f, 0.f, 0.f, 0.f};
+        resid_pre[j] = (f4){0.f, 0.f, 0.f, 0.f};
+        const int f = wave + j * NW;
+        if (f < NFR) {
+            const int n = n0 + (f % NF) * 16 + fgrp * 4, m = m_base + (f / NF) * 16 + frow;
+            if (p.bias && n < N) bias_pre[j] = *(const f4 *)(p.bias + n);
+            if constexpr (!LNA) {
+                if (m < p.M && n < N) resid_pre[j] = *(const f4 *)(p.resid + src_row(m) * p.ldr + n);
+            }
+        }
+    }
+
+    float mean[MF], rstd[MF];
+    if constexpr (LNA) {
+        for (int k4 = tid; k4 < p.W.K / 4; k4 += NW * 64) {
+            *(f4 *)(lng + 4 * k4) = *(const f4 *)(p.ln_w + 4 * k4);
+            *(f4 *)(lnb + 4 * k4) = *(const f4 *)(p.ln_b + 4 * k4);
+        }
+        {
+            constexpr int TPR = (NW * 64) / (MF * 16);
+            const int r = tid / TPR, sub = tid % TPR;
+            const int gr = m_base + r;
+            const float2 * row = p.stats_in + (size_t)(gr < p.M ? gr : p.M - 1) * TAIL_STATS_CAP;
+            float s1 = 0.f, s2 = 0.f;
+            for (int base = 0; base < p.stats_slots; base += TPR * 16) {
+                float2 v[16];
+#pragma unroll
+                for (int i = 0; i < 16; i++) {
+                    const int sl = base + i * TPR + sub;
+                    v[i] = sl < p.stats_slots ? row[sl] : make_float2(0.f, 0.f);
+                }
+#pragma unroll
+                for (int i = 0; i < 16; i++) { s1 += v[i].x; s2 += v[i].y; }
+            }
+#pragma unroll
+            for (int o = TPR / 2; o > 0; o >>= 1) { s1 += __shfl_xor(s1, o); s2 += __shfl_xor(s2, o); }
+            if (sub == 0) {
+                const float mu = s1 / (float)p.W.K;
+                float var = s2 / (float)p.W.K - mu * mu;
+                var = var > 0.f ? var : 0.f;
+                lnst[r] = make_float2(mu, 1.0f / sqrtf(var + p.eps));
+            }
+        }
+        __syncthreads();
+#pragma unroll
+        for (int b = 0; b < MF; b++) { const float2 st = lnst[b * 16 + frow]; mean[b] = st.x; rstd[b] = st.y; }
+    }
+
+    f4 acc[MF][NF];
+#pragma unroll
+    for (int b = 0; b < MF; b++)
+#pragma unroll
+        for (int a = 0; a < NF; a++) acc[b][a] = (f4){0.f, 0.f, 0.f, 0.f};
+#define TL_COMPUTE(W_, X_, c_)                                                                                    \
+    _Pragma("unroll") for (int i = 0; i < CH; i++)                                                                \
+        if ((c_) + i < kb_hi) {                                                                                   \
+            h8 wf[NF];                                                                                            \
+            _Pragma("unroll") for (int a = 0; a < NF; a++) wf[a] = tail_wfrag<WT>(W_[i][a], fgrp);                \
+            f4 g0, g1, b0, b1;                                                                                    \
+            if constexpr (LNA) {                                                                                  \
+                const int k0 = ((c_) + i) * 32 + fgrp * 8;                                                        \
+                g0 = *(const f4 *)(lng + k0); g1 = *(const f4 *)(lng + k0 + 4);                                   \
+                b0 = *(const f4 *)(lnb + k0); b1 = *(const f4 *)(lnb + k0 + 4);                                   \
+            }                                                                                                     \
+            _Pragma("unroll") for (int b = 0; b < MF; b++) {                                                      \
+                h8 xf;                                                                                            \
+                if constexpr (LNA) xf = normalise8(X_[i][b].lo, X_[i][b].hi, mean[b], rstd[b], g0, g1, b0, b1);   \
+                else xf = X_[i][b].h;                                                                             \
+                _Pragma("unroll") for (int a = 0; a < NF; a++)                                                    \
+                    acc[b][a] = __builtin_amdgcn_mfma_f32_16x16x32_f16(wf[a], xf, acc[b][a], 0, 0, 0);            \
+            }                                                                                                     \
+        }
+    for (int c = kb_lo; c < kb_hi; c += 2 * CH) {
+        TL_LOAD(wB, xB, c + CH);
+        TL_COMPUTE(wA, xA, c);
+        TL_LOAD(wA, xA, c + 2 * CH);
+        TL_COMPUTE(wB, xB, c + CH);
+    }
+#undef TL_LOAD
+#undef TL_COMPUTE
+
+#pragma unroll
+    for (int b = 0; b < MF; b++)
+#pragma unroll
+        for (int a = 0; a < NF; a++) red[(wave * NFR + b * NF + a) * 64 + lane] = acc[b][a];
+    __syncthreads();
+#pragma unroll
+    for (int j = 0; j < FPW; j++) {
+        const int f = wave + j * NW;
+        if (f >= NFR) continue;
+        f4 v = red[f * 64 + lane];
+        for (int w = 1; w < NW; w++) v = v + red[(w * NFR + f) * 64 + lane];
+        const int n = n0 + (f % NF) * 16 + fgrp * 4;
+        const int m = m_base + (f / NF) * 16 + frow;
+        const bool ok = m < p.M && n < N;
+        if constexpr (EPI == EPI_RESID_F32) {
+            v = v + bias_pre[j];
+            f4 o = (f4){0.f, 0.f, 0.f, 0.f};
+            if (ok) {
+                o = resid_pre[j] + v;
+                *(f4 *)((float *)p.out + (size_t)m * p.ldc + n) = o;
+            }
+            float s1 = (o[0] + o[1]) + (o[2] + o[3]);
+            float s2 = (o[0] * o[0] + o[1] * o[1]) + (o[2] * o[2] + o[3] * o[3]);
+            s1 += __shfl_xor(s1, 16); s2 += __shfl_xor(s2, 16);
+            s1 += __shfl_xor(s1, 32); s2 += __shfl_xor(s2, 32);
+            if (fgrp == 0) rowst[((f / NF) * 16 + frow) * NF + f % NF] = make_float2(s1, s2);
+        } else {
+            v = ln_apply(make_float2(0.f, 1.f), 1.0f, v, (f4){0.f, 0.f, 0.f, 0.f}, bias_pre[j]);
+            if constexpr (EPI == EPI_GELU_F16) {
+#pragma unroll
+                for (int r = 0; r < 4; r++) v[r] = gelu_tanh(v[r]);
+            } else {
+#pragma unroll
+                for (int r = 0; r < 4; r++) v[r] = gelu_quick(v[r]);
+            }
+            const h2 lo = (h2){(_Float16)v[0], (_Float16)v[1]};
+            const h2 hi = (h2){(_Float16)v[2], (_Float16)v[3]};
+            if (ok) *(uint2 *)((half_t *)p.out + (size_t)m * p.ldc + n) = make_uint2(h2u(lo), h2u(hi));
+        }
+    }
+    if constexpr (EPI == EPI_RESID_F32) {
+        if (p.stats_out) {
+            __syncthreads();
+            const int m = m_base + tid;
+            if (tid < MF * 16 && m < p.M && (int)blockIdx.x < TAIL_STATS_CAP) {
+                float s1 = 0.f, s2 = 0.f;
+#pragma unroll
+                for (int a = 0; a < NF; a++) { const float2 t = rowst[tid * NF + a]; s1 += t.x; s2 += t.y; }
+                p.stats_out[(size_t)m * TAIL_STATS_CAP + blockIdx.x] = make_float2(s1, s2);
+            }
+        }
+    }
+}
+
+template <int WT, int NFW>
+__global__ void __launch_bounds__(512) gemm_tail_proj_kernel(const TailParams p) {
+    constexpr int NW = 8;
+    constexpr int NG = NFW / 4;
+    constexpr bool Q4 = WT == W_Q4_0 || WT == W_Q4_1;
+    constexpr int CH = NG == 1 ? (Q4 ? 3 : 2) : (Q4 ? 3 : WT == W_F16 ? 2 : 1);
+    extern __shared__ __align__(16) unsigned char tail_smem[];
+    half_t * As = (half_t *)tail_smem;
+    __shared__ float sqp[NW][16];
+
+    const int tid = threadIdx.x;
+    const int lane = tid & 63;
+    const int wave = __builtin_amdgcn_readfirstlane(tid >> 6);
+    const int frow = lane & 15, fgrp = lane >> 4;
+    const int K = p.W.K, N = p.W.N;
+    const int pitch = K + 8;
+    const int nkb = K / 32, nfr = (N + 15) / 16;
+    const int m_base = blockIdx.x * 16;
+
+    TailW<WT> wA[CH][4], wB[CH][4];
+#define TP_LOAD(W_, g_, c_)                                                                                       \
+    _Pragma("unroll") for (int i = 0; i < CH; i++)                                                                \
+        if ((c_) + i < nkb) {                                                                                     \
+            _Pragma("unroll") for (int j = 0; j < 4; j++)                                                         \
+                if (wave + ((g_) * 4 + j) * NW < nfr) tail_load_w<WT>(W_[i][j], p.W, (wave + ((g_) * 4 + j) * NW) * 16 + frow, (c_) + i, fgrp); \
+        }
+    TP_LOAD(wA, 0, 0);
+
+    {
+        const int r = tid >> 5, sub = tid & 31;
+        const int m = m_base + r;
+        const size_t mc = (size_t)(m < p.M ? m : p.M - 1);
+        const float2 * st = p.stats_in + mc * TAIL_STATS_CAP;
+        float2 v[TAIL_STATS_CAP / 32];
+#pragma unroll
+        for (int i = 0; i < TAIL_STATS_CAP / 32; i++) {
+            const int sl = sub + 32 * i;
+            v[i] = sl < p.stats_slots ? st[sl] : make_float2(0.f, 0.f);
+        }
+        float s1 = 0.f, s2 = 0.f;
+#pragma unroll
+        for (int i = 0; i < TAIL_STATS_CAP / 32; i++) { s1 += v[i].x; s2 += v[i].y; }
+#pragma unroll
+        for (int o = 16; o > 0; o >>= 1) { s1 += __shfl_xor(s1, o); s2 += __shfl_xor(s2, o); }
+        const float mu = s1 / (float)K;
+        float var = s2 / (float)K - mu * mu;
+        var = var > 0.f ? var : 0.f;
+        const float rs = 1.0f / sqrtf(var + p.eps);
+        const float * xr = p.x32 + mc * p.ldx;
+        for (int c = sub * 8; c < K; c += 256) {
+            const f4 lo = *(const f4 *)(xr + c), hi = *(const f4 *)(xr + c + 4);
+            const f4 g0 = *(const f4 *)(p.ln_w + c), g1 = *(const f4 *)(p.ln_w + c + 4);
+            const f4 b0 = *(const f4 *)(p.ln_b + c), b1 = *(const f4 *)(p.ln_b + c + 4);
+            *(h8 *)(As + r * pitch + c) = normalise8(lo, hi, mu, rs, g0, g1, b0, b1);
+        }
+    }
+    __syncthreads();
+
+    f4 acc[NFW];
+#pragma unroll
+    for (int j = 0; j < NFW; j++) acc[j] = (f4){0.f, 0.f, 0.f, 0.f};
+#define TP_COMPUTE(W_, g_, c_)                                                                                    \
+    _Pragma("unroll") for (int i = 0; i < CH; i++)                                                                \
+        if ((c_) + i < nkb) {                                                                                     \
+            const h8 xf = *(const h8 *)(As + frow * pitch + ((c_) + i) * 32 + fgrp * 8);                          \
+            _Pragma("unroll") for (int j = 0; j < 4; j++)                                                         \
+                if (wave + ((g_) * 4 + j) * NW < nfr)                                                             \
+                    acc[(g_) * 4 + j] = __builtin_amdgcn_mfma_f32_16x16x32_f16(tail_wfrag<WT>(W_[i][j], fgrp), xf, acc[(g_) * 4 + j], 0, 0, 0); \
+        }
+#pragma unroll
+    for (int g = 0; g < NG; g++) {
+        if (g > 0) { TP_LOAD(wA, g, 0); }
+        for (int c = 0; c < nkb; c += 2 * CH) {
+            TP_LOAD(wB, g, c + CH);
+            TP_COMPUTE(wA, g, c);
+            TP_LOAD(wA, g, c + 2 * CH);
+            TP_COMPUTE(wB, g, c + CH);
+        }
+    }
+#undef TP_LOAD
+#undef TP_COMPUTE
+
+    float sq = 0.f;
+#pragma unroll
+    for (int j = 0; j < NFW; j++) {
+        const int n = (wave + j * NW) * 16 + fgrp * 4;
+        if (wave + j * NW < nfr && n < N) sq += (acc[j][0] * acc[j][0] + acc[j][1] * acc[j][1]) + (acc[j][2] * acc[j][2] + acc[j][3] * acc[j][3]);
+    }
+    sq += __shfl_xor(sq, 16);
+    sq += __shfl_xor(sq, 32);
+    if (fgrp == 0) sqp[wave][frow] = sq;
+    __syncthreads();
+    float tot = 0.f;
+#pragma unroll
+    for (int w = 0; w < NW; w++) tot += sqp[w][frow];
+    const float inv = p.normalize ? 1.0f / sqrtf(tot) : 1.0f;
+    const int m = m_base + frow;
+#pragma unroll
+    for (int j = 0; j < NFW; j++) {
+        const int n = (wave + j * NW) * 16 + fgrp * 4;
+        if (wave + j * NW < nfr && n < N && m < p.M) *(f4 *)((float *)p.out + (size_t)m * p.ldc + n) = acc[j] * inv;
+    }
+}
+
+template <int WT, int MF, int NF, int NW, int EPI>
+void launch_t(const TailParams & p, hipStream_t stream) {
+    hipLaunchKernelGGL((gemm_tail_kernel<WT, MF, NF, NW, EPI>), dim3((p.W.N + NF * 16 - 1) / (NF * 16), (p.M + MF * 16 - 1) / (MF * 16)), dim3(NW * 64), 0, stream, p);
+}
+
+template <int WT, int NFW>
+void launch_tp(const TailParams & p, hipStream_t stream) {
+    const size_t lds = (size_t)16 * (p.W.K + 8) * sizeof(half_t);
+    if (lds > 65536) {
+        static unsigned long long done = 0;
+        opt_in_dynamic_lds(gemm_tail_proj_kernel<WT, NFW>, lds, done);
+    }
+    hipLaunchKernelGGL((gemm_tail_proj_kernel<WT, NFW>), dim3((p.M + 15) / 16), dim3(512), lds, stream, p);
+}
+
+}
+
+#ifdef CLIPAMD_TAIL_WT
+#define CLIPAMD_TCAT2(a, b) a##b
+#define CLIPAMD_TCAT(a, b) CLIPAMD_TCAT2(a, b)
+void CLIPAMD_TCAT(launch_tail_wt, CLIPAMD_TAIL_WT)(const TailParams & p, int epilogue, hipStream_t stream) {
+    constexpr int WT = CLIPAMD_TAIL_WT;
+    switch (epilogue) {
+    case EPI_RESID_F32:
+        if (p.W.Kpad >= 2048) launch_t<WT, 2, TAIL_RESID_COLS / 16, 8, EPI_RESID_F32>(p, stream);
+        else launch_t<WT, 2, TAIL_RESID_COLS / 16, 4, EPI_RESID_F32>(p, stream);
+        break;
+    case EPI_GELU_F16: launch_t<WT, 2, 4, 4, EPI_GELU_F16>(p, stream); break;
+    case EPI_QGELU_F16: launch_t<WT, 2, 4, 4, EPI_QGELU_F16>(p, stream); break;
+    default: break;
+    }
+}
+void CLIPAMD_TCAT(launch_tail_proj_wt, CLIPAMD_TAIL_WT)(const TailParams & p, hipStream_t stream) {
+    if (p.W.N <= 512) launch_tp<CLIPAMD_TAIL_WT, 4>(p, stream);
+    else launch_tp<CLIPAMD_TAIL_WT, 8>(p, stream);
+}
+#else
+#define CLIPAMD_TAIL_DECL(n)                                              \
+    void launch_tail_wt##n(const TailParams &, int, hipStream_t);         \
+    void launch_tail_proj_wt##n(const TailParams &, hipStream_t);
+CLIPAMD_TAIL_DECL(0) CLIPAMD_TAIL_DECL(1) CLIPAMD_TAIL_DECL(2) CLIPAMD_TAIL_DECL(3) CLIPAMD_TAIL_DECL(4) CLIPAMD_TAIL_DECL(5)
+#undef CLIPAMD_TAIL_DECL
+
+void tail_shape(const TailParams & p, int epilogue, int & mf, int & nf, int & nw) {
+    mf = 2;
+    if (epilogue == EPI_RESID_F32) { nf = TAIL_RESID_COLS / 16; nw = p.W.Kpad >= 2048 ? 8 : 4; }
+    else { nf = 4; nw = 4; }
+}
+int tail_proj_nfw(const TailParams & p) { return p.W.N <= 512 ? 4 : 8; }
+
+static bool tail_weight_ok(const DevWeight & W) {
+    return W.wtype >= W_F16 && W.wtype <= W_Q8_0 && W.N > 0 && W.N % 4 == 0 && W.K > 0 && W.K == W.Kpad && W.Kpad % 32 == 0 && W.Npad % 128 == 0 && W.Npad >= W.N;
+}
+
+bool tail_supported(const TailParams & p, int epilogue) {
+    if (p.M <= 0 || !tail_weight_ok(p.W) || !p.out || p.ldc % 4 || p.ldc < p.W.N) return false;
+    if (epilogue == EPI_RESID_F32) {
+        if (!p.A16 || p.lda % 8 || p.lda < p.W.K || !p.resid || p.ldr % 4 || p.ldr < p.W.N || (!p.in_rows && p.in_row_mul < 0)) return false;
+        return !p.stats_out || (p.W.N + TAIL_RESID_COLS - 1) / TAIL_RESID_COLS <= TAIL_STATS_CAP;
+    }
+    if (epilogue != EPI_GELU_F16 && epilogue != EPI_QGELU_F16) return false;
+    return p.x32 && p.ldx % 4 == 0 && p.ldx >= p.W.K && p.W.K <= TAIL_LN_KMAX && p.ln_w && p.ln_b && p.stats_in && p.stats_slots > 0 && p.stats_slots <= TAIL_STATS_CAP;
+}
+
+bool tail_proj_supported(const TailParams & p) {
+    return p.M > 0 && tail_weight_ok(p.W) && p.W.N <= 1024 && p.W.K <= 2048 && p.out && p.ldc % 4 == 0 && p.ldc >= p.W.N && p.x32 && p.ldx % 4 == 0 && p.ldx >= p.W.K &&
+           p.ln_w && p.ln_b && p.stats_in && p.stats_slots > 0 && p.stats_slots <= TAIL_STATS_CAP;
+}
+
+void launch_tail(const TailParams & p, int epilogue, hipStream_t stream) {
+    switch (p.W.wtype) {
+    case W_F16: launch_tail_wt0(p, epilogue, stream); break;
+    case W_Q4_0: launch_tail_wt1(p, epilogue, stream); break;
+    case W_Q4_1: launch_tail_wt2(p, epilogue, stream); break;
+    case W_Q5_0: launch_tail_wt3(p, epilogue, stream); break;
+    case W_Q5_1: launch_tail_wt4(p, epilogue, stream); break;
+    case W_Q8_0: launch_tail_wt5(p, epilogue, stream); break;
+    }
+}
+
+void launch_tail_proj(const TailParams & p, hipStream_t stream) {
+    switch (p.W.wtype) {
+    case W_F16: launch_tail_proj_wt0(p, stream); break;
+    case W_Q4_0: launch_tail_proj_wt1(p, stream); break;
+    case W_Q4_1: launch_tail_proj_wt2(p, stream); break;
+    case W_Q5_0: launch_tail_proj_wt3(p, stream); break;
+    case W_Q5_1: launch_tail_proj_wt4(p, stream); break;
+    case W_Q8_0: launch_tail_proj_wt5(p, stream); break;
+    }
+}
+#endif
+
+}
diff --git a/clip_cpp_amd/csrc/kernels.h b/clip_cpp_amd/csrc/kernels.h
--- a/clip_cpp_amd/csrc/kernels.h
+++ b/clip_cpp_amd/csrc/kernels.h
@@ -146,6 +146,37 @@
 void launch_skinny(const SkinnyParams & p, int epilogue, hipStream_t stream);
 void launch_row_stats(const float * x, int ldx, int rows, int h, float2 * stats, hipStream_t stream);
 
+struct TailParams {
+    int M = 0;
+    DevWeight W;
+    const float * bias = nullptr;
+    const half_t * A16 = nullptr;
+    int lda = 0;
+    const float * x32 = nullptr;
+    int ldx = 0;
+    const float * ln_w = nullptr, * ln_b = nullptr;
+    float eps = 0.f;
+    const float2 * stats_in = nullptr;
+    int stats_slots = 0;
+    const int * in_rows = nullptr;
+    int in_row_mul = 1;
+    const float * resid = nullptr;
+    int ldr = 0;
+    void * out = nullptr;
+    int ldc = 0;
+    float2 * stats_out = nullptr;
+    bool normalize = true;
+};
+constexpr int TAIL_STATS_CAP = 128;
+constexpr int TAIL_RESID_COLS = 32;
+constexpr int TAIL_LN_KMAX = 3072;
+bool tail_supported(const TailParams & p, int epilogue);
+void launch_tail(const TailParams & p, int epilogue, hipStream_t stream);
+bool tail_proj_supported(const TailParams & p);
+void launch_tail_proj(const TailParams & p, hipStream_t stream);
+void tail_shape(const TailParams & p, int epilogue, int & mf, int & nf, int & nw);
+int tail_proj_nfw(const TailParams & p);
+
 void launch_layernorm(const float * x, int ldx, const int * in_rows, int in_row_mul, const float * w, const float * b, float eps,
                       int rows, int h, half_t * out16, int ld16, float * out32, int ld32, hipStream_t stream);
 void launch_layernorm_prep(const float * x, int ldx, const float * w, const float * b, float eps, int rows, int h, float * out32, int ld32,
diff --git a/clip_cpp_amd/csrc/load.cpp b/clip_cpp_amd/csrc/load.cpp
--- a/clip_cpp_amd/csrc/load.cpp
+++ b/clip_cpp_amd/csrc/load.cpp
@@ -588,6 +588,8 @@
         ctx->f32_acts = !(ef && ef[0] == '0');
         const char * ep = getenv("CLIP_AMD_PRUNE_LAST");
         ctx->prune_last = !(ep && ep[0] == '0');
+        const char * et = getenv("CLIP_AMD_POOLED_TAIL");
+        ctx->pooled_tail4 = !(et && et[0] == '0');
         const char * ec = getenv("CLIP_AMD_LNFOLD_CENTRE");
         ctx->ln_fold_centre = !(ec && ec[0] == '0');
     }
@@ -620,7 +622,7 @@
     c->vision = owner->vision; c->text = owner->text;
     c->weights_borrowed = true;
     c->owner = owner;
-    c->ln_fold = owner->ln_fold; c->ln_fold_force = owner->ln_fold_force; c->ln_fold_centre = owner->ln_fold_centre; c->prune_last = owner->prune_last;
+    c->ln_fold = owner->ln_fold; c->ln_fold_force = owner->ln_fold_force; c->ln_fold_centre = owner->ln_fold_centre; c->prune_last = owner->prune_last; c->pooled_tail4 = owner->pooled_tail4;
     c->f32_acts = owner->f32_acts;
     c->resident_panels_on = owner->resident_panels_on;
     c->graphs_enabled = false;
diff --git a/clip_cpp_amd/csrc/model.h b/clip_cpp_amd/csrc/model.h
--- a/clip_cpp_amd/csrc/model.h
+++ b/clip_cpp_amd/csrc/model.h
@@ -131,6 +131,7 @@
     float2 * sk_stats = nullptr;
     bool ln_fold_force = false;
     bool prune_last = true;
+    bool pooled_tail4 = true;
     bool ln_fold_centre = true;
     bool ln_fold = true;
     clipamd::half_t * w16_panel = nullptr;
@@ -187,6 +188,7 @@
     half_t * xn = nullptr, * qkv = nullptr, * att = nullptr, * mid = nullptr, * pooled = nullptr;
     float * xp = nullptr;
     half_t * ap = nullptr, * xnp = nullptr, * midp = nullptr;
+    float2 * tst = nullptr;
 };
 struct VisionStage {
     TowerBufs b;
diff --git a/include/clip_amd.h b/include/clip_amd.h
--- a/include/clip_amd.h
+++ b/include/clip_amd.h
@@ -147,6 +147,9 @@
 int clip_amd_test_skinny(int type, const void * w_raw, int64_t N, int64_t K, const float * x, int64_t M, const float * bias,
                          const float * resid, const float * ln_w, const float * ln_b, float eps, float * y, int epilogue,
                          int qcols, float qscale, float * stats_out);
+int clip_amd_test_tail(int op, int type, const void * w_raw, int64_t N, int64_t K, const float * a, int64_t a_rows, const int32_t * idx, int in_row_mul,
+                       int64_t M, const float * bias, const float * resid, const float * ln_w, const float * ln_b, float eps, const float * stats_in,
+                       int slots, int act, int normalize, float * y, float * stats_out);
 int clip_amd_test_layernorm(const float * x, const float * w, const float * b, float eps, int64_t rows, int64_t h,
                             float * y, int out_f16);
 int clip_amd_test_layernorm_ex(const float * x, int64_t x_rows, int ldx, const int32_t * in_rows, int in_row_mul, const float * w, const float * b,
```
